# YannisLamp/crypto-recommendation

Measured on AMD Instinct MI355X. Metric: point hash+assign ops/sec at d=128, N=10M, K=256; 1/2/4/8 MI355X, higher is better.
Workload: dtype fp32 points; split-f16 MFMA scores (f32 accumulate); tuples, bucket IDs and cluster IDs bit-exact (x87-exact hashing, certified argmin); distances: certified f32, <= 2^-20 relative to the reference's fp64 (north star: 1e-5; the context's default LSHKM_DIST_CERTIFIED mode), LSHKM_DIST_EXACT for the r; 1 GPU; C3 Lloyd K=256 + C2 LSH L=5 k=4 hashing, N=10000000 per GPU, d=128; N_per_gpu=10000000, N_total=10000000, d=128, K=256, L=5, k=4, nb=100000, parallelism=dp1 (row shards)

## Files before the change

### crypto-recommendation_amd/csrc/api.cpp

```cpp
#include <hip/hip_runtime.h>

#include <algorithm>
#include <cmath>
#include <cstring>
#include <map>
#include <mutex>
#include <random>
#include <sstream>
#include <string>
#include <vector>

#include "../../include/lshkm.h"
#include "common.h"
#include "kernels.h"
#include "index.h"

namespace lshkm {
static thread_local std::string g_err;
void set_error(const std::string& msg) { g_err = msg; }

int device_cu_count(int* ncu) {
    static std::mutex mu;
    static std::map<int, int> cus;
    int dev = 0;
// ... 288 lines not shown
    return 0;
}

extern "C" {

int lshkm_kmeans_pp(lshkm_ctx ctx, const float* X, int64_t N, int d, int K, int metric, uint64_t seed,
                    int32_t* rows) {
    return kmeans_pp_impl(ctx, X, N, d, K, metric, seed, rows);
}

int lshkm_kmeans_pp_f64(lshkm_ctx ctx, const double* X, int64_t N, int d, int K, int metric, uint64_t seed,
                        int32_t* rows) {
    return kmeans_pp_impl(ctx, X, N, d, K, metric, seed, rows);
}

}

struct KppShardHost {
    uint64_t max_bits;
    double sum, s_out;
    int64_t pick;
};

static int kpp_shard_ws_check(lshkm_ctx ctx, int64_t n, const void* ws, int64_t ws_bytes) {
    LSHKM_CHECK(ctx && n >= 0 && n <= INT32_MAX, LSHKM_ERR_ARG, "bad arguments (need 0 <= n < 2^31)");
    LSHKM_CHECK(n == 0 || (ws && ws_bytes >= 0 && (size_t)ws_bytes >= kmeans_pp_ws_bytes(n)), LSHKM_ERR_ARG,
                "workspace smaller than lshkm_kpp_shard_ws_bytes");
    LSHKM_HIP(hipSetDevice(ctx->device));
    return 0;
}

static int kpp_shard_read(lshkm_ctx ctx, int64_t n, const void* ws, KppShardHost* out) {
    LSHKM_HIP(hipMemcpyAsync(out, (const char*)ws + kpp_shard_out_offset(n), sizeof(*out), hipMemcpyDeviceToHost,
                             ctx->stream));
    LSHKM_HIP(hipStreamSynchronize(ctx->stream));
    return 0;
}

static int kpp_shard_dist_impl(lshkm_ctx ctx, Pts X, int64_t n, int d, int metric, const void* c, int it, void* ws,
                               int64_t ws_bytes, uint64_t* max_bits, double* sum) {
    if (const int rc = kpp_shard_ws_check(ctx, n, ws, ws_bytes)) return rc;
    LSHKM_CHECK(max_bits && sum && d >= 1 && d <= 4096 && it >= 1, LSHKM_ERR_ARG,
                "bad arguments (need 1 <= d <= 4096, it >= 1)");
    LSHKM_CHECK(metric == LSHKM_METRIC_EUCLIDEAN || metric == LSHKM_METRIC_COSINE, LSHKM_ERR_ARG, "unknown metric");
    *max_bits = 0;
    *sum = 0.0;
    if (n == 0) return 0;
    LSHKM_CHECK(X.p && c, LSHKM_ERR_ARG, "rows or centroid row is NULL");
    KppShardHost o;
    int rc;
    if ((rc = launch_kpp_shard_dist(ctx->stream, X, n, d, metric, c, it, ws)) || (rc = kpp_shard_read(ctx, n, ws, &o))) {
        (void)hipStreamSynchronize(ctx->stream);
        return rc;
    }
    *max_bits = o.max_bits;
    *sum = o.sum;
    return 0;
}

extern "C" {

int lshkm_kpp_shard_ws_bytes(int64_t n, int64_t* bytes) {
    LSHKM_CHECK(bytes && n >= 0 && n <= INT32_MAX, LSHKM_ERR_ARG, "bad arguments (need 0 <= n < 2^31)");
    *bytes = (int64_t)kmeans_pp_ws_bytes(n);
    return 0;
}

int lshkm_kpp_shard_dist(lshkm_ctx ctx, const float* X, int64_t n, int d, int metric, const float* c, int it, void* ws,
                         int64_t ws_bytes, uint64_t* max_bits, double* sum) {
    return kpp_shard_dist_impl(ctx, X, n, d, metric, c, it, ws, ws_bytes, max_bits, sum);
}

int lshkm_kpp_shard_dist_f64(lshkm_ctx ctx, const double* X, int64_t n, int d, int metric, const double* c, int it,
                             void* ws, int64_t ws_bytes, uint64_t* max_bits, double* sum) {
    return kpp_shard_dist_impl(ctx, X, n, d, metric, c, it, ws, ws_bytes, max_bits, sum);
}

int lshkm_kpp_shard_units(lshkm_ctx ctx, int64_t n, uint64_t gmax_bits, double start, void* ws, int64_t ws_bytes) {
    if (const int rc = kpp_shard_ws_check(ctx, n, ws, ws_bytes)) return rc;
    if (n == 0) return 0;
    return launch_kpp_shard_units(ctx->stream, n, gmax_bits, start, ws);
}

int lshkm_kpp_shard_chain(lshkm_ctx ctx, int64_t n, double s_in, void* ws, int64_t ws_bytes, double* s_out) {
    if (const int rc = kpp_shard_ws_check(ctx, n, ws, ws_bytes)) return rc;
    LSHKM_CHECK(s_out, LSHKM_ERR_ARG, "s_out is NULL");
    *s_out = s_in;
    if (n == 0) return 0;
    KppShardHost o;
    int rc;
    if ((rc = launch_kpp_shard_chain(ctx->stream, n, s_in, ws, (unsigned long long*)ctx->stats.p)) ||
        (rc = kpp_shard_read(ctx, n, ws, &o))) {
        (void)hipStreamSynchronize(ctx->stream);
        return rc;
    }
    *s_out = o.s_out;
    return 0;
}

int lshkm_kpp_shard_pick(lshkm_ctx ctx, int64_t n, double rd, int owns_row0, void* ws, int64_t ws_bytes,
                         int64_t* row) {
    if (const int rc = kpp_shard_ws_check(ctx, n, ws, ws_bytes)) return rc;
    LSHKM_CHECK(row, LSHKM_ERR_ARG, "row is NULL");
    *row = -1;
    if (n == 0) return 0;
    KppShardHost o;
    int rc;
    if ((rc = launch_kpp_shard_pick(ctx->stream, n, rd, owns_row0, ws)) || (rc = kpp_shard_read(ctx, n, ws, &o))) {
        (void)hipStreamSynchronize(ctx->stream);
        return rc;
    }
    LSHKM_CHECK(o.pick >= -1 && o.pick < n, LSHKM_ERR_STATE, "pick outside the shard (rd above the running sum?)");
    *row = o.pick;
    return 0;
}

int lshkm_params_cube_cosine(uint64_t seed, int k, int d, double* R, uint32_t* state) {
    LSHKM_CHECK(k > 0 && d > 0 && R, LSHKM_ERR_ARG, "bad arguments");
    std::default_random_engine g;
    g.seed((unsigned long)seed);
    for (int i = 0; i < k; i++) draw_cosine_h(g, d, R + (size_t)i * d);
    if (state) *state = engine_state(g);
    return 0;
}

}

namespace lshkm {

int ProjTable::upload(hipStream_t s, int metric_, int d_, int L_, int k_, float w_, const float* V, const float* t,
                      const int32_t* r, const double* R) {
    metric = metric_; d = d_; L = L_; k = k_; w = w_;
    LK = L * k;
    LKpad = hash_lkpad(LK);
    const int drows = (d + 3) / 4 * 4;
    std::vector<double> PT((size_t)drows * LKpad, 0.0), pn(LK, 0.0);
    std::vector<float> tt(LK, 0.f);
    std::vector<int32_t> rr(LK, 0);
    for (int f = 0; f < LK; f++) {
        long double n2 = 0.0L;
        for (int j = 0; j < d; j++) {
            const double v = metric == LSHKM_METRIC_EUCLIDEAN ? (double)V[(size_t)f * d + j] : R[(size_t)f * d + j];
            PT[(size_t)j * LKpad + f] = v;
            n2 += (long double)v * (long double)v;
        }
        pn[f] = (double)sqrtl(n2) * (1.0 + 0x1p-40);
        if (metric == LSHKM_METRIC_EUCLIDEAN) { tt[f] = t ? t[f] : 0.f; rr[f] = r ? r[f] : 0; }
    }
    int rc;
    if ((rc = PT_d.reserve(PT.size() * 8)) || (rc = t_d.reserve(LK * 4)) || (rc = pn_d.reserve(LK * 8)) ||
        (rc = r_d.reserve(LK * 4)))
        return rc;
    LSHKM_HIP(hipMemcpyAsync(PT_d.p, PT.data(), PT.size() * 8, hipMemcpyHostToDevice, s));
    LSHKM_HIP(hipMemcpyAsync(t_d.p, tt.data(), LK * 4, hipMemcpyHostToDevice, s));
    LSHKM_HIP(hipMemcpyAsync(pn_d.p, pn.data(), LK * 8, hipMemcpyHostToDevice, s));
    LSHKM_HIP(hipMemcpyAsync(r_d.p, rr.data(), LK * 4, hipMemcpyHostToDevice, s));
    bool r_small = true;
    for (int f = 0; f < LK; f++) r_small = r_small && rr[f] >= 0 && rr[f] <= 100;
    fused_ok = metric == LSHKM_METRIC_EUCLIDEAN && d == 128 && LK <= 32 && r_small;
    mfma_ok = d == 128 && LK <= 32;
    std::vector<_Float16> vh, vl;
    std::vector<double> v1;
    if (mfma_ok) {
        vh.assign(64 * 128, (_Float16)0.f);
        vl.assign(64 * 128, (_Float16)0.f);
        v1.assign(LK, 0.0);
        for (int f = 0; f < LK; f++) {
            long double s1 = 0.0L;
            for (int j = 0; j < 128; j++) {
                const double v = metric == LSHKM_METRIC_EUCLIDEAN ? (double)V[(size_t)f * d + j] : R[(size_t)f * d + j];
                const _Float16 hv = (_Float16)v;
                vh[f * 128 + j] = hv;
                vl[f * 128 + j] = (_Float16)(float)(v - (double)hv);
                s1 += fabsl((long double)v);
            }
            v1[f] = (double)s1 * (1.0 + 0x1p-40);
        }
        if ((rc = vh_d.reserve(vh.size() * 2)) || (rc = vl_d.reserve(vl.size() * 2)) || (rc = v1_d.reserve(LK * 8)))
            return rc;
        LSHKM_HIP(hipMemcpyAsync(vh_d.p, vh.data(), vh.size() * 2, hipMemcpyHostToDevice, s));
        LSHKM_HIP(hipMemcpyAsync(vl_d.p, vl.data(), vl.size() * 2, hipMemcpyHostToDevice, s));
        LSHKM_HIP(hipMemcpyAsync(v1_d.p, v1.data(), LK * 8, hipMemcpyHostToDevice, s));
    }
    LSHKM_HIP(hipStreamSynchronize(s));
    hV.assign(V ? V : (const float*)nullptr, V ? V + (size_t)LK * d : nullptr);
    return 0;
}

HashParams ProjTable::params(int64_t nb) const {
    HashParams p;
    p.PT = (const double*)PT_d.p;
    p.t = (const float*)t_d.p;
    p.pnorm = (const double*)pn_d.p;
    p.r = (const int32_t*)r_d.p;
    p.w = w;
    p.d = d; p.L = L; p.k = k; p.LK = LK; p.LKpad = LKpad;
    p.nb = nb;
    return p;
}

HashMfmaParams ProjTable::mfma_params(int64_t nb) const {
    HashMfmaParams p;
    p.Vh = vh_d.as<_Float16>(); p.Vl = vl_d.as<_Float16>();
    p.t = (const float*)t_d.p; p.pnorm = (const double*)pn_d.p; p.v1 = (const double*)v1_d.p;
    p.r = (const int32_t*)r_d.p; p.PT = (const double*)PT_d.p;
    p.w = w;
    p.d = d; p.L = L; p.k = k; p.LK = LK; p.LKpad = LKpad;
    p.nb = nb;
    return p;
}

}

extern "C" {

int lshkm_lsh_create(lshkm_ctx ctx, int metric, int d, int k, int L, int64_t nb, float w, const float* V,
                     const float* t, const int32_t* r, const double* R, lshkm_lsh* out) {
    LSHKM_CHECK(ctx && out, LSHKM_ERR_ARG, "ctx/out is NULL");
    LSHKM_CHECK(d > 0 && d <= 1024 && k > 0 && L > 0 && L * k <= 256, LSHKM_ERR_ARG, "unsupported d/k/L");
    LSHKM_CHECK(k <= 30, LSHKM_ERR_ARG, "k > 30");
    if (metric == LSHKM_METRIC_EUCLIDEAN) {
        LSHKM_CHECK(V && t && r, LSHKM_ERR_ARG, "euclidean LSH needs V, t, r");
        LSHKM_CHECK(nb > 0 && nb < (1ll << 31), LSHKM_ERR_ARG, "nb must be in [1, 2^31)");
        LSHKM_CHECK(w > 0.f, LSHKM_ERR_ARG, "w must be > 0");
    } else if (metric == LSHKM_METRIC_COSINE) {
        LSHKM_CHECK(R, LSHKM_ERR_ARG, "cosine LSH needs R");
        nb = (int64_t)1 << k;
    } else {
        set_error("unknown metric");
        return LSHKM_ERR_ARG;
    }
    LSHKM_HIP(hipSetDevice(ctx->device));
    lshkm_lsh h = new lshkm_lsh_s();
    h->ctx = ctx; h->metric = metric; h->nb = nb;
    int rc = h->proj.upload(ctx->stream, metric, d, L, k, w, V, t, r, R);
    if (rc) { delete h; return rc; }
    *out = h;
    return 0;
}

int lshkm_lsh_destroy(lshkm_lsh lsh) {
    if (!lsh) return 0;
    (void)hipDeviceSynchronize();
    delete lsh;
    return 0;
}

}

static int lsh_hash_impl(lshkm_lsh lsh, Pts X, int64_t N, int32_t* tuples, int32_t* phi, int32_t* bucket) {
    LSHKM_CHECK(lsh && (X.p || N == 0) && N >= 0, LSHKM_ERR_ARG, "bad arguments");
    lshkm_ctx ctx = lsh->ctx;
    LSHKM_HIP(hipSetDevice(ctx->device));
    const int mode = lsh->metric == LSHKM_METRIC_EUCLIDEAN ? HM_LSH_EUCLID : HM_LSH_COSINE;
    const int rc = hash_rows(ctx, mode, X, N, lsh->proj, lsh->nb, mode == HM_LSH_EUCLID ? tuples : nullptr, phi, bucket,
                             nullptr);
    if (rc) { LSHKM_LAUNCH_CHECK(); return rc; }
    return 0;
}

extern "C" {

int lshkm_lsh_hash(lshkm_lsh lsh, const float* X, int64_t N, int32_t* tuples, int32_t* phi, int32_t* bucket) {
    return lsh_hash_impl(lsh, X, N, tuples, phi, bucket);
}

int lshkm_lsh_hash_f64(lshkm_lsh lsh, const double* X, int64_t N, int32_t* tuples, int32_t* phi, int32_t* bucket) {
    return lsh_hash_impl(lsh, X, N, tuples, phi, bucket);
}

}

static int assign_path(int metric, int d, int K, bool f64) {
    if (test_switch("LSHKM_ASSIGN_PATH", "exact")) return 2;
    if (!test_switch("LSHKM_ASSIGN_PATH", "f32")) {
        const FusedRoute r = fused_route(metric != LSHKM_METRIC_EUCLIDEAN, f64, d, K, false, 0, 0,
                                         test_switch("LSHKM_FUSED_FORM", "chunked"));
        if (r.form != FusedForm::none) return r.rows == 0 ? 0 : 3;
    }
    return assign_dp(d) > 0 ? 1 : 2;
}

static bool fuse_hash(const lshkm_lsh_s* lsh, int metric, int K, bool f64) {
    const lshkm::ProjTable& pj = lsh->proj;
    if (lsh->metric != metric || !(metric == LSHKM_METRIC_EUCLIDEAN ? pj.fused_ok : pj.mfma_ok)) return false;
    return fused_route(metric != LSHKM_METRIC_EUCLIDEAN, f64, pj.d, K, true, pj.k, pj.LK,
                       test_switch("LSHKM_FUSED_FORM", "chunked")).form != FusedForm::none;
}

bool lshkm::exact_pruned(Pts X, int d, int K, int metric) {
    return K <= 1024 && d <= 256 && !test_switch("LSHKM_EXACT_PASS", "full") &&
           (metric == LSHKM_METRIC_EUCLIDEAN || !X.f64);
}

static size_t exact_ct_bytes(const AssignJob& q) { return (size_t)q.d * ((q.K + 255) / 256 * 256) * 8; }

int lshkm::exact_listed_prep(lshkm_ctx ctx, const AssignJob& q) {
    int rc;
    if ((rc = ctx->ws_ct.reserve(exact_ct_bytes(q)))) return rc;
    return launch_assign_pruned_prep(ctx->stream, q.X.f64, q.d, q.C, q.K, (float*)ctx->ws_ct.p,
                                     q.metric == LSHKM_METRIC_EUCLIDEAN ? 0 : 1);
}

int lshkm::exact_listed(lshkm_ctx ctx, const AssignJob& q, const RowList& l, bool exact_dist, bool prepped,
                        const double* xn2, const double* nbv) {
    const bool prune = exact_pruned(q.X, q.d, q.K, q.metric);
    if (!prune && (q.metric != LSHKM_METRIC_EUCLIDEAN || (l.nseg == 0 && q.d > 256)))
        return launch_assign_exact(ctx->stream, q, l, xn2, nbv);
    int rc;
    if ((rc = ctx->ws_ct.reserve(exact_ct_bytes(q)))) return rc;
    if (prune) return launch_assign_pruned_list(ctx->stream, q, (float*)ctx->ws_ct.p, l, exact_dist ? 1 : 0, prepped);
    return launch_assign_exact_list(ctx->stream, q, (double*)ctx->ws_ct.p, l);
}

static int assign_f32_mfma(lshkm_ctx ctx, const AssignJob& q) {
    hipStream_t s = ctx->stream;
    const int DP = assign_dp(q.d), Kpad = (q.K + 63) / 64 * 64;
    const int64_t N = q.N;
    int rc;
    if ((rc = ctx->ws_c32.reserve((size_t)Kpad * DP * 4)) || (rc = ctx->ws_cconst.reserve((size_t)3 * Kpad * 4)) ||
        (rc = ctx->ws_ambig.reserve((size_t)std::max<int64_t>(N, 1) * 2 * 4)) ||
        (rc = ctx->ws_counter.reserve(64)))
        return rc;
    unsigned long long* cnt = (unsigned long long*)ctx->ws_counter.p;
    LSHKM_HIP(hipMemsetAsync(cnt, 0, 16, s));
    if ((rc = launch_centroid_prep(s, q.C, q.K, Kpad, q.d, DP, q.metric, q.X.f64, (float*)ctx->ws_c32.p, (float*)ctx->ws_cconst.p))) return rc;
    if ((rc = launch_assign_mfma(s, q.X, N, q.d, DP, q.C, q.K, Kpad, q.metric, (const float*)ctx->ws_c32.p, (const float*)ctx->ws_cconst.p,
                                 q.assign, q.dist, (int32_t*)ctx->ws_ambig.p, cnt))) return rc;
    RowList l;
    l.p = (int32_t*)ctx->ws_ambig.p; l.count = cnt; l.bound = N;
    if ((rc = exact_listed(ctx, q, l, true, false, nullptr, nullptr))) return rc;
    if (q.metric != LSHKM_METRIC_EUCLIDEAN &&
        ((rc = launch_cos_fix(s, q.X, N, q.d, q.C, (const int32_t*)ctx->ws_ambig.p + N, cnt + 1, q.assign, q.dist)) ||
         (rc = launch_add_counter(s, (unsigned long long*)ctx->stats.p + STAT_COS_FIX, cnt + 1)))) return rc;
    return launch_add_counter(s, (unsigned long long*)ctx->stats.p + STAT_ASSIGN_AMBIG, cnt);
}

static int assign_impl(lshkm_ctx ctx, Pts X, int64_t N, int d, const double* C, int K, int metric,
                       const int32_t* src_rows_host, int32_t* assign, double* dist, lshkm_lsh lsh, int32_t* tuples,
                       int32_t* phi, int32_t* bucket, bool force_exact = false) {
    hipStream_t s = ctx->stream;
    const int path = assign_path(metric, d, K, X.f64);
    AssignRequest q;
    q.X = X; q.N = N; q.d = d; q.C = C; q.K = K; q.metric = metric; q.assign = assign; q.dist = dist;
    q.tuples = tuples; q.phi = phi; q.bucket = bucket; q.force_exact = force_exact;
    if (lsh && path == 0 && fuse_hash(lsh, metric, K, X.f64)) q.lsh = lsh;
    int rc;
    if (lsh && !q.lsh && (rc = hash_rows(ctx, lsh->metric == LSHKM_METRIC_EUCLIDEAN ? HM_LSH_EUCLID : HM_LSH_COSINE,
                                         X, N, lsh->proj, lsh->nb,
                                         lsh->metric == LSHKM_METRIC_EUCLIDEAN ? tuples : nullptr, phi, bucket,
                                         nullptr))) { LSHKM_LAUNCH_CHECK(); return rc; }
    if (path == 0 || path == 3) rc = fused_assign(ctx, q);
    else if (path == 1) rc = assign_f32_mfma(ctx, q);
    else {
        RowList all;
        all.bound = N;
        rc = launch_assign_exact(s, q, all);
    }
    if (rc) { LSHKM_LAUNCH_CHECK(); return rc; }
    if (src_rows_host) {
        if ((rc = ctx->ws_src.reserve((size_t)K * 4))) return rc;
        const bool same = ctx->src_cache_dev == ctx->ws_src.p && ctx->src_cache_cap == ctx->ws_src.cap &&
                          ctx->src_cache.size() == (size_t)K &&
                          std::memcmp(ctx->src_cache.data(), src_rows_host, (size_t)K * 4) == 0;
        if (!same) {
            if ((rc = ctx->pin_stage((size_t)K * 4))) return rc;
            std::memcpy(ctx->pinned, src_rows_host, (size_t)K * 4);
            LSHKM_HIP(hipMemcpyAsync(ctx->ws_src.p, ctx->pinned, (size_t)K * 4, hipMemcpyHostToDevice, s));
            LSHKM_HIP(hipEventRecord(ctx->pinned_ev, s));
            ctx->src_cache.assign(src_rows_host, src_rows_host + K);
            ctx->src_cache_dev = ctx->ws_src.p;
            ctx->src_cache_cap = ctx->ws_src.cap;
        }
        if ((rc = launch_assign_override(s, (const int32_t*)ctx->ws_src.p, K, N, assign, dist))) { LSHKM_LAUNCH_CHECK(); return rc; }
    }
    return 0;
}

static int lloyd_impl(lshkm_ctx ctx, Pts X, int64_t N, int d, const double* C, int K, int metric,
                      const int32_t* src_rows_host, int32_t* assign, double* dist) {
    LSHKM_CHECK(ctx && (X.p || N == 0) && C && (assign || N == 0) && (dist || N == 0) && N >= 0 && d > 0 && K > 0,
                LSHKM_ERR_ARG, "bad arguments");
    LSHKM_CHECK(metric == LSHKM_METRIC_EUCLIDEAN || metric == LSHKM_METRIC_COSINE, LSHKM_ERR_ARG, "unknown metric");
    LSHKM_HIP(hipSetDevice(ctx->device));
    return assign_impl(ctx, X, N, d, C, K, metric, src_rows_host, assign, dist, nullptr, nullptr, nullptr, nullptr);
}

static int hash_assign_impl(lshkm_lsh lsh, Pts X, int64_t N, const double* C, int K, const int32_t* src_rows_host,
                            int32_t* tuples, int32_t* phi, int32_t* bucket, int32_t* assign, double* dist,
                            int metric = LSHKM_METRIC_EUCLIDEAN) {
    LSHKM_CHECK(lsh && (X.p || N == 0) && C && (assign || N == 0) && (dist || N == 0) && N >= 0 && K > 0, LSHKM_ERR_ARG,
                "bad arguments");
    lshkm_ctx ctx = lsh->ctx;
    LSHKM_HIP(hipSetDevice(ctx->device));
    LSHKM_CHECK(metric == LSHKM_METRIC_EUCLIDEAN || metric == LSHKM_METRIC_COSINE, LSHKM_ERR_ARG, "unknown metric");
    return assign_impl(ctx, X, N, lsh->proj.d, C, K, metric, src_rows_host, assign, dist, lsh, tuples, phi, bucket);
}

static int range_impl(lshkm_ctx ctx, Pts X, int64_t N, int d, const double* C, int K, int metric,
                      const int64_t* comb_ptr, const int32_t* comb_idx, const int32_t* key_host,
                      const int32_t* src_rows_host, int32_t* assign, double* dist, int* passes_host) {
    LSHKM_CHECK(ctx && (X.p || N == 0) && C && comb_ptr && (assign || N == 0) && (dist || N == 0) && N >= 0 &&
                    N < (1ll << 31) && d > 0 && K > 0,
                LSHKM_ERR_ARG, "bad arguments");
    LSHKM_CHECK(metric == LSHKM_METRIC_EUCLIDEAN || metric == LSHKM_METRIC_COSINE, LSHKM_ERR_ARG, "unknown metric");
    LSHKM_HIP(hipSetDevice(ctx->device));
    hipStream_t s = ctx->stream;
    lshkm::Buf* w = ctx->ws_range;
    int rc;
    int64_t M = 0;
    LSHKM_HIP(hipMemcpyAsync(&M, comb_ptr + K, 8, hipMemcpyDeviceToHost, s));
    LSHKM_HIP(hipStreamSynchronize(s));
    LSHKM_CHECK(M >= 0 && (M == 0 || comb_idx), LSHKM_ERR_ARG, "bad combined-bucket CSR");
    const size_t scratch = sort_scratch_bytes(std::max<int64_t>(M, 1), std::max<int64_t>(N, 1));
    if ((rc = w[0].reserve(64)) || (rc = w[1].reserve((size_t)std::max<int64_t>(M, 1) * 4 * 4)) ||
        (rc = w[2].reserve(scratch)) || (rc = w[3].reserve((size_t)(N + 1) * 8)) ||
        (rc = w[4].reserve((size_t)std::max<int64_t>(M, 1) * 9)) || (rc = w[5].reserve((size_t)K * 4)))
        return rc;
    double* r0 = (double*)w[0].p;
    unsigned long long* cnt = (unsigned long long*)w[0].p + 1;
    int32_t* rows = (int32_t*)w[1].p;
    int32_t* cents = rows + std::max<int64_t>(M, 1);
    int32_t* rows_s = cents + std::max<int64_t>(M, 1);
    int32_t* cents_s = rows_s + std::max<int64_t>(M, 1);
    int64_t* vptr = (int64_t*)w[3].p;
    double* cache = (double*)w[4].p;
    int8_t* cached = (int8_t*)(cache + std::max<int64_t>(M, 1));
    const int32_t* key = nullptr;
    if (key_host) {
        LSHKM_HIP(hipMemcpyAsync(w[5].p, key_host, (size_t)K * 4, hipMemcpyHostToDevice, s));
        key = (const int32_t*)w[5].p;
    }
    if ((rc = launch_range_radius(s, C, K, d, metric, r0, (unsigned long long*)w[0].p + 4))) return rc;
    if ((rc = launch_range_init(s, N, assign, dist))) return rc;
    int passes = 0;
    if (M > 0 && N > 0) {
        if ((rc = launch_range_pairs(s, comb_ptr, comb_idx, K, rows, cents))) return rc;
        if ((rc = stable_sort_by_key(s, rows, 1, cents, M, N, rows_s, cents_s, w[2].p))) return rc;
        if ((rc = launch_csr_bounds(s, rows_s, M, N, vptr))) return rc;
        LSHKM_HIP(hipMemsetAsync(cached, 0, (size_t)M, s));
        for (;;) {
            unsigned long long assigned = 0;
            LSHKM_HIP(hipMemsetAsync(cnt, 0, 8, s));
            if ((rc = launch_range_pass(s, X, d, C, K, metric, key, vptr, cents_s, cache, cached, N, r0, passes,
                                        assign, dist, cnt)))
                return rc;
            passes++;
            LSHKM_HIP(hipMemcpyAsync(&assigned, cnt, 8, hipMemcpyDeviceToHost, s));
            LSHKM_HIP(hipStreamSynchronize(s));
            if (!assigned) break;
        }
    } else {
        passes = 1;
    }
    if (N > 0) {
        if ((rc = w[6].reserve((size_t)N * 4))) return rc;
        int32_t* list = (int32_t*)w[6].p;
        unsigned long long* ucnt = cnt + 1;
        unsigned long long U = 0;
        LSHKM_HIP(hipMemsetAsync(ucnt, 0, 8, s));
        if ((rc = launch_range_unassigned(s, assign, N, list, ucnt))) return rc;
        LSHKM_HIP(hipMemcpyAsync(&U, ucnt, 8, hipMemcpyDeviceToHost, s));
        LSHKM_HIP(hipStreamSynchronize(s));
        if (U > 0) {
            if ((rc = w[7].reserve((size_t)U * d * X.esize())) || (rc = w[8].reserve((size_t)U * 12))) return rc;
            double* dr = (double*)w[8].p;
            int32_t* ar = (int32_t*)(dr + U);
            if ((rc = launch_range_gather(s, X, d, list, (int64_t)U, w[7].p))) return rc;
            const Pts Xr = X.f64 ? Pts(w[7].as<double>()) : Pts(w[7].as<float>());
            rc = assign_impl(ctx, Xr, (int64_t)U, d, C, K, metric, nullptr, ar, dr, nullptr, nullptr, nullptr, nullptr,
                             true);
            if (rc) return rc;
            if ((rc = launch_range_scatter(s, list, (int64_t)U, ar, dr, assign, dist))) return rc;
        }
    }
    if (src_rows_host) {
        if ((rc = ctx->ws_src.reserve((size_t)K * 4))) return rc;
        ctx->src_cache_dev = nullptr;
        LSHKM_HIP(hipMemcpyAsync(ctx->ws_src.p, src_rows_host, (size_t)K * 4, hipMemcpyHostToDevice, s));
        if ((rc = launch_assign_override(s, (const int32_t*)ctx->ws_src.p, K, N, assign, dist))) return rc;
        LSHKM_HIP(hipStreamSynchronize(s));
    }
    if (key_host) LSHKM_HIP(hipStreamSynchronize(s));
    if (passes_host) *passes_host = passes;
    return 0;
}

extern "C" {

int lshkm_lloyd_assign(lshkm_ctx ctx, const float* X, int64_t N, int d, const double* C, int K, int metric,
                       const int32_t* src_rows_host, int32_t* assign, double* dist) {
    return lloyd_impl(ctx, X, N, d, C, K, metric, src_rows_host, assign, dist);
}

int lshkm_lloyd_assign_f64(lshkm_ctx ctx, const double* X, int64_t N, int d, const double* C, int K, int metric,
                           const int32_t* src_rows_host, int32_t* assign, double* dist) {
    return lloyd_impl(ctx, X, N, d, C, K, metric, src_rows_host, assign, dist);
}

int lshkm_hash_assign(lshkm_lsh lsh, const float* X, int64_t N, const double* C, int K, const int32_t* src_rows_host,
                      int32_t* tuples, int32_t* phi, int32_t* bucket, int32_t* assign, double* dist) {
    return hash_assign_impl(lsh, X, N, C, K, src_rows_host, tuples, phi, bucket, assign, dist);
}

int lshkm_hash_assign_f64(lshkm_lsh lsh, const double* X, int64_t N, const double* C, int K,
                          const int32_t* src_rows_host, int32_t* tuples, int32_t* phi, int32_t* bucket,
                          int32_t* assign, double* dist) {
    return hash_assign_impl(lsh, X, N, C, K, src_rows_host, tuples, phi, bucket, assign, dist);
}

int lshkm_hash_assign_metric(lshkm_lsh lsh, const float* X, int64_t N, const double* C, int K, int metric,
                             const int32_t* src_rows_host, int32_t* tuples, int32_t* phi, int32_t* bucket,
                             int32_t* assign, double* dist) {
    return hash_assign_impl(lsh, X, N, C, K, src_rows_host, tuples, phi, bucket, assign, dist, metric);
}

int lshkm_hash_assign_metric_f64(lshkm_lsh lsh, const double* X, int64_t N, const double* C, int K, int metric,
                                 const int32_t* src_rows_host, int32_t* tuples, int32_t* phi, int32_t* bucket,
                                 int32_t* assign, double* dist) {
    return hash_assign_impl(lsh, X, N, C, K, src_rows_host, tuples, phi, bucket, assign, dist, metric);
}

int lshkm_range_assign(lshkm_ctx ctx, const float* X, int64_t N, int d, const double* C, int K, int metric,
                       const int64_t* comb_ptr, const int32_t* comb_idx, const int32_t* key_host,
                       const int32_t* src_rows_host, int32_t* assign, double* dist, int* passes_host) {
    return range_impl(ctx, X, N, d, C, K, metric, comb_ptr, comb_idx, key_host, src_rows_host, assign, dist,
                      passes_host);
}

int lshkm_range_assign_f64(lshkm_ctx ctx, const double* X, int64_t N, int d, const double* C, int K, int metric,
                           const int64_t* comb_ptr, const int32_t* comb_idx, const int32_t* key_host,
                           const int32_t* src_rows_host, int32_t* assign, double* dist, int* passes_host) {
    return range_impl(ctx, X, N, d, C, K, metric, comb_ptr, comb_idx, key_host, src_rows_host, assign, dist,
                      passes_host);
}

int lshkm_synth(lshkm_ctx ctx, uint64_t seed, int64_t row0, int64_t rows, int d, float* X) {
    LSHKM_CHECK(ctx && (X || rows == 0) && rows >= 0 && d > 0, LSHKM_ERR_ARG, "bad arguments");
    LSHKM_HIP(hipSetDevice(ctx->device));
    int rc = launch_synth(ctx->stream, seed, row0, rows, d, X);
    if (rc) { LSHKM_LAUNCH_CHECK(); }
    return rc;
}

int lshkm_synth_normal(lshkm_ctx ctx, uint64_t seed, int64_t row0, int64_t rows, int d, float* X) {
    LSHKM_CHECK(ctx && (X || rows == 0) && rows >= 0 && d > 0, LSHKM_ERR_ARG, "bad arguments");
    LSHKM_HIP(hipSetDevice(ctx->device));
    int rc = launch_synth(ctx->stream, seed, row0, rows, d, X, 1);
    if (rc) { LSHKM_LAUNCH_CHECK(); }
    return rc;
}

}
```

### crypto-recommendation_amd/csrc/assign.hip

```cpp
#include "common.h"
#include "kernels.h"
#include "exact.h"

namespace lshkm {

constexpr int AS_THREADS = 256;
constexpr int AS_PB = 128;
constexpr int AS_CC = 64;

typedef float floatx16 __attribute__((ext_vector_type(16)));

int assign_dp(int d) {
    const int dps[] = {16, 32, 64, 128, 256};
    for (int dp : dps)
        if (d <= dp) return dp;
    return 0;
}

__global__ void centroid_prep_kernel(const double* __restrict__ C, int K, int Kpad, int d, int DP, int metric,
                                     int xf64, float* __restrict__ C32, float* __restrict__ cconst) {
    const int c = blockIdx.x * 64 + threadIdx.x;
    const double xw = xf64 ? 2.0 : 0.0;
    float* cn2 = cconst;
    float* chunk = cconst + Kpad + 2 * blockIdx.x;
// ... 269 lines not shown

constexpr int XC_MAXV = 4;
constexpr int XE_SPLIT = 2;
template <typename TX>
__global__ __launch_bounds__(256) void assign_exact_kernel(
    const TX* __restrict__ X, int64_t N, int d, const double* __restrict__ C, int K, int metric,
    const int32_t* __restrict__ rows, const unsigned long long* __restrict__ row_count, int64_t max_rows,
    int32_t* __restrict__ assign, double* __restrict__ dist, const int32_t* __restrict__ seg_counts,
    int64_t seg_rows, const double* __restrict__ xn2, const double* __restrict__ nbv) {
    const int lane = threadIdx.x & 63;
    int64_t wglobal = (int64_t)blockIdx.x * 4 + (threadIdx.x >> 6);
    int64_t nw = (int64_t)gridDim.x * 4;
    int64_t total = rows ? (int64_t)*row_count : N;
    if (seg_counts) {
        const int seg = blockIdx.x % (gridDim.x / XE_SPLIT);
        rows += (int64_t)seg * seg_rows;
        total = seg_counts[SEG_SLOTS * seg + SEG_ROWS];
        wglobal = (int64_t)(blockIdx.x / (gridDim.x / XE_SPLIT)) * 4 + (threadIdx.x >> 6);
        nw = XE_SPLIT * 4;
    }
    if (total > max_rows) total = max_rows;
    for (int64_t it = wglobal; it < total; it += nw) {
        const int64_t row = rows ? rows[it] : it;
        const TX* x = X + row * d;
        double best = 0.0; int bi = -1;
        const double xa = metric == 1 && xn2 ? xn2[row] : -1.0;
        if (metric == 1 && K <= 64 * XC_MAXV) {
            double v[XC_MAXV], rad[XC_MAXV];
            int st[XC_MAXV];
            double U = __builtin_inf();
            bool unknown = false;
#pragma unroll
            for (int k = 0; k < XC_MAXV; k++) {
                const int c = lane + 64 * k;
                st[k] = 0; v[k] = 0.0; rad[k] = 0.0;
                if (c < K) {
                    st[k] = cosine_interval(x, C + (size_t)c * d, d, v[k], rad[k], xa, nbv ? nbv[c] : -1.0);
                    unknown |= st[k] == 2;
                    if (st[k] != 2) U = fmin(U, v[k] + rad[k]);
                }
            }
            if (!__ballot(unknown)) {
                for (int off = 32; off >= 1; off >>= 1) U = fmin(U, __shfl_xor(U, off));
#pragma unroll
                for (int k = 0; k < XC_MAXV; k++) {
                    const int c = lane + 64 * k;
                    if (c < K && v[k] - rad[k] <= U) {
                        const double dd = st[k] == 0 ? v[k] : exact_cosine_x87(x, C + (size_t)c * d, d, xa, nbv ? nbv[c] : -1.0);
                        if (bi < 0 || dd < best) { best = dd; bi = c; }
                    }
                }
                for (int off = 32; off >= 1; off >>= 1) {
                    const double ob = __shfl_xor(best, off);
                    const int oi = __shfl_xor(bi, off);
                    const bool take = oi >= 0 && (bi < 0 || ob < best || (ob == best && oi < bi));
                    if (take) { best = ob; bi = oi; }
                }
                if (lane == 0) {
                    assign[row] = bi;
                    dist[row] = best;
                }
                continue;
            }
        }
        for (int c = lane; c < K; c += 64) {
            const double dd = metric == 0 ? exact_euclid(x, C + (size_t)c * d, d)
                                          : exact_cosine_x87(x, C + (size_t)c * d, d, xa, nbv ? nbv[c] : -1.0);
            if (bi < 0 ? (dd == dd || c == 0) : dd < best) { best = dd; bi = c; }
        }
        for (int off = 32; off >= 1; off >>= 1) {
            const double ob = __shfl_xor(best, off);
            const int oi = __shfl_xor(bi, off);
            const bool take = oi >= 0 && (bi < 0 || ob < best || (ob == best && oi < bi));
            if (take) { best = ob; bi = oi; }
        }
        if (lane == 0) {
            assign[row] = bi < 0 ? 0 : bi;
            dist[row] = bi < 0 ? -1.0 : best;
        }
    }
}

int launch_assign_exact(hipStream_t s, const AssignJob& q, const RowList& l, const double* xn2, const double* nbv) {
    const Pts X = q.X;
    const int64_t N = q.N, max_rows = l.bound, seg_rows = l.seg_rows;
    const int d = q.d, K = q.K, metric = q.metric, nseg = l.nseg;
    const double* C = q.C;
    const int32_t *rows = l.p, *seg_counts = l.seg_counts();
    const unsigned long long* row_count = l.count;
    int32_t* assign = q.assign;
    double* dist = q.dist;
    if (max_rows <= 0) return 0;
    const int64_t blocks = seg_counts ? (int64_t)nseg * XE_SPLIT : std::min<int64_t>((max_rows + 3) / 4, rows ? 256 : 2048);
    if (blocks <= 0) return 0;
    if (X.f64)
        hipLaunchKernelGGL(assign_exact_kernel<double>, dim3((unsigned)blocks), dim3(256), 0, s, X.d(), N, d, C, K,
                           metric, rows, row_count, max_rows, assign, dist, seg_counts, seg_rows, xn2, nbv);
    else
        hipLaunchKernelGGL(assign_exact_kernel<float>, dim3((unsigned)blocks), dim3(256), 0, s, X.f(), N, d, C, K,
                           metric, rows, row_count, max_rows, assign, dist, seg_counts, seg_rows, xn2, nbv);
    return kstatus("assign.hip");
}

constexpr int XB_R = 8;
constexpr int XB_WAVES = 4;
constexpr int XB_SPLIT = 4;
constexpr int XB_DMAX = 256;

__global__ void transpose_centroids_kernel(const double* __restrict__ C, int K, int Kpad, int d,
                                           double* __restrict__ CT) {
    const int64_t e = (int64_t)blockIdx.x * blockDim.x + threadIdx.x;
    if (e >= (int64_t)d * Kpad) return;
    const int j = (int)(e / Kpad), c = (int)(e % Kpad);
    CT[e] = c < K ? C[(size_t)c * d + j] : 0.0;
}

template <typename TX>
__global__ __launch_bounds__(64 * XB_WAVES) void assign_exact_batch_kernel(
    const TX* __restrict__ X, int d, const double* __restrict__ CT, int K, int Kpad,
    const int32_t* __restrict__ rows, const unsigned long long* __restrict__ row_count, int64_t max_rows,
    int32_t* __restrict__ assign, double* __restrict__ dist, const int32_t* __restrict__ seg_counts,
    int64_t seg_rows) {
    __shared__ TX xs[XB_WAVES][XB_R][XB_DMAX];
    const int lane = threadIdx.x & 63, wave = threadIdx.x >> 6;
    int64_t total, g0, gstride;
    if (seg_counts) {
        const int nseg = gridDim.x / XB_SPLIT;
        const int seg = blockIdx.x % nseg, part = blockIdx.x / nseg;
        rows += (int64_t)seg * seg_rows;
        total = seg_counts[SEG_SLOTS * seg + SEG_ROWS];
        g0 = (int64_t)part * XB_WAVES + wave;
        gstride = (int64_t)XB_SPLIT * XB_WAVES;
    } else {
        total = (int64_t)*row_count;
        if (total > max_rows) total = max_rows;
        g0 = (int64_t)blockIdx.x * XB_WAVES + wave;
        gstride = (int64_t)gridDim.x * XB_WAVES;
    }
    const int64_t ngroups = (total + XB_R - 1) / XB_R;
    for (int64_t g = g0; g < ngroups; g += gstride) {
        const int nr = (int)min((int64_t)XB_R, total - g * XB_R);
        int64_t myrow[XB_R];
#pragma unroll
        for (int r = 0; r < XB_R; r++) myrow[r] = rows[g * XB_R + min(r, nr - 1)];
#pragma unroll
        for (int r = 0; r < XB_R; r++)
            for (int j = lane; j < d; j += 64) xs[wave][r][j] = X[myrow[r] * d + j];
        wave_sync();
        double best[XB_R];
        int bi[XB_R];
#pragma unroll
        for (int r = 0; r < XB_R; r++) { best[r] = 0.0; bi[r] = -1; }
        for (int c0 = 0; c0 < K; c0 += 256) {
            double acc[XB_R][4];
#pragma unroll
            for (int r = 0; r < XB_R; r++)
#pragma unroll
                for (int i = 0; i < 4; i++) acc[r][i] = 0.0;
            const double* ct = CT + c0 + lane;
#pragma unroll 4
            for (int j = 0; j < d; j++) {
                double cv[4];
#pragma unroll
                for (int i = 0; i < 4; i++) cv[i] = ct[(size_t)j * Kpad + 64 * i];
#pragma unroll
                for (int r = 0; r < XB_R; r++) {
                    const double xj = (double)xs[wave][r][j];
#pragma unroll
                    for (int i = 0; i < 4; i++) {
                        const double df = __dsub_rn(xj, cv[i]);
                        acc[r][i] = __dadd_rn(acc[r][i], gp_sq(df));
                    }
                }
            }
#pragma unroll
            for (int i = 0; i < 4; i++) {
                const int c = c0 + lane + 64 * i;
                if (c >= K) continue;
#pragma unroll
                for (int r = 0; r < XB_R; r++) {
                    const double dd = sqrt(acc[r][i]);
                    if (bi[r] < 0 || dd < best[r]) { best[r] = dd; bi[r] = c; }
                }
            }
        }
#pragma unroll
        for (int r = 0; r < XB_R; r++) {
            double b = best[r];
            int i1 = bi[r];
            for (int off = 32; off >= 1; off >>= 1) {
                const double ob = __shfl_xor(b, off);
                const int oi = __shfl_xor(i1, off);
                const bool take = oi >= 0 && (i1 < 0 || ob < b || (ob == b && oi < i1));
                if (take) { b = ob; i1 = oi; }
            }
            if (lane == 0 && r < nr) {
                assign[myrow[r]] = i1;
                dist[myrow[r]] = b;
            }
        }
        wave_sync();
    }
}

#ifndef XP_ROWS
#define XP_ROWS 8
#endif
#ifndef XP_SPLITS
#define XP_SPLITS 4
#endif
constexpr int XP_R = XP_ROWS;
#ifndef XP_WIDE_ROWS
#define XP_WIDE_ROWS 2
#endif
constexpr int XP_WR = XP_WIDE_ROWS;
constexpr int XP_WAVES = 4;
constexpr int XP_SPLIT = XP_SPLITS;

template <typename TX>
__device__ __attribute__((always_inline)) inline double exact_euclid_rolled(const TX* __restrict__ x,
                                                                            const double* __restrict__ c, int d) {
    double acc = 0.0;
#pragma unroll 1
    for (int j = 0; j < d; j++) acc = __dadd_rn(acc, gp_sq(__dsub_rn((double)x[j], c[j])));
    return sqrt(acc);
}

template <int MET, typename TX>
__device__ inline double pruned_dist(const TX* __restrict__ x, const double* __restrict__ c, int d) {
    if constexpr (MET == 0) {
        return exact_euclid_rolled(x, c, d);
    } else {
        if constexpr (sizeof(TX) == 4) {
            if ((d & 15) == 0) return exact_cosine_x87_b16(x, c, d);
        }
        return exact_cosine_x87(x, c, d);
    }
}

template <typename TX>
__device__ inline double euclid_sumsq_mul(const TX* __restrict__ x, const double* __restrict__ c, int d, PwAcc& pw) {
    double acc = 0.0;
    for (int j0 = 0; j0 < d; j0 += 16) {
        double cv[16];
#pragma unroll
        for (int t = 0; t < 16; t++) cv[t] = j0 + t < d ? c[j0 + t] : 0.0;
#pragma unroll
        for (int t = 0; t < 16; t++)
            if (j0 + t < d) {
                const double df = __dsub_rn((double)x[j0 + t], cv[t]);
                const double p = __dmul_rn(df, df);
                pw.add<true>(df);
                acc = __dadd_rn(acc, p);
            }
    }
    return acc;
}

template <int G>
__device__ inline void group_argmin(double& best, int& bi) {
#pragma unroll
    for (int off = G / 2; off >= 1; off >>= 1) {
        const double ob = __shfl_xor(best, off);
        const int oi = __shfl_xor(bi, off);
        const bool take = oi >= 0 && (bi < 0 || ob < best || (ob == best && oi < bi));
        if (take) { best = ob; bi = oi; }
    }
}
template <int G>
__device__ inline double group_min(double v) {
#pragma unroll
    for (int off = G / 2; off >= 1; off >>= 1) v = fmin(v, __shfl_xor(v, off));
    return v;
}

template <int G, typename TX>
__device__ inline void pruned_pick_euclid(const TX* __restrict__ xr, const double* __restrict__ C, int d, int c,
                                          bool exact_dist, double& best, int& bi) {
    PwAcc pw;
    const double S = c >= 0 ? euclid_sumsq_mul(xr, C + (size_t)c * d, d, pw) : 0.0;
    const bool hard = c >= 0 && pw.hard();
    best = c >= 0 ? sqrt(S) : 0.0;
    bi = c;
    group_argmin<G>(best, bi);
    int anyh = hard ? 1 : 0;
#pragma unroll
    for (int off = G / 2; off >= 1; off >>= 1) anyh |= __shfl_xor(anyh, off);
    if (!anyh) return;
    const double S1 = group_min<G>(c >= 0 && c == bi ? S : __builtin_inf());
    const double S2 = group_min<G>(c >= 0 && c != bi ? S : __builtin_inf());
    if (S2 != __builtin_inf() && !(S2 - S1 > 0x1p-41 * S2)) {
        best = c >= 0 ? exact_euclid_rolled(xr, C + (size_t)c * d, d) : 0.0;
        bi = c;
        group_argmin<G>(best, bi);
        return;
    }
    if (!exact_dist) return;
    const int w = bi;
    double v = __builtin_inf();
    if (c == w) v = hard ? exact_euclid_rolled(xr, C + (size_t)c * d, d) : best;
    best = group_min<G>(v);
}

__global__ void exact_prep_kernel(const double* __restrict__ C, int K, int Kpad, int d, int xf64,
                                  float* __restrict__ CT32, float* __restrict__ cconst, int metric) {
    const int c = blockIdx.x, lane = threadIdx.x;
    double scale = 1.0;
    if (metric == 1) {
        double q = 0.0;
        for (int j = lane; j < d; j += 64) {
            const double v = c < K ? C[(size_t)c * d + j] : 0.0;
            q = fma(v, v, q);
        }
        for (int off = 32; off >= 1; off >>= 1) q += __shfl_xor(q, off);
        scale = (q >= 1e-200 && q <= 1e200) ? 1.0 / sqrt(q) : 0.0;
        if (c < K && scale == 0.0) {
            for (int j = lane; j < d; j += 64) CT32[(size_t)j * Kpad + c] = 0.f;
            if (lane == 0) cconst[c] = __builtin_inff();
            return;
        }
    }
    double sq = 0.0;
    for (int j = lane; j < d; j += 64) {
        const double v = c < K ? C[(size_t)c * d + j] * scale : 0.0;
        sq = fma(v, v, sq);
        CT32[(size_t)j * Kpad + c] = (float)v;
    }
    for (int off = 32; off >= 1; off >>= 1) sq += __shfl_xor(sq, off);
    if (lane != 0) return;
    if (c >= K) { cconst[c] = __builtin_inff(); return; }
    if (metric == 1) {
        cconst[c] = 0.f;
        const double ec = ((d + 2.0) * 0x1p-24 * (1.0 + 0x1p-10) + 0x1p-40 + (xf64 ? 0x1p-23 : 0.0)) * (1.0 + 0x1p-18);
        unsigned int* chunk = reinterpret_cast<unsigned int*>(cconst + Kpad + 2 * (c / 64));
        atomicMax(chunk, __float_as_uint((float)(ec * (1.0 + 0x1p-20))));
        atomicMax(chunk + 1, __float_as_uint(1e-30f));
        return;
    }
    const double up = 1.0 + 0x1p-18;
    const double nc = sqrt(sq) * (1.0 + 0x1p-30);
    cconst[c] = (float)sq;
    const double ec = 0x1p-24 * (2.0 * d + 12.0 + (xf64 ? 2.0 : 0.0)) * nc * up;
    const double eb = (0x1p-24 * 5.0 * sq + 0x1p-40 * sq + (xf64 ? 0x1p-140 * nc : 0.0)) * up + 1e-30;
    unsigned int* chunk = reinterpret_cast<unsigned int*>(cconst + Kpad + 2 * (c / 64));
    atomicMax(chunk, __float_as_uint((float)(ec * (1.0 + 0x1p-20))));
    atomicMax(chunk + 1, __float_as_uint((float)(eb * (1.0 + 0x1p-20))));
}

template <typename TX, int NCH = 4, int R = XP_R, int MET = 0>
__global__ __launch_bounds__(64 * XP_WAVES) void assign_pruned_kernel(
    const TX* __restrict__ X, int d, const double* __restrict__ C, const float* __restrict__ CT32,
    const float* __restrict__ cconst, int K, int Kpad, const int32_t* __restrict__ rows,
    const unsigned long long* __restrict__ row_count, int64_t max_rows, int32_t* __restrict__ assign,
    double* __restrict__ dist, const int32_t* __restrict__ seg_counts, int64_t seg_rows, int exact_dist) {
    constexpr int RL = 64 / R;
    __shared__ TX xs[XP_WAVES][R][XB_DMAX];
    const int lane = threadIdx.x & 63, wave = threadIdx.x >> 6;
    int64_t total, g0, gstride;
    if (seg_counts) {
        const int nseg = gridDim.x / XP_SPLIT;
        const int seg = blockIdx.x % nseg, part = blockIdx.x / nseg;
        rows += (int64_t)seg * seg_rows;
        total = seg_counts[SEG_SLOTS * seg + SEG_ROWS];
        g0 = (int64_t)part * XP_WAVES + wave;
        gstride = (int64_t)XP_SPLIT * XP_WAVES;
    } else {
        total = (int64_t)*row_count;
        if (total > max_rows) total = max_rows;
        g0 = (int64_t)blockIdx.x * XP_WAVES + wave;
        gstride = (int64_t)gridDim.x * XP_WAVES;
    }
    const float* chunkc = cconst + Kpad;
    const int64_t ngroups = (total + R - 1) / R;
    for (int64_t g = g0; g < ngroups; g += gstride) {
        const int nr = (int)min((int64_t)R, total - g * R);
        int32_t myrow[R];
#pragma unroll
        for (int r = 0; r < R; r++) myrow[r] = rows[g * R + min(r, nr - 1)];
        float xn2p[R];
        TX xv[R][XB_DMAX / 64];
#pragma unroll
        for (int r = 0; r < R; r++)
#pragma unroll
            for (int u = 0; u < XB_DMAX / 64; u++) {
                const int j = lane + 64 * u;
                xv[r][u] = j < d ? X[(int64_t)myrow[r] * d + j] : TX(0);
            }
#pragma unroll
        for (int r = 0; r < R; r++) {
            float q = 0.f;
#pragma unroll
            for (int u = 0; u < XB_DMAX / 64; u++) {
                const int j = lane + 64 * u;
                if (j < d) {
                    xs[wave][r][j] = xv[r][u];
                    q = fmaf((float)xv[r][u], (float)xv[r][u], q);
                }
            }
            xn2p[r] = q;
        }
        wave_sync();
        float acc[R][NCH];
#pragma unroll
        for (int r = 0; r < R; r++)
#pragma unroll
            for (int i = 0; i < NCH; i++) acc[r][i] = 0.f;
        int coff[NCH];
#pragma unroll
        for (int i = 0; i < NCH; i++) coff[i] = (64 * i < Kpad ? 64 * i : 0) + lane;
#pragma unroll 8
        for (int j = 0; j < d; j++) {
            float cv[NCH];
#pragma unroll
            for (int i = 0; i < NCH; i++) cv[i] = CT32[(size_t)j * Kpad + coff[i]];
#pragma unroll
            for (int r = 0; r < R; r++) {
                const float xj = (float)xs[wave][r][j];
#pragma unroll
                for (int i = 0; i < NCH; i++) acc[r][i] = fmaf(xj, cv[i], acc[r][i]);
            }
        }
        unsigned long long cm[R][NCH];
        int ncand[R];
        bool pr[R];
#pragma unroll
        for (int r = 0; r < R; r++) {
            double xn2 = (double)xn2p[r];
            for (int off = 32; off >= 1; off >>= 1) xn2 += __shfl_xor(xn2, off);
            xn2 = xn2 * (sizeof(TX) == 4 ? 1.0 + 0x1p-20 : 1.0 + 0x1p-19) + (sizeof(TX) == 4 ? 0.0 : 0x1p-280);
            const float nx = (float)(sqrt(xn2) * (1.0 + 0x1p-30));
            const float ex = (float)(0x1p-40 * xn2 * (1.0 + 0x1p-18) + 1e-30);
            float lo[NCH];
            float U = __builtin_inff();
            bool finite = nx <= 3.0e38f;
#pragma unroll
            for (int i = 0; i < NCH; i++) {
                const int c = lane + 64 * i;
                lo[i] = __builtin_inff();
                if (c < K) {
                    const float E = fmaf(nx, chunkc[2 * i], chunkc[2 * i + 1] + ex);
                    const float sc = MET == 1 ? cconst[c] - acc[r][i] : fmaf(-2.f, acc[r][i], cconst[c]);
                    lo[i] = sc - E;
                    const float hi = sc + E;
                    finite = finite && (hi - lo[i]) <= 3.0e38f;
                    U = fminf(U, hi);
                }
            }
            for (int off = 32; off >= 1; off >>= 1) U = fminf(U, __shfl_xor(U, off));
            ncand[r] = 0;
#pragma unroll
            for (int i = 0; i < NCH; i++) {
                cm[r][i] = __ballot(lo[i] <= U);
                ncand[r] += __popcll(cm[r][i]);
            }
            pr[r] = r < nr && __all(finite) && ncand[r] >= 1;
        }
        {
            const int r = lane / RL, k = lane % RL;
            int c = -1;
            int seen = 0;
#pragma unroll
            for (int rr = 0; rr < R; rr++) {
                if (rr != r || !pr[rr] || ncand[rr] > RL) continue;
#pragma unroll
                for (int i = 0; i < NCH; i++) {
                    const int n = __popcll(cm[rr][i]);
                    if (c < 0 && k >= seen && k < seen + n) {
                        unsigned long long m = cm[rr][i];
                        for (int t = k - seen; t > 0; t--) m &= m - 1;
                        c = 64 * i + __builtin_ctzll(m);
                    }
                    seen += n;
                }
            }
            double best = 0.0;
            int bi = -1;
            if constexpr (MET == 0) {
                pruned_pick_euclid<RL>(xs[wave][r], C, d, c, exact_dist != 0, best, bi);
            } else {
                if (c >= 0) {
                    best = pruned_dist<MET>(xs[wave][r], C + (size_t)c * d, d);
                    bi = c;
                }
                group_argmin<RL>(best, bi);
            }
            if (k == 0 && bi >= 0) {
                assign[myrow[r]] = bi;
                dist[myrow[r]] = best;
            }
        }
        for (int r = 0; r < nr; r++) {
            if (pr[r] && ncand[r] <= RL) continue;
            const bool prune = pr[r] && ncand[r] <= 64;
            const TX* xr = xs[wave][r];
            double best = 0.0;
            int bi = -1;
            if (prune) {
                int c = -1, seen = 0;
#pragma unroll
                for (int i = 0; i < NCH; i++) {
                    const int n = __popcll(cm[r][i]);
                    if (c < 0 && lane >= seen && lane < seen + n) {
                        unsigned long long m = cm[r][i];
                        for (int t = lane - seen; t > 0; t--) m &= m - 1;
                        c = 64 * i + __builtin_ctzll(m);
                    }
                    seen += n;
                }
                if constexpr (MET == 0) {
                    pruned_pick_euclid<64>(xr, C, d, c, exact_dist != 0, best, bi);
                } else if (c >= 0) {
                    best = pruned_dist<MET>(xr, C + (size_t)c * d, d);
                    bi = c;
                }
            } else {
                for (int c = lane; c < K; c += 64) {
                    const double dd = pruned_dist<MET>(xr, C + (size_t)c * d, d);
                    if (bi < 0 ? (dd == dd || c == 0) : dd < best) { best = dd; bi = c; }
                }
            }
            for (int off = 32; off >= 1; off >>= 1) {
                const double ob = __shfl_xor(best, off);
                const int oi = __shfl_xor(bi, off);
                const bool take = oi >= 0 && (bi < 0 || ob < best || (ob == best && oi < bi));
                if (take) { best = ob; bi = oi; }
            }
            if (lane == 0) {
                assign[myrow[r]] = bi < 0 ? 0 : bi;
                dist[myrow[r]] = bi < 0 ? -1.0 : best;
            }
        }
        wave_sync();
    }
}

#ifndef XPW_ROWS
#define XPW_ROWS 4
#endif
constexpr int XPW_MAXSEG = 4096;
template <typename TX, int MET = 0, int NCH = 16, int R = XPW_ROWS>
__global__ __launch_bounds__(64 * XP_WAVES) void assign_pruned_wide_kernel(
    const TX* __restrict__ X, int d, const double* __restrict__ C, const float* __restrict__ CT32,
    const float* __restrict__ cconst, int K, int Kpad, const int32_t* __restrict__ rows,
    const unsigned long long* __restrict__ row_count, int64_t max_rows, int32_t* __restrict__ assign,
    double* __restrict__ dist, const int32_t* __restrict__ seg_counts, int64_t seg_rows, int nseg, int exact_dist) {
    __shared__ TX xs[XP_WAVES][R][XB_DMAX];
    __shared__ int gpre[XPW_MAXSEG + 1];
    const int lane = threadIdx.x & 63, wave = threadIdx.x >> 6;
    int64_t ngroups;
    if (seg_counts) {
        for (int sg = threadIdx.x; sg < nseg; sg += 64 * XP_WAVES) gpre[sg + 1] = (seg_counts[SEG_SLOTS * sg + SEG_ROWS] + R - 1) / R;
        __syncthreads();
        if (threadIdx.x == 0) {
            gpre[0] = 0;
            for (int sg = 0; sg < nseg; sg++) gpre[sg + 1] += gpre[sg];
        }
        __syncthreads();
        ngroups = gpre[nseg];
    } else {
        int64_t total = (int64_t)*row_count;
        if (total > max_rows) total = max_rows;
        ngroups = (total + R - 1) / R;
    }
    const float* chunkc = cconst + Kpad;
    const int64_t g0 = (int64_t)blockIdx.x * XP_WAVES + wave, gstride = (int64_t)gridDim.x * XP_WAVES;
    for (int64_t g = g0; g < ngroups; g += gstride) {
        const int32_t* grows;
        int64_t gbase, cnt;
        if (seg_counts) {
            int lo = 0, hi = nseg;
            while (hi - lo > 1) {
                const int mid = (lo + hi) >> 1;
                if (gpre[mid] <= g) lo = mid; else hi = mid;
            }
            grows = rows + (int64_t)lo * seg_rows;
            gbase = (g - gpre[lo]) * R;
            cnt = seg_counts[SEG_SLOTS * lo + SEG_ROWS];
        } else {
            grows = rows;
            gbase = g * R;
            cnt = min((int64_t)*row_count, max_rows);
        }
        const int nr = (int)min((int64_t)R, cnt - gbase);
        int32_t myrow[R];
#pragma unroll
        for (int r = 0; r < R; r++) myrow[r] = grows[gbase + min(r, nr - 1)];
        float xn2p[R];
#pragma unroll
        for (int r = 0; r < R; r++) {
            TX xv[XB_DMAX / 64];
#pragma unroll
            for (int u = 0; u < XB_DMAX / 64; u++) {
                const int j = lane + 64 * u;
                xv[u] = j < d ? X[(int64_t)myrow[r] * d + j] : TX(0);
            }
            float q = 0.f;
#pragma unroll
            for (int u = 0; u < XB_DMAX / 64; u++) {
                const int j = lane + 64 * u;
                if (j < d) {
                    xs[wave][r][j] = xv[u];
                    q = fmaf((float)xv[u], (float)xv[u], q);
                }
            }
            xn2p[r] = q;
        }
        wave_sync();
        float acc[R][NCH];
#pragma unroll
        for (int r = 0; r < R; r++)
#pragma unroll
            for (int i = 0; i < NCH; i++) acc[r][i] = 0.f;
        int coff[NCH];
#pragma unroll
        for (int i = 0; i < NCH; i++) coff[i] = (64 * i < Kpad ? 64 * i : 0) + lane;
#pragma unroll 2
        for (int j = 0; j < d; j++) {
            float cv[NCH];
#pragma unroll
            for (int i = 0; i < NCH; i++) cv[i] = CT32[(size_t)j * Kpad + coff[i]];
#pragma unroll
            for (int r = 0; r < R; r++) {
                const float xj = (float)xs[wave][r][j];
#pragma unroll
                for (int i = 0; i < NCH; i++) acc[r][i] = fmaf(xj, cv[i], acc[r][i]);
            }
        }
#pragma unroll
        for (int r = 0; r < R; r++) {
            if (r >= nr) break;
            double xn2 = (double)xn2p[r];
            for (int off = 32; off >= 1; off >>= 1) xn2 += __shfl_xor(xn2, off);
            xn2 = xn2 * (sizeof(TX) == 4 ? 1.0 + 0x1p-20 : 1.0 + 0x1p-19) + (sizeof(TX) == 4 ? 0.0 : 0x1p-280);
            const float nx = (float)(sqrt(xn2) * (1.0 + 0x1p-30));
            const float ex = (float)(0x1p-40 * xn2 * (1.0 + 0x1p-18) + 1e-30);
            float lo[NCH];
            float U = __builtin_inff();
            bool finite = nx <= 3.0e38f;
#pragma unroll
            for (int i = 0; i < NCH; i++) {
                const int c = lane + 64 * i;
                lo[i] = __builtin_inff();
                if (c < K) {
                    const float E = fmaf(nx, chunkc[2 * i], chunkc[2 * i + 1] + ex);
                    const float sc = MET == 1 ? cconst[c] - acc[r][i] : fmaf(-2.f, acc[r][i], cconst[c]);
                    lo[i] = sc - E;
                    const float hi = sc + E;
                    finite = finite && (hi - lo[i]) <= 3.0e38f;
                    U = fminf(U, hi);
                }
            }
            for (int off = 32; off >= 1; off >>= 1) U = fminf(U, __shfl_xor(U, off));
            unsigned long long cm[NCH];
            int ncand = 0;
#pragma unroll
            for (int i = 0; i < NCH; i++) {
                cm[i] = __ballot(lo[i] <= U);
                ncand += __popcll(cm[i]);
            }
            const bool prune = __all(finite) && ncand >= 1 && ncand <= 64;
            const TX* xr = xs[wave][r];
            double best = 0.0;
            int bi = -1;
            if (prune) {
                int c = -1, seen = 0;
#pragma unroll
                for (int i = 0; i < NCH; i++) {
                    const int n = __popcll(cm[i]);
                    if (c < 0 && lane >= seen && lane < seen + n) {
                        unsigned long long m = cm[i];
                        for (int t = lane - seen; t > 0; t--) m &= m - 1;
                        c = 64 * i + __builtin_ctzll(m);
                    }
                    seen += n;
                }
                if constexpr (MET == 0) {
                    pruned_pick_euclid<64>(xr, C, d, c, exact_dist != 0, best, bi);
                } else if (c >= 0) {
                    best = pruned_dist<MET>(xr, C + (size_t)c * d, d);
                    bi = c;
                }
            } else {
                for (int c = lane; c < K; c += 64) {
                    const double dd = pruned_dist<MET>(xr, C + (size_t)c * d, d);
                    if (bi < 0 ? (dd == dd || c == 0) : dd < best) { best = dd; bi = c; }
                }
            }
            for (int off = 32; off >= 1; off >>= 1) {
                const double ob = __shfl_xor(best, off);
                const int oi = __shfl_xor(bi, off);
                const bool take = oi >= 0 && (bi < 0 || ob < best || (ob == best && oi < bi));
                if (take) { best = ob; bi = oi; }
            }
            if (lane == 0) {
                assign[myrow[r]] = bi < 0 ? 0 : bi;
                dist[myrow[r]] = bi < 0 ? -1.0 : best;
            }
        }
        wave_sync();
    }
}

int launch_assign_pruned_prep(hipStream_t s, bool xf64, int d, const double* C, int K, float* ws, int metric) {
    if (d > XB_DMAX || K > 1024) {
        set_error("launch_assign_pruned_prep: unsupported shape");
        return -1;
    }
    const int Kpad = (K + 63) / 64 * 64;
    float* cconst = ws + (size_t)d * Kpad;
    if (hipMemsetAsync(cconst + Kpad, 0, (size_t)(Kpad / 64) * 2 * 4, s) != hipSuccess) return kstatus("pruned prep");
    hipLaunchKernelGGL(exact_prep_kernel, dim3((unsigned)Kpad), dim3(64), 0, s, C, K, Kpad, d, xf64 ? 1 : 0, ws, cconst,
                       metric);
    return kstatus("exact_prep_kernel");
}

int launch_assign_pruned_list(hipStream_t s, const AssignJob& q, float* ws, const RowList& l, int exact_dist,
                              bool prepped) {
    const Pts X = q.X;
    const int64_t max_rows = l.bound, seg_rows = l.seg_rows;
    const int d = q.d, K = q.K, nseg = l.nseg, metric = q.metric == 0 ? 0 : 1;
    const double* C = q.C;
    const int32_t *rows = l.p, *seg_counts = l.seg_counts();
    const unsigned long long* row_count = l.count;
    int32_t* assign = q.assign;
    double* dist = q.dist;
    if (max_rows <= 0) return 0;
    if (d > XB_DMAX || K > 1024 || (seg_counts && nseg <= 0)) {
        set_error("launch_assign_pruned_list: unsupported shape");
        return -1;
    }
    const int Kpad = (K + 63) / 64 * 64;
    float* CT32 = ws;
    float* cconst = ws + (size_t)d * Kpad;
    if (!prepped) {
        int rc = launch_assign_pruned_prep(s, X.f64, d, C, K, ws, metric);
        if (rc) return rc;
    }
    const bool wide = Kpad > 256;
    const bool flat = wide && (!seg_counts || nseg <= XPW_MAXSEG);
    const int R = wide ? (flat ? XPW_ROWS : XP_WR) : XP_R;
    const int64_t groups = (max_rows + R - 1) / R;
    const int64_t blocks = seg_counts ? (int64_t)nseg * XP_SPLIT : std::min<int64_t>((groups + XP_WAVES - 1) / XP_WAVES, 2048);
#define XP_LAUNCH(TX, NCH, RR, MT, XP)                                                                              \
    hipLaunchKernelGGL((assign_pruned_kernel<TX, NCH, RR, MT>), dim3((unsigned)blocks), dim3(64 * XP_WAVES), 0, s, XP, \
                       d, C, CT32, cconst, K, Kpad, rows, row_count, max_rows, assign, dist, seg_counts, seg_rows, exact_dist)
#define XPW_LAUNCH(TX, MT, NC, RW, XP)                                                                           \
    hipLaunchKernelGGL((assign_pruned_wide_kernel<TX, MT, NC, RW>), dim3((unsigned)wblocks), dim3(64 * XP_WAVES), 0, s, \
                       XP, d, C, CT32, cconst, K, Kpad, rows, row_count, max_rows, assign, dist, seg_counts, seg_rows, nseg, \
                       exact_dist)
    const int64_t wblocks = std::min<int64_t>((groups + XP_WAVES - 1) / XP_WAVES, 1024);
    if (flat) {
        if (metric == 1) {
            if (X.f64) XPW_LAUNCH(double, 1, 16, XPW_ROWS, X.d()); else XPW_LAUNCH(float, 1, 16, XPW_ROWS, X.f());
        } else {
            if (X.f64) XPW_LAUNCH(double, 0, 16, XPW_ROWS, X.d()); else XPW_LAUNCH(float, 0, 16, XPW_ROWS, X.f());
        }
    } else if (metric == 1) {
        if (X.f64) {
            if (wide) XP_LAUNCH(double, 16, XP_WR, 1, X.d()); else XP_LAUNCH(double, 4, XP_R, 1, X.d());
        } else {
            if (wide) XP_LAUNCH(float, 16, XP_WR, 1, X.f()); else XP_LAUNCH(float, 4, XP_R, 1, X.f());
        }
    } else if (X.f64) {
        if (wide) XP_LAUNCH(double, 16, XP_WR, 0, X.d()); else XP_LAUNCH(double, 4, XP_R, 0, X.d());
    } else {
        if (wide) XP_LAUNCH(float, 16, XP_WR, 0, X.f()); else XP_LAUNCH(float, 4, XP_R, 0, X.f());
    }
#undef XP_LAUNCH
#undef XPW_LAUNCH
    return kstatus("assign_pruned_kernel");
}

int launch_assign_exact_list(hipStream_t s, const AssignJob& q, double* CT, const RowList& l) {
    const Pts X = q.X;
    const int64_t max_rows = l.bound, seg_rows = l.seg_rows;
    const int d = q.d, K = q.K, nseg = l.nseg;
    const double* C = q.C;
    const int32_t *rows = l.p, *seg_counts = l.seg_counts();
    const unsigned long long* row_count = l.count;
    int32_t* assign = q.assign;
    double* dist = q.dist;
    if (max_rows <= 0) return 0;
    if (d > XB_DMAX || (seg_counts && nseg <= 0)) {
        set_error("launch_assign_exact_list: unsupported shape");
        return -1;
    }
    const int Kpad = (K + 255) / 256 * 256;
    const int64_t ne = (int64_t)d * Kpad;
    hipLaunchKernelGGL(transpose_centroids_kernel, dim3((unsigned)((ne + 255) / 256)), dim3(256), 0, s, C, K, Kpad, d, CT);
    const int64_t groups = (max_rows + XB_R - 1) / XB_R;
    const int64_t blocks = seg_counts ? (int64_t)nseg * XB_SPLIT : std::min<int64_t>((groups + XB_WAVES - 1) / XB_WAVES, 2048);
    if (X.f64)
        hipLaunchKernelGGL(assign_exact_batch_kernel<double>, dim3((unsigned)blocks), dim3(64 * XB_WAVES), 0, s, X.d(),
                           d, CT, K, Kpad, rows, row_count, max_rows, assign, dist, seg_counts, seg_rows);
    else
        hipLaunchKernelGGL(assign_exact_batch_kernel<float>, dim3((unsigned)blocks), dim3(64 * XB_WAVES), 0, s, X.f(),
                           d, CT, K, Kpad, rows, row_count, max_rows, assign, dist, seg_counts, seg_rows);
    return kstatus("assign_exact_batch_kernel");
}

__global__ void assign_override_kernel(const int32_t* __restrict__ src, int K, int64_t N,
                                       int32_t* __restrict__ assign, double* __restrict__ dist) {
    const int c = blockIdx.x * blockDim.x + threadIdx.x;
    if (c >= K) return;
    const int32_t r = src[c];
    if (r < 0 || r >= N) return;
    for (int c2 = c + 1; c2 < K; c2++)
        if (src[c2] == r) return;
    assign[r] = c;
    dist[r] = 0.0;
}

constexpr int OV_LDS_MAX = 8192;
__global__ __launch_bounds__(1024) void assign_override_lds_kernel(const int32_t* __restrict__ src, int K, int64_t N,
                                                                  int32_t* __restrict__ assign,
                                                                  double* __restrict__ dist) {
    __shared__ __attribute__((aligned(16))) int32_t ls[OV_LDS_MAX + 16];
    const int Kp = (K + 15) & ~15;
    for (int c = threadIdx.x; c < Kp + 16; c += blockDim.x) ls[c] = c < K ? src[c] : -1;
    __syncthreads();
    for (int c = threadIdx.x; c < K; c += blockDim.x) {
        const int32_t r = ls[c];
        if (r < 0 || r >= N) continue;
        bool later = false;
        for (int b = (c + 1) & ~15; b < Kp && !later; b += 16) {
            const int4 v0 = *reinterpret_cast<const int4*>(ls + b);
            const int4 v1 = *reinterpret_cast<const int4*>(ls + b + 4);
            const int4 v2 = *reinterpret_cast<const int4*>(ls + b + 8);
            const int4 v3 = *reinterpret_cast<const int4*>(ls + b + 12);
            const int w[16] = {v0.x, v0.y, v0.z, v0.w, v1.x, v1.y, v1.z, v1.w,
                               v2.x, v2.y, v2.z, v2.w, v3.x, v3.y, v3.z, v3.w};
#pragma unroll
            for (int t = 0; t < 16; t++) later |= b + t > c && w[t] == r;
        }
        if (!later) {
            assign[r] = c;
            dist[r] = 0.0;
        }
    }
}

int launch_assign_override(hipStream_t s, const int32_t* src_rows, int K, int64_t N, int32_t* assign,
                           double* dist) {
    if (K <= OV_LDS_MAX)
        hipLaunchKernelGGL(assign_override_lds_kernel, dim3(1), dim3(1024), 0, s, src_rows, K, N, assign, dist);
    else
        hipLaunchKernelGGL(assign_override_kernel, dim3((K + 255) / 256), dim3(256), 0, s, src_rows, K, N, assign,
                           dist);
    return kstatus("assign.hip");
}

__global__ void add_counter_kernel(unsigned long long* dst, const unsigned long long* src) {
    if (threadIdx.x == 0) *dst += *src;
}

int launch_add_counter(hipStream_t s, unsigned long long* dst, const unsigned long long* src) {
    hipLaunchKernelGGL(add_counter_kernel, dim3(1), dim3(1), 0, s, dst, src);
    return kstatus("assign.hip");
}

struct CounterAdds {
    int n;
    int dst[8];
    const unsigned long long* src[8];
};
__global__ void add_counters_kernel(unsigned long long* stats, CounterAdds c) {
    if ((int)threadIdx.x < c.n) atomicAdd(stats + c.dst[threadIdx.x], *c.src[threadIdx.x]);
}

int launch_add_counters(hipStream_t s, unsigned long long* stats, int n, const int* dst_idx,
                        const unsigned long long* const* src) {
    if (n <= 0) return 0;
    if (n > 8) {
        set_error("launch_add_counters: at most 8 counters");
        return -1;
    }
    CounterAdds c;
    c.n = n;
    for (int i = 0; i < n; i++) { c.dst[i] = dst_idx[i]; c.src[i] = src[i]; }
    hipLaunchKernelGGL(add_counters_kernel, dim3(1), dim3(64), 0, s, stats, c);
    return kstatus("assign.hip");
}

}
```

### crypto-recommendation_amd/csrc/common.h

```cpp
#pragma once
#include <hip/hip_runtime.h>
#include <stdint.h>
#include <string>
#ifdef LSHKM_TEST_SWITCHES
#include <cstdlib>
#include <cstring>
#endif

namespace lshkm {

inline bool test_switch(const char* name, const char* value) {
#ifdef LSHKM_TEST_SWITCHES
    const char* e = std::getenv(name);
    return e && !std::strcmp(e, value);
#else
    (void)name;
    (void)value;
    return false;
#endif
}

void set_error(const std::string& msg);

#define LSHKM_HIP(expr)                                                              \
    do {                                                                             \
        hipError_t _e = (expr);                                                      \
        if (_e != hipSuccess) {                                                      \
            ::lshkm::set_error(std::string(#expr) + ": " + hipGetErrorString(_e));   \
            return LSHKM_ERR_HIP;                                                    \
        }                                                                            \
    } while (0)

#define LSHKM_CHECK(cond, code, msg)                                                 \
    do {                                                                             \
        if (!(cond)) { ::lshkm::set_error(msg); return code; }                       \
    } while (0)

#define LSHKM_LAUNCH_CHECK() LSHKM_HIP(hipGetLastError())

inline int kstatus(const char* what) {
    const hipError_t e = hipGetLastError();
    if (e == hipSuccess) return 0;
    set_error(std::string(what) + ": " + hipGetErrorString(e));
    return -2;
}

__device__ inline void wave_sync() {
    __builtin_amdgcn_fence(__ATOMIC_RELEASE, "wavefront");
    __builtin_amdgcn_wave_barrier();
    __builtin_amdgcn_fence(__ATOMIC_ACQUIRE, "wavefront");
}

template <typename E, typename C>
__device__ __forceinline__ void seg_append(bool want, E entry, C* count, E* seg, int lane) {
    const unsigned long long m = __ballot(want);
    if (!m) return;
    const int leader = __builtin_ctzll(m);
    C base = 0;
    if (lane == leader) base = atomicAdd(count, (C)__popcll(m));
    base = __shfl(base, leader);
    if (want) seg[base + __popcll(m & ((1ull << lane) - 1ull))] = entry;
}

inline unsigned gsz(int64_t work, int64_t per_block, int64_t cap) {
    int64_t b = (work + per_block - 1) / per_block;
    if (b < 1) b = 1;
    if (b > cap) b = cap;
    return (unsigned)b;
}

enum Stat {
    STAT_HASH_EXACT = 0,
    STAT_ASSIGN_AMBIG = 1,
    STAT_KPP_CHUNKS = 2,
    STAT_KPP_SEQ = 3,
    STAT_COS_FIX = 4,
    STAT_REFINED = 5,
    STAT_HASH_FIX = 6,
    STAT_REC_SOFT = 7,
    STAT_POW_FIX = 8,
    STAT_KM_SEQ = 9,
    STAT_PAM_SCREENED = 10,
    STAT_PAM_EXACT = 11,
    STAT_COUNT = 12
};

constexpr int WAVE = 64;

int device_cu_count(int* ncu);

}
```

### crypto-recommendation_amd/csrc/fused.hip

```cpp
#include "../../include/lshkm.h"
#include "fused_impl.h"
#include "index.h"

namespace lshkm {

namespace {

struct FusedPlan {
    bool hash = false, cos = false;
    int rows = 0;
    int nblk = 0;
    int64_t seg_rows = 0;
    int np_hi = 0;
    int np_refine = 0;
};

int fused_workspace(lshkm_ctx ctx, const FusedShape& sh, FusedWorkspace& w) {
    const FusedLayout l = fused_layout(sh);
    int rc;
    struct { Buf& b; size_t bytes; } const bufs[] = {
        {ctx->ws_c32, l.c16},      {ctx->ws_cconst, l.cconst}, {ctx->ws_ambig, l.list1}, {ctx->ws_counter, l.counter},
        {ctx->ws_seg, l.seg1},     {ctx->ws_hfix, l.fix},      {ctx->ws_seg3, l.seg3},   {ctx->ws_part, l.part},
        {ctx->ws_ambig2, l.list2}, {ctx->ws_seg2, l.seg2},     {ctx->ws_tuples, l.tuples}, {ctx->ws_cf32, l.cf32},
        {ctx->ws_c64p, l.c64p},    {ctx->ws_xn2, l.xn2}};
    for (const auto& e : bufs)
        if (e.bytes && (rc = e.b.reserve(e.bytes))) return rc;
    const auto at = [](const Buf& b, size_t off) { return off == FusedLayout::NONE ? nullptr : (char*)b.p + off; };
    w.list_cap = l.list_cap;
    w.Ch = (_Float16*)at(ctx->ws_c32, 0); w.Cl = (_Float16*)at(ctx->ws_c32, l.cl_off);
    w.cbound = (float*)at(ctx->ws_cconst, 0); w.cnh = (float*)at(ctx->ws_cconst, l.cnh_off);
    w.nbv = (double*)at(ctx->ws_cconst, l.nbv_off);
    if (l.cf32) { w.C32 = (float*)at(ctx->ws_cf32, 0); w.rn32 = (float*)at(ctx->ws_cf32, l.rn32_off); }
    if (l.c64p) w.C64p = ctx->ws_c64p.as<double>();
    w.list1 = ctx->ws_ambig.as<int32_t>(); w.seg1 = ctx->ws_seg.as<int32_t>();
    w.list2 = ctx->ws_ambig2.as<int32_t>(); w.seg2 = ctx->ws_seg2.as<int32_t>();
    if (l.seg3) w.seg3 = ctx->ws_seg3.as<int32_t>();
    w.hfix = (unsigned long long*)at(ctx->ws_hfix, l.hfix_off);
    w.cfix = (unsigned long long*)at(ctx->ws_hfix, l.cfix_off);
    w.hfix2 = (unsigned long long*)at(ctx->ws_hfix, l.hfix2_off);
    if (l.part) w.part = ctx->ws_part.as<float4>();
    w.cnt = ctx->ws_counter.as<unsigned long long>();
    if (l.xn2) w.xn2 = ctx->ws_xn2.as<double>();
    if (l.tuples) w.tuples = ctx->ws_tuples.as<int32_t>();
    return 0;
}

FusedArgs fused_common_args(lshkm_ctx ctx, const AssignRequest& q, const FusedShape& sh, const FusedWorkspace& w) {
    FusedArgs a{};
    a.X = q.X.f64 ? nullptr : q.X.f(); a.X64 = q.X.f64 ? q.X.d() : nullptr;
    a.N = q.N; a.d = q.d;
    a.xvec = sh.rows == 1 ? (a.d % 4 == 0 && ((uintptr_t)a.X & 15) == 0) : (a.d % 2 == 0 && ((uintptr_t)a.X64 & 15) == 0);
    a.Ch = w.Ch; a.Cl = w.Cl; a.cnh = w.cnh; a.cbound = w.cbound; a.Kpad = sh.Kpad();
    a.C64 = w.C64p ? w.C64p : q.C; a.Cd = q.C;
    a.C32 = w.C32; a.rn32 = w.rn32; a.fast_dist = sh.fast ? 1 : 0;
    a.assign = q.assign; a.dist = q.dist;
    a.stats = ctx->stats.as<unsigned long long>();
    a.nb = 1;
    if (q.lsh) {
        const ProjTable& pj = q.lsh->proj;
        a.Vh = pj.vh_d.as<_Float16>(); a.Vl = pj.vl_d.as<_Float16>(); a.PT = pj.PT_d.as<double>();
        a.tv = pj.t_d.as<float>(); a.pnorm = pj.pn_d.as<double>(); a.v1 = pj.v1_d.as<double>();
        a.rv = pj.r_d.as<int32_t>(); a.w = pj.w; a.L = pj.L; a.k = pj.k; a.LK = pj.LK; a.LKpad = pj.LKpad;
        a.nb = q.lsh->nb;
    }
    a.bdiv = make_bucket_div(a.nb);
    if (sh.cosine) { a.nbv = w.nbv; a.xn2 = w.xn2; }
    a.cfix = w.cfix; a.cfix_counts = w.seg3; a.cfix_count = w.cfix ? w.cnt + CNT_CFIX : nullptr;
    a.pass_first = 1; a.pass_last = 1;
    return a;
}

void hash_outputs(FusedArgs& a, const AssignRequest& q, const FusedShape& sh, const FusedWorkspace& w) {
    a.hfix = w.hfix; a.hfix_count = w.hfix ? w.cnt + CNT_HFIX : nullptr;
    if (!q.lsh) return;
    a.phi = q.phi; a.bucket = q.bucket;
    a.tuples = sh.cosine ? nullptr : q.tuples ? q.tuples : w.tuples;
}

template <typename T>
DevList<T> segmented(T* p, unsigned long long* count, int32_t* counts, const AssignRequest& q, const FusedPlan& plan) {
    DevList<T> l;
    l.p = p; l.count = count; l.bound = q.N; l.counts = counts;
    l.seg_rows = plan.seg_rows; l.nseg = plan.nblk;
    return l;
}

int fused_hi_passes(hipStream_t s, const FusedArgs& hi, const FusedPlan& p) {
    const bool gather_on = !test_switch("LSHKM_GATHER", "0");
    int rc;
    if (p.rows != 0) {
        HiForm h;
        h.metric = p.cos; h.rows = p.rows;
        h.fast = !p.cos && hi.fast_dist;
        h.gath = !p.cos && !h.fast && p.rows == 1 && hi.Kpad <= FH_GATH_KMAX && gather_on;
        return launch_fused_hi_pass(s, p.nblk, h, hi);
    }
    if (!p.cos && p.np_hi == 2 && test_switch("LSHKM_HI_TWO_IMAGE", "1")) {
        HiForm h;
        h.hash = p.hash; h.two_image = true;
        return launch_fused_hi_pass(s, p.nblk, h, hi);
    }
    for (int i = 0; i < p.np_hi; i++) {
        const int c0 = i * FH_KMAX;
        FusedArgs a = hi;
        a.Ch = hi.Ch + (size_t)c0 * FU_D; a.cnh = hi.cnh + c0;
        a.Kpad = std::min(FH_KMAX, hi.Kpad - c0);
        a.t0 = c0 / 32; a.pass_first = i == 0; a.pass_last = i == p.np_hi - 1;
        HiForm h;
        h.hash = p.hash && i == 0; h.mp = p.np_hi > 1; h.metric = p.cos;
        if (!p.cos && !h.mp) {
            const bool small = a.Kpad <= FH_GATH_KMAX && gather_on;
            h.fast = small && a.fast_dist;
            h.gath = small && !a.fast_dist;
        } else if (!p.cos) {
            h.fast = !h.hash && a.fast_dist && a.pass_last;
        }
        if ((rc = launch_fused_hi_pass(s, p.nblk, h, a))) return rc;
    }
    return 0;
}

int fused_refine_passes(hipStream_t s, const FusedArgs& rf, const FusedPlan& p) {
    for (int i = 0; i < p.np_refine; i++) {
        const int c0 = i * FP_KMAX;
        FusedArgs r = rf;
        r.Ch = rf.Ch + (size_t)c0 * FU_D; r.Cl = rf.Cl + (size_t)c0 * FU_D; r.cnh = rf.cnh + c0;
        r.Kpad = std::min(FP_KMAX, rf.Kpad - c0);
        r.t0 = c0 / 32; r.pass_first = i == 0; r.pass_last = i == p.np_refine - 1;
        const int rc = launch_fused_refine_pass(s, (unsigned)p.nblk, p.cos, p.np_refine > 1, p.rows, r);
        if (rc) return rc;
    }
    return 0;
}

struct SideFork {
    lshkm_ctx c;
    bool open = false;
    int fork() {
        if (hipEventRecord(c->fork_ev, c->stream) != hipSuccess ||
            hipStreamWaitEvent(c->side_stream, c->fork_ev, 0) != hipSuccess)
            return kstatus("fused_assign (fork)");
        open = true;
        return 0;
    }
    int end_side() {
        if (c->timing) {
            if (hipEventRecord(c->tev[2], c->side_stream) != hipSuccess) return kstatus("fused_assign (timing)");
            c->tev_side = true;
        }
        if (hipEventRecord(c->join_ev, c->side_stream) != hipSuccess) return kstatus("fused_assign (join)");
        return 0;
    }
    int join() {
        if (!open) return 0;
        if (hipStreamWaitEvent(c->stream, c->join_ev, 0) != hipSuccess) return kstatus("fused_assign (join)");
        open = false;
        return 0;
    }
    ~SideFork() { if (open) (void)hipStreamSynchronize(c->side_stream); }
};

#ifdef LSHKM_PHASE_TIMING
struct PhaseReport {
    hipStream_t s;
    unsigned long long* d = nullptr;
    explicit PhaseReport(hipStream_t s_) : s(s_) {
        static unsigned long long* prof_d = nullptr;
        if (!prof_d) (void)hipMalloc(&prof_d, 64);
        (void)hipMemsetAsync(prof_d, 0, 64, s);
        d = prof_d;
    }
    ~PhaseReport() {
        unsigned long long v[6];
        (void)hipMemcpyAsync(v, d, 48, hipMemcpyDeviceToHost, s);
        (void)hipStreamSynchronize(s);
        fprintf(stderr, "PHASES %llu %llu %llu %llu %llu\n", v[0], v[1], v[2], v[3], v[4]);
    }
};
#endif

}

int fused_assign(lshkm_ctx ctx, const AssignRequest& q) {
    hipStream_t s = ctx->stream;
    const bool cosine = q.metric != LSHKM_METRIC_EUCLIDEAN;
    const ProjTable* pj = q.lsh ? &q.lsh->proj : nullptr;
    const FusedRoute route = fused_route(cosine, q.X.f64, q.d, q.K, pj != nullptr, pj ? pj->k : 0, pj ? pj->LK : 0,
                                         test_switch("LSHKM_FUSED_FORM", "chunked"));
    if (route.form == FusedForm::none || (pj && (q.lsh->metric != q.metric || !pj->mfma_ok))) {
        set_error("fused_assign: no fused form runs this shape (fused_route, fused_layout.h)");
        return LSHKM_ERR_ARG;
    }
    FusedShape sh;
    sh.N = q.N; sh.d = q.d; sh.K = q.K; sh.cosine = cosine; sh.rows = route.rows;
    sh.hash = pj != nullptr; sh.LK = pj ? pj->LK : 0;
    sh.fast = !cosine && sh.rows != 2 && !q.force_exact && ctx->dist_mode == LSHKM_DIST_CERTIFIED;
    sh.image32 = sh.fast || (!cosine && sh.rows != 2 && sh.Kpad() <= 256 && !test_switch("LSHKM_GATHER32", "0"));
    sh.own_tuples = sh.hash && !cosine && !q.tuples;
    const bool pwfix = sh.pwfix();
    int rc;
    FusedWorkspace w;
    if ((rc = fused_workspace(ctx, sh, w))) return rc;
    LSHKM_HIP(hipMemsetAsync(w.cnt, 0, FUSED_COUNTER_CLEAR, s));
    if (ctx->timing) LSHKM_HIP(hipEventRecord(ctx->tev[0], s));
    ctx->tev_side = false;
    if ((rc = launch_fused_prep(s, q.C, q.K, q.d, cosine ? 1 : 0, w))) return rc;
    const bool xprep = exact_pruned(q.X, q.d, q.K, q.metric);
    if (xprep && (rc = exact_listed_prep(ctx, q))) return rc;
    if (w.xn2 && (rc = launch_row_sumsq(s, q.X.d(), q.N, q.d, w.xn2))) return rc;

    const FusedArgs common = fused_common_args(ctx, q, sh, w);
    RowList exact_rows;
    exact_rows.p = w.list1; exact_rows.count = w.cnt + CNT_AMBIG; exact_rows.bound = q.N;
    RecList dist_fix[2];
    int ndist_fix = 0;
    SideFork side{ctx};
    if (q.N > 0 && route.form == FusedForm::chunked) {
        FusedArgs a = common;
        hash_outputs(a, q, sh, w);
        a.ambig = w.list1; a.ambig_count = w.cnt + CNT_AMBIG;
        if ((rc = launch_fused_chunked(s, sh.hash, a))) return rc;
    } else if (q.N > 0) {
        FusedPlan p;
        p.hash = sh.hash; p.cos = cosine; p.rows = sh.rows;
        int ncu = 0;
        if (device_cu_count(&ncu)) return LSHKM_ERR_HIP;
        p.nblk = fused_grid(q.N, ncu);
        p.seg_rows = fused_seg_rows(q.N, p.nblk);
        if (p.nblk > FUSED_MAX_SEGS) {
            set_error("fused_assign: more blocks than list segments");
            return LSHKM_ERR_ARG;
        }
        p.np_hi = (sh.Kpad() + FH_KMAX - 1) / FH_KMAX;
        p.np_refine = (sh.Kpad() + FP_KMAX - 1) / FP_KMAX;
        const RowList l1 = segmented(w.list1, w.cnt + CNT_REFINED, w.seg1, q, p);
        const RecList lh = segmented(w.hfix, w.cnt + CNT_HFIX, w.seg1, q, p);
        const RowList l2 = segmented(w.list2, w.cnt + CNT_AMBIG, w.seg2, q, p);
        FusedArgs seg = common;
        seg.seg_rows = p.seg_rows; seg.part = w.part;
#ifdef LSHKM_PHASE_TIMING
        PhaseReport report(s);
        seg.prof = report.d;
#endif
        FusedArgs hi = seg;
        hash_outputs(hi, q, sh, w);
        hi.ambig = l1.p; hi.ambig_count = l1.count; hi.seg_counts = l1.counts;
        if ((rc = fused_hi_passes(s, hi, p))) return rc;
        if (sh.hash) {
            const bool forked = ctx->side_init() == 0;
            if (forked && (rc = side.fork())) return rc;
            launch_hash_fixup(forked ? ctx->side_stream : s, lh, cosine, hi);
            if (forked && (rc = side.end_side())) return rc;
        }
        FusedArgs rf = seg;
        rf.list_in = l1.p; rf.list_counts = l1.counts; rf.list_seg_rows = l1.seg_rows;
        rf.ambig = l2.p; rf.ambig_count = l2.count; rf.seg_counts = l2.counts;
        rf.hfix = cosine ? w.hfix2 : hi.hfix; rf.hfix_count = cosine ? w.cnt + CNT_CFIX : hi.hfix_count;
        if ((rc = fused_refine_passes(s, rf, p))) return rc;
        if (cosine && (rc = side.join())) return rc;
        if ((rc = kstatus("fused_hi_kernel"))) return rc;
        exact_rows = l2;
        if (cosine || pwfix) dist_fix[ndist_fix++] = segmented(w.cfix, w.cnt + CNT_CFIX, w.seg3, q, p);
        if (cosine) dist_fix[ndist_fix++] = segmented(w.hfix2, w.cnt + CNT_CFIX, w.seg2, q, p);
    }
    if (ctx->timing) LSHKM_HIP(hipEventRecord(ctx->tev[1], s));
    if ((rc = exact_listed(ctx, q, exact_rows, !sh.fast, xprep, cosine ? w.xn2 : nullptr, cosine ? w.nbv : nullptr)))
        return rc;
    if ((rc = side.join())) return rc;
    {
        int di[3], n = 0;
        const unsigned long long* sp[3];
        di[n] = STAT_REFINED; sp[n++] = w.cnt + CNT_REFINED;
        if (sh.hash) { di[n] = STAT_HASH_FIX; sp[n++] = w.cnt + CNT_HFIX; }
        di[n] = STAT_ASSIGN_AMBIG; sp[n++] = w.cnt + CNT_AMBIG;
        if ((rc = launch_add_counters(s, ctx->stats.as<unsigned long long>(), n, di, sp))) return rc;
    }
    if (cosine || pwfix) {
        if ((rc = launch_cos_fix_seg(s, q, ndist_fix, dist_fix, cosine ? w.xn2 : nullptr, cosine ? w.nbv : nullptr)))
            return rc;
        if ((rc = launch_add_counter(s, ctx->stats.as<unsigned long long>() + (cosine ? STAT_COS_FIX : STAT_POW_FIX),
                                     w.cnt + CNT_CFIX)))
            return rc;
    }
    return 0;
}

}
```

### crypto-recommendation_amd/csrc/fused_args.h

```cpp
#pragma once
#include <hip/hip_runtime.h>
#include <stdint.h>

#include "fused_layout.h"
#include "tile.h"

namespace lshkm {

struct FusedArgs {
    const float* X;
    int64_t N;
    const _Float16* Ch;
    const _Float16* Cl;
    const float* cnh;
    const float* cbound;
    const double* C64;
    int Kpad;
    const _Float16* Vh;
    const _Float16* Vl;
    const double* PT;
    const float* tv;
    const double* pnorm;
    const double* v1;
    const int32_t* rv;
    float w;
    int L, k, LK, LKpad;
    int64_t nb;
    int32_t* tuples;
    int32_t* phi;
    int32_t* bucket;
    int32_t* assign;
    double* dist;
    int32_t* ambig;
    unsigned long long* ambig_count;
    unsigned long long* hfix;
    unsigned long long* hfix_count;
    unsigned long long* cfix;
    int32_t* cfix_counts;
    unsigned long long* cfix_count;
    unsigned long long* stats;
    int64_t seg_rows;
    int32_t* seg_counts;
    BucketDiv bdiv;
    const double* nbv;
    const double* xn2;
    float4* part;
    int t0, pass_first, pass_last;
    const int32_t* list_in;
    const int32_t* list_counts;
    int64_t list_seg_rows;
    unsigned long long* prof;
    const float* C32;
    const float* rn32;
    int fast_dist;
    const double* X64;
    int d, xvec;
    const double* Cd;
    int pw_lds;
};

}
```

### crypto-recommendation_amd/csrc/fused_impl.h

```cpp
#pragma once
#include <algorithm>
#include <cstdlib>
#include <cstring>
#include <cstdio>
#include <type_traits>

#include "common.h"
#include "kernels.h"
#include "hash_exact.h"
#include "exact.h"
#include "hash_tile.h"
#include "fused_args.h"

namespace lshkm {

static_assert(FU_D == FUSED_DIMS, "fused_layout.h states the kernels' dimension");
constexpr int FP_THREADS = 64 * FP_WAVES;
constexpr int FH_GATH_KMAX = 256;
constexpr int FP_HC_BYTES = 32 * (4 + 4 + 4 + 4);
constexpr int MFMA_PRIO = 1;
constexpr int CHAIN_PRIO = 2;

struct FusedWorkspace {
    int64_t list_cap = 0;
    _Float16 *Ch = nullptr, *Cl = nullptr;
    float *cbound = nullptr, *cnh = nullptr;
    double* nbv = nullptr;
    float *C32 = nullptr, *rn32 = nullptr;
    double* C64p = nullptr;
    int32_t *list1 = nullptr, *seg1 = nullptr;
    int32_t *list2 = nullptr, *seg2 = nullptr;
    int32_t* seg3 = nullptr;
    unsigned long long *hfix = nullptr, *cfix = nullptr, *hfix2 = nullptr;
    float4* part = nullptr;
    unsigned long long* cnt = nullptr;
    double* xn2 = nullptr;
    int32_t* tuples = nullptr;
};

int launch_fused_prep(hipStream_t s, const double* C, int K, int d, int metric, const FusedWorkspace& w);
int launch_row_sumsq(hipStream_t s, const double* X, int64_t N, int d, double* out);
int launch_fused_chunked(hipStream_t s, bool hash, const FusedArgs& a);
struct HiForm {
    bool hash = false;
    bool mp = false;
    int metric = 0;
    bool two_image = false;
    bool gath = false;
    int rows = 0;
    bool fast = false;
};
int launch_fused_hi_pass(hipStream_t s, unsigned nblk, const HiForm& f, FusedArgs a);
int launch_fused_refine_pass(hipStream_t s, unsigned nblk, int metric, bool mp, int rows, const FusedArgs& a);
void launch_hash_fixup(hipStream_t s, const RecList& l, bool cosine, FusedArgs a);
int launch_cos_fix_seg(hipStream_t s, const AssignJob& q, int nlists, const RecList* lists, const double* xn2,
                       const double* nbv);

#ifdef LSHKM_PHASE_TIMING
#define PT_DECL unsigned long long pt_acc[6] = {0, 0, 0, 0, 0, 0}; unsigned long long pt_t = __builtin_amdgcn_s_memtime();
#define PT_MARK(i) { const unsigned long long t_ = __builtin_amdgcn_s_memtime(); pt_acc[i] += t_ - pt_t; pt_t = t_; }
#define PT_FLUSH if (lane == 0) for (int i_ = 0; i_ < 6; i_++) atomicAdd(a.prof + i_, pt_acc[i_]);
#elif defined(LSHKM_ISA_MARK)
#define PT_DECL
#define PT_MARK(i) asm volatile(";PTMARK " #i);
#define PT_FLUSH
#else
#define PT_DECL
#define PT_MARK(i)
#define PT_FLUSH
#endif

__device__ inline double swap_halves(double v, int h) {
    const uint64_t b = (uint64_t)__double_as_longlong(v);
    const auto lo = __builtin_amdgcn_permlane32_swap((uint32_t)b, (uint32_t)b, false, false);
    const auto hi = __builtin_amdgcn_permlane32_swap((uint32_t)(b >> 32), (uint32_t)(b >> 32), false, false);
    const uint32_t l = h ? lo[0] : lo[1], u = h ? hi[0] : hi[1];
    return __longlong_as_double((long long)(((uint64_t)u << 32) | l));
}

__device__ inline float swap_halves_f(float v, int h) {
    const auto r = __builtin_amdgcn_permlane32_swap(__float_as_uint(v), __float_as_uint(v), false, false);
    return __uint_as_float(h ? r[0] : r[1]);
}

__device__ inline double take_from_lower(double v) {
    const uint64_t b = (uint64_t)__double_as_longlong(v);
    const uint32_t l = __builtin_amdgcn_permlane32_swap((uint32_t)b, (uint32_t)b, false, false)[0];
    const uint32_t u = __builtin_amdgcn_permlane32_swap((uint32_t)(b >> 32), (uint32_t)(b >> 32), false, false)[0];
    return __longlong_as_double((long long)(((uint64_t)u << 32) | l));
}
__device__ inline double take_from_upper(double v) {
    const uint64_t b = (uint64_t)__double_as_longlong(v);
    const uint32_t l = __builtin_amdgcn_permlane32_swap((uint32_t)b, (uint32_t)b, false, false)[1];
    const uint32_t u = __builtin_amdgcn_permlane32_swap((uint32_t)(b >> 32), (uint32_t)(b >> 32), false, false)[1];
    return __longlong_as_double((long long)(((uint64_t)u << 32) | l));
}

__device__ inline void tile_mfma(const _Float16* ah_row, const _Float16* al_row, const half8 (&bh)[8],
                                 const half8 (&bl)[8], floatx16& acc_hi, floatx16& acc_lo) {
#pragma unroll
    for (int r = 0; r < 16; r++) { acc_hi[r] = 0.f; acc_lo[r] = 0.f; }
#pragma unroll
    for (int s = 0; s < 8; s++) {
        const half8 ah = *reinterpret_cast<const half8*>(ah_row + 16 * s);
        const half8 al = *reinterpret_cast<const half8*>(al_row + 16 * s);
        acc_hi = __builtin_amdgcn_mfma_f32_32x32x16_f16(ah, bh[s], acc_hi, 0, 0, 0);
        acc_lo = __builtin_amdgcn_mfma_f32_32x32x16_f16(ah, bl[s], acc_lo, 0, 0, 0);
        acc_lo = __builtin_amdgcn_mfma_f32_32x32x16_f16(al, bh[s], acc_lo, 0, 0, 0);
    }
}

template <int ROWS>
__device__ inline void load_row_gen(const FusedArgs& a, int64_t rowc, int h, float (&dst)[64]) {
    const int64_t ro = rowc * (int64_t)a.d;
#pragma unroll
    for (int s = 0; s < 8; s++) {
        const int j0 = 16 * s + 8 * h;
        if (a.xvec && j0 + 8 <= a.d) {
            if constexpr (ROWS == 1) {
                const float4 p0 = *reinterpret_cast<const float4*>(a.X + ro + j0);
                const float4 p1 = *reinterpret_cast<const float4*>(a.X + ro + j0 + 4);
                dst[8 * s + 0] = p0.x; dst[8 * s + 1] = p0.y; dst[8 * s + 2] = p0.z; dst[8 * s + 3] = p0.w;
                dst[8 * s + 4] = p1.x; dst[8 * s + 5] = p1.y; dst[8 * s + 6] = p1.z; dst[8 * s + 7] = p1.w;
            } else {
#pragma unroll
                for (int j = 0; j < 4; j++) {
                    const double2 q = *reinterpret_cast<const double2*>(a.X64 + ro + j0 + 2 * j);
                    dst[8 * s + 2 * j] = (float)q.x;
                    dst[8 * s + 2 * j + 1] = (float)q.y;
                }
            }
        } else {
#pragma unroll
            for (int e = 0; e < 8; e++) {
                float v = 0.f;
                if (j0 + e < a.d) v = ROWS == 1 ? a.X[ro + j0 + e] : (float)a.X64[ro + j0 + e];
                dst[8 * s + e] = v;
            }
        }
    }
}
__device__ inline void load_x64_step(const FusedArgs& a, int64_t rowc, int st, int h, double2 (&o)[4]) {
    const int64_t ro = rowc * (int64_t)a.d;
    const int j0 = 16 * st + 8 * h;
    if (a.xvec && j0 + 8 <= a.d) {
#pragma unroll
        for (int j = 0; j < 4; j++) o[j] = *reinterpret_cast<const double2*>(a.X64 + ro + j0 + 2 * j);
    } else {
#pragma unroll
        for (int j = 0; j < 4; j++) {
            o[j] = make_double2(0.0, 0.0);
            if (j0 + 2 * j < a.d) o[j].x = a.X64[ro + j0 + 2 * j];
            if (j0 + 2 * j + 1 < a.d) o[j].y = a.X64[ro + j0 + 2 * j + 1];
        }
    }
}

__device__ inline float vmax3(float a, float b, float c) {
    float r;
    asm("v_max3_f32 %0, %1, %2, %3" : "=v"(r) : "v"(a), "v"(b), "v"(c));
    return r;
}
__device__ inline void tile_epilogue(const float (&sv)[16], float& m1, float& m2) {
#pragma unroll
    for (int r = 0; r < 16; r += 2) {
        const float ta = __uint_as_float((__float_as_uint(sv[r]) & ~0xFu) | (uint32_t)r);
        const float tb = __uint_as_float((__float_as_uint(sv[r + 1]) & ~0xFu) | (uint32_t)(r + 1));
        m2 = __builtin_amdgcn_fmed3f(m2, __builtin_amdgcn_fmed3f(m1, ta, tb), 0x1.fffffep127f);
        m1 = vmax3(m1, ta, tb);
    }
}

}
```

### crypto-recommendation_amd/csrc/fused_layout.h

```cpp
#pragma once
#include <algorithm>
#include <cstddef>
#include <cstdint>

namespace lshkm {

constexpr int FP_WAVES = 8;
constexpr int FH_WAVES_MIN = 8, FH_WAVES_MAX = 12;
constexpr int HMF_W = 4;
constexpr int HMF_BPC = 2;
constexpr int FP_KMAX = 256;
constexpr int FH_KMAX = 512;
constexpr int FUSED_DIMS = 128;

enum class FusedForm { none, hi, chunked };
struct FusedRoute {
    FusedForm form;
    int rows;
};
inline FusedRoute fused_route(bool cosine, bool f64, int d, int K, bool hash, int k, int LK, bool chunked_switch) {
    const bool hash_ok = !hash || (LK >= 1 && LK <= 32 && (!cosine || k == 4));
    if (!f64 && d == FUSED_DIMS && hash_ok) {
        if (!cosine) return {chunked_switch || (hash && k != 4) ? FusedForm::chunked : FusedForm::hi, 0};
        if (!chunked_switch) return {FusedForm::hi, 0};
    }
    if (!hash && d >= 1 && d <= FUSED_DIMS && K <= FH_KMAX) return {FusedForm::hi, f64 ? 2 : 1};
    return {FusedForm::none, 0};
}

constexpr int FUSED_MAX_SEGS = 1024;
constexpr int SEG_ROWS = 0, SEG_FIX = 1, SEG_SLOTS = 2;
constexpr size_t SEG_COUNTER_BYTES = (size_t)FUSED_MAX_SEGS * SEG_SLOTS * 4;
constexpr int64_t FUSED_LIST_SLACK = 32 + (int64_t)FUSED_MAX_SEGS * FH_WAVES_MAX * 32;
inline int64_t fused_list_cap(int64_t N) { return N + FUSED_LIST_SLACK; }
inline int64_t seg_rows_for(int64_t N, int nblk, int W) {
    const int64_t ntiles = (N + 31) / 32;
    return (int64_t)W * 32 * ((ntiles + (int64_t)nblk * W - 1) / ((int64_t)nblk * W));
}
inline int fused_grid(int64_t N, int ncu) {
    const int64_t want = ((N + 31) / 32 + FP_WAVES - 1) / FP_WAVES;
    return (int)std::max<int64_t>(1, std::min<int64_t>(ncu, want));
}
inline int64_t fused_seg_rows(int64_t N, int nblk) {
    int64_t r = 0;
    for (const int W : {FP_WAVES, FH_WAVES_MIN, FH_WAVES_MAX}) r = std::max(r, seg_rows_for(N, nblk, W));
    return r;
}
inline int hash_mfma_grid(int64_t N, int ncu) {
    const int64_t want = ((N + 31) / 32 + HMF_W - 1) / HMF_W;
    return (int)std::max<int64_t>(1, std::min<int64_t>((int64_t)ncu * HMF_BPC, want));
}
inline int64_t hash_mfma_seg_rows(int64_t N, int nblk) { return seg_rows_for(N, nblk, HMF_W); }

constexpr int64_t FUSED_PART_BYTES_PER_ROW = 32;
inline int64_t fused_part_bytes(int64_t N) {
    const int64_t tiles = std::max<int64_t>((N + 31) / 32, (fused_list_cap(N) + 31) / 32 + FUSED_MAX_SEGS);
    return tiles * 32 * FUSED_PART_BYTES_PER_ROW;
}

constexpr int CNT_AMBIG = 0;
constexpr int CNT_HFIX = 1;
constexpr int CNT_REFINED = 2;
constexpr int CNT_CFIX = 3;
constexpr size_t FUSED_COUNTER_BYTES = 64, FUSED_COUNTER_CLEAR = 32;

struct FusedShape {
    int64_t N = 0;
    int d = FUSED_DIMS, K = 0;
    bool cosine = false;
    int rows = 0;
    bool hash = false;
    int LK = 0;
    bool fast = false;
    bool image32 = false;
    bool own_tuples = false;
    int Kpad() const { return (K + 63) / 64 * 64; }
    bool pwfix() const { return !cosine && !fast; }
};
struct FusedLayout {
    static constexpr size_t NONE = ~(size_t)0;
    int64_t list_cap = 0;
    int64_t part_bytes = 0;
    size_t c16 = 0;
    size_t cconst = 0;
    size_t list1 = 0, list2 = 0;
    size_t seg1 = 0, seg2 = 0, seg3 = 0;
    size_t counter = 0;
    size_t fix = 0;
    size_t part = 0;
    size_t tuples = 0;
    size_t cf32 = 0;
    size_t c64p = 0;
    size_t xn2 = 0;
    size_t cl_off = 0, cnh_off = 0, nbv_off = 0, rn32_off = 0;
    size_t hfix_off = NONE, cfix_off = NONE, hfix2_off = NONE;
};
inline FusedLayout fused_layout(const FusedShape& q) {
    FusedLayout l;
    const size_t Kpad = (size_t)q.Kpad(), D = FUSED_DIMS;
    const bool pwfix = q.pwfix();
    l.list_cap = fused_list_cap(q.N);
    const size_t cap = (size_t)l.list_cap, rows1 = (size_t)std::max<int64_t>(q.N, 1);
    l.c16 = Kpad * D * 2 * 2;
    l.cl_off = Kpad * D * 2;
    l.cconst = (Kpad + 8) * 4 + Kpad * 8;
    l.cnh_off = 8 * 4;
    l.nbv_off = (Kpad + 8) * 4;
    l.list1 = l.list2 = cap * 4;
    l.seg1 = l.seg2 = SEG_COUNTER_BYTES;
    l.counter = FUSED_COUNTER_BYTES;
    size_t regions = 0;
    if (q.hash || q.cosine || pwfix) regions++;
    if (q.hash || q.cosine) l.hfix_off = 0;
    if (q.cosine || pwfix) l.cfix_off = regions++ * cap * 8;
    if (q.cosine) l.hfix2_off = regions++ * cap * 8;
    l.fix = regions * cap * 8;
    if (q.cosine || pwfix) l.seg3 = SEG_COUNTER_BYTES;
    if (Kpad > (size_t)FP_KMAX) l.part = (size_t)(l.part_bytes = fused_part_bytes(q.N));
    if (q.hash && !q.cosine && q.own_tuples) l.tuples = rows1 * (size_t)q.LK * 4;
    if (q.image32) {
        l.cf32 = Kpad * D * 4 + Kpad * 4;
        l.rn32_off = Kpad * D * 4;
    }
    if (q.rows != 0 && q.d != FUSED_DIMS) l.c64p = Kpad * D * 8;
    if (q.cosine && q.rows == 2) l.xn2 = rows1 * 8;
    return l;
}

struct HashLayout {
    int64_t list_cap = 0;
    size_t fix = 0, seg1 = 0, tuples = 0;
};
inline HashLayout hash_layout(int64_t N, int LK, bool own_tuples) {
    HashLayout l;
    l.list_cap = fused_list_cap(N);
    l.fix = (size_t)l.list_cap * 8;
    l.seg1 = SEG_COUNTER_BYTES;
    if (own_tuples) l.tuples = (size_t)N * (size_t)LK * 4;
    return l;
}

}
```

### crypto-recommendation_amd/csrc/fused_refine.hip

```cpp
#include "fused_impl.h"

namespace lshkm {

__device__ inline void split8p(const float* x, half8& hi, half8& lo) {
#pragma unroll
    for (int j = 0; j < 8; j += 2) {
        const half2v hp = {(_Float16)x[j], (_Float16)x[j + 1]};
        hi[j] = hp.x;
        hi[j + 1] = hp.y;
        const half2v lp = {(_Float16)resid_lo(x[j], hp), (_Float16)resid_hi(x[j + 1], hp)};
        lo[j] = lp.x;
        lo[j + 1] = lp.y;
    }
}

__device__ inline void tile_scores(const floatx16& acc_hi, const floatx16& acc_lo, const float* cn_tile_h,
                                   float (&sv)[16]) {
#pragma unroll
    for (int g = 0; g < 4; g++) {
        const float4 cn = *reinterpret_cast<const float4*>(cn_tile_h + 8 * g);
        const float2v h01 = {acc_hi[4 * g], acc_hi[4 * g + 1]}, l01 = {acc_lo[4 * g], acc_lo[4 * g + 1]};
        const float2v h23 = {acc_hi[4 * g + 2], acc_hi[4 * g + 3]}, l23 = {acc_lo[4 * g + 2], acc_lo[4 * g + 3]};
        const float2v c01 = {cn.x, cn.y}, c23 = {cn.z, cn.w};
        const float2v s01 = (h01 + l01) + c01, s23 = (h23 + l23) + c23;
        sv[4 * g] = s01.x; sv[4 * g + 1] = s01.y; sv[4 * g + 2] = s23.x; sv[4 * g + 3] = s23.y;
    }
}

__host__ __device__ constexpr int fp_lds_bytes(int Kpad) { return 16 + 2 * Kpad * FU_RS * 2 + Kpad * 4; }
static_assert(fp_lds_bytes(FP_KMAX) <= 160 * 1024, "refinement LDS image exceeds 160 KiB");

template <int MET, bool MP, int ROWS>
__global__ __launch_bounds__(FP_THREADS, 1) void fused_persistent_kernel(FusedArgs a) {
    extern __shared__ __attribute__((aligned(16))) char smem[];
    const int Kpad = a.Kpad;
    int* lcount = reinterpret_cast<int*>(smem);
    _Float16* lch = reinterpret_cast<_Float16*>(smem + 16);
    _Float16* lcl = lch + Kpad * FU_RS;
    float* lcn = reinterpret_cast<float*>(lcl + Kpad * FU_RS);

    constexpr int FP_CU = 4;
    for (int e0 = 0; e0 < Kpad * 16; e0 += FP_THREADS * FP_CU) {
        float4 vh[FP_CU], vl[FP_CU];
#pragma unroll
        for (int u = 0; u < FP_CU; u++) {
            const int e = e0 + u * FP_THREADS + (int)threadIdx.x < Kpad * 16 ? e0 + u * FP_THREADS + (int)threadIdx.x : 0;
            const int r = e >> 4, g = e & 15;
            vh[u] = *reinterpret_cast<const float4*>(a.Ch + (size_t)r * FU_D + g * 8);
            vl[u] = *reinterpret_cast<const float4*>(a.Cl + (size_t)r * FU_D + g * 8);
        }
#pragma unroll
        for (int u = 0; u < FP_CU; u++) {
            const int e = e0 + u * FP_THREADS + (int)threadIdx.x < Kpad * 16 ? e0 + u * FP_THREADS + (int)threadIdx.x : 0;
            const int r = e >> 4, g = e & 15;
            *reinterpret_cast<float4*>(lch + r * FU_RS + g * 8) = vh[u];
            *reinterpret_cast<float4*>(lcl + r * FU_RS + g * 8) = vl[u];
        }
    }
    for (int e = threadIdx.x; e < Kpad; e += FP_THREADS) lcn[e] = a.cnh[e];
    if (threadIdx.x < 2) lcount[threadIdx.x] = 0;
    int32_t* ambig_seg = a.ambig + (int64_t)blockIdx.x * a.seg_rows;
    unsigned long long* hfix_seg = a.hfix + (int64_t)blockIdx.x * a.seg_rows;
    __syncthreads();

    const int lane = threadIdx.x & 63, wave = threadIdx.x >> 6;
    const int col = lane & 31, h = lane >> 5;
    const float ecf = a.cbound[0], ebf = a.cbound[1], cmaxf = a.cbound[3];
    const bool c_ok = __float_as_uint(a.cbound[2]) == 0u;
    const _Float16* my_h = lch + col * FU_RS + 8 * h;
    const _Float16* my_l = lcl + col * FU_RS + 8 * h;
    const int ntile32 = Kpad >> 5;
    const int32_t* lrows = a.list_in + (int64_t)blockIdx.x * a.list_seg_rows;
    const int64_t lcnt = (int64_t)a.list_counts[SEG_SLOTS * blockIdx.x + SEG_ROWS];
    const int64_t ptile0 = (int64_t)blockIdx.x * ((a.list_seg_rows + 31) >> 5);

    PT_DECL
    for (int64_t tile = wave; tile < (lcnt + 31) >> 5; tile += FP_WAVES) {
        const bool valid = tile * 32 + col < lcnt;
        const int64_t row = lrows[valid ? tile * 32 + col : lcnt - 1];
        const int64_t ptile = ptile0 + tile;

        float xf[64];
        if constexpr (ROWS != 0) {
            load_row_gen<ROWS>(a, valid ? row : a.N - 1, h, xf);
        } else {
            load_row_b(a.X + (valid ? row : a.N - 1) * FU_D + 8 * h, xf);
        }
        half8 bh[8], bl[8];
        float2v n2a = {0.f, 0.f}, n2b = {0.f, 0.f};
#pragma unroll
        for (int s = 0; s < 8; s++) {
            split8p(xf + 8 * s, bh[s], bl[s]);
#pragma unroll
            for (int j = 0; j < 8; j += 4) {
                const float2v u = {xf[8 * s + j], xf[8 * s + j + 1]}, v = {xf[8 * s + j + 2], xf[8 * s + j + 3]};
                n2a = __builtin_elementwise_fma(u, u, n2a);
                n2b = __builtin_elementwise_fma(v, v, n2b);
            }
        }
        float xn2f = (n2a.x + n2a.y) + (n2b.x + n2b.y);
        xn2f += __shfl_xor(xn2f, 32);
        const double xn2 = (double)xn2f * (1.0 + 0x1p-16);
        const double nx = sqrt(xn2);
        const double x1 = FU_SQRT_D * nx;
        const bool x_ok = xn2f <= FU_RANGE * FU_RANGE;

        PT_MARK(0)
        PT_MARK(1)
        const float E = MET == 0
            ? (float)(nx * (double)ecf + (double)ebf + FU_A2 * x1 + 0x1p-41 * xn2 +
                      0x1p-18 * (nx * (double)cmaxf + 0.5 * (double)cmaxf * (double)cmaxf) +
                      (ROWS == 2 ? 0x1p-24 * nx * (double)cmaxf : 0.0)) * (1.f + 0x1p-20f) + 1e-30f
            : (float)(nx * (double)ecf + (double)ebf + FU_A2 * x1 + 0x1p-41 * xn2 +
                      0x1p-18 * nx * (double)cmaxf + 0x1p-43 * nx) * (1.f + 0x1p-20f) + 1e-30f;
        float m1 = -__builtin_inff(), m2 = -__builtin_inff();
        int t1 = 0;
        if (MP && !a.pass_first) {
            const float4 st = a.part[ptile * 64 + lane];
            m1 = st.x; m2 = st.y; t1 = __float_as_int(st.z);
        }
        const int tg0 = MP ? a.t0 : 0;
        __builtin_amdgcn_s_setprio(MFMA_PRIO);
#pragma unroll 1
        for (int t = 0; t < ntile32; t++) {
            const float m1_prev = m1;
            float sv[16];
            floatx16 acc_hi, acc_lo;
            tile_mfma(my_h + t * 32 * FU_RS, my_l + t * 32 * FU_RS, bh, bl, acc_hi, acc_lo);
            tile_scores(acc_hi, acc_lo, lcn + t * 32 + 4 * h, sv);
            tile_epilogue(sv, m1, m2);
            t1 = m1 != m1_prev ? t + tg0 : t1;
        }
        __builtin_amdgcn_s_setprio(0);
        if (MP && !a.pass_last) {
            a.part[ptile * 64 + lane] = make_float4(m1, m2, __int_as_float(t1), 0.f);
            continue;
        }
        const uint32_t l1 = __float_as_uint(m1) & 0xFu;
        const int i1 = t1 * 32 + 8 * (int)(l1 >> 2) + 4 * h + (int)(l1 & 3u);
        const float om1 = __shfl_xor(m1, 32), om2 = __shfl_xor(m2, 32);
        const int oi1 = __shfl_xor(i1, 32);
        const float M2 = fmaxf(fmaxf(m2, om2), fminf(m1, om1));
        const int I1 = (om1 > m1 || (om1 == m1 && oi1 < i1)) ? oi1 : i1;
        const float M1 = fmaxf(m1, om1);
        const bool cert = x_ok && c_ok && ((double)M2 < (double)M1 - 2.0 * (double)E);

        PT_MARK(2)
        if constexpr (MET == 1) {
            bool fix = false;
            if (h == 1 && valid && cert) {
                a.assign[row] = I1;
                double v;
                bool okc;
                if constexpr (ROWS == 1) okc = cosine_fast_nb(a.X + row * a.d, a.Cd + (size_t)I1 * a.d, a.d, a.nbv[I1], v);
                else if constexpr (ROWS == 2) okc = cosine_fast_nb(a.X64 + row * a.d, a.Cd + (size_t)I1 * a.d, a.d, a.nbv[I1], v);
                else okc = cosine_fast_nb(a.X + row * FU_D, a.C64 + (size_t)I1 * FU_D, FU_D, a.nbv[I1], v);
                if (okc) a.dist[row] = v;
                else fix = true;
            }
            const unsigned long long fb = __ballot(fix);
            if (fb) {
                const int leader = __builtin_ctzll(fb);
                int base = 0;
                if (lane == leader) base = atomicAdd(lcount + 1, __popcll(fb));
                base = __shfl(base, leader);
                if (fix) hfix_seg[base + __popcll(fb & ((1ull << lane) - 1ull))] = (unsigned long long)row;
            }
        } else {
            const double* crow = a.C64 + (size_t)I1 * FU_D + 8 * h;
            double acc = 0.0;
            double2 cbuf[4];
            double2 xnext[4];
            const int64_t rowc = valid ? row : a.N - 1;
            if constexpr (ROWS == 2) load_x64_step(a, rowc, 0, h, xnext);
#pragma unroll
            for (int j = 0; j < 4; j++) cbuf[j] = *reinterpret_cast<const double2*>(crow + 2 * j);
#pragma unroll
            for (int s = 0; s < 8; s++) {
                double sq[8];
                double2 cur[4];
#pragma unroll
                for (int j = 0; j < 4; j++) cur[j] = cbuf[j];
                if (s + 1 < 8) {
#pragma unroll
                    for (int j = 0; j < 4; j++) cbuf[j] = *reinterpret_cast<const double2*>(crow + 16 * (s + 1) + 2 * j);
                }
                double2 xcur[4];
                if constexpr (ROWS == 2) {
#pragma unroll
                    for (int j = 0; j < 4; j++) xcur[j] = xnext[j];
                    if (s + 1 < 8) load_x64_step(a, rowc, s + 1, h, xnext);
                } else {
#pragma unroll
                    for (int j = 0; j < 4; j++) xcur[j] = make_double2((double)xf[8 * s + 2 * j], (double)xf[8 * s + 2 * j + 1]);
                }
#pragma unroll
                for (int j = 0; j < 4; j++) {
                    const double2 cc = cur[j];
                    const double d0 = __dsub_rn(xcur[j].x, cc.x);
                    const double d1 = __dsub_rn(xcur[j].y, cc.y);
                    sq[2 * j] = a.fast_dist ? __dmul_rn(d0, d0) : gp_sq(d0);
                    sq[2 * j + 1] = a.fast_dist ? __dmul_rn(d1, d1) : gp_sq(d1);
                }
                if (h == 0) {
#pragma unroll
                    for (int j = 0; j < 8; j++) acc = __dadd_rn(acc, sq[j]);
                }
                acc = take_from_lower(acc);
                if (h == 1) {
#pragma unroll
                    for (int j = 0; j < 8; j++) acc = __dadd_rn(acc, sq[j]);
                }
                acc = take_from_upper(acc);
            }
            if (h == 1 && valid && cert) {
                a.assign[row] = I1;
                a.dist[row] = sqrt(acc);
            }
        }
        PT_MARK(3)
        const bool amb = valid && !cert;
        const unsigned long long amask = __ballot(amb && h == 1);
        if (h == 1 && valid) {
            if (!cert) {
                int base = 0;
                const int leader = __builtin_ctzll(amask);
                if (lane == leader) base = atomicAdd(lcount, __popcll(amask));
                base = __shfl(base, leader);
                const int rank = __popcll(amask & ((1ull << lane) - 1ull));
                ambig_seg[base + rank] = (int32_t)row;
            }
        }
        PT_MARK(4)
    }
    PT_FLUSH
    __syncthreads();
    if (threadIdx.x < 2 && (!MP || (threadIdx.x == 0 ? a.pass_last != 0 : (MET == 1 && a.pass_last)))) {
        const int c = lcount[threadIdx.x];
        a.seg_counts[SEG_SLOTS * blockIdx.x + threadIdx.x] = c;
        if (c) atomicAdd(threadIdx.x == 0 ? a.ambig_count : a.hfix_count, (unsigned long long)c);
    }
}

template <int MET, bool MP, int ROWS>
static void refine_launch(hipStream_t s, unsigned nblk, const FusedArgs& a) {
    hipLaunchKernelGGL((fused_persistent_kernel<MET, MP, ROWS>), dim3(nblk), dim3(FP_THREADS),
                       (size_t)fp_lds_bytes(a.Kpad), s, a);
}
template <int MET, bool MP>
static void refine_rows(hipStream_t s, unsigned nblk, int rows, const FusedArgs& a) {
    if (rows == 0) refine_launch<MET, MP, 0>(s, nblk, a);
    else if (rows == 1) refine_launch<MET, MP, 1>(s, nblk, a);
    else refine_launch<MET, MP, 2>(s, nblk, a);
}

int launch_fused_refine_pass(hipStream_t s, unsigned nblk, int metric, bool mp, int rows, const FusedArgs& a) {
    if (metric < 0 || metric > 1 || rows < 0 || rows > 2 || a.Kpad > FP_KMAX) {
        set_error("launch_fused_refine_pass: no kernel for this metric / row kind / slice");
        return -1;
    }
    if (metric == 1) mp ? refine_rows<1, true>(s, nblk, rows, a) : refine_rows<1, false>(s, nblk, rows, a);
    else mp ? refine_rows<0, true>(s, nblk, rows, a) : refine_rows<0, false>(s, nblk, rows, a);
    return 0;
}

}
```

### crypto-recommendation_amd/csrc/index.h

```cpp
#pragma once
#include <algorithm>
#include <hip/hip_runtime.h>
#include <stdint.h>

#include <vector>

#include "kernels.h"

namespace lshkm {

struct Buf {
    void* p = nullptr;
    size_t cap = 0;
    Buf() = default;
    Buf(const Buf&) = delete;
    Buf& operator=(const Buf&) = delete;
    ~Buf();
    int reserve(size_t bytes);
    template <typename T> T* as() const { return reinterpret_cast<T*>(p); }
};

struct ProjTable {
    int metric = 0, d = 0, L = 0, k = 0, LK = 0, LKpad = 0;
    float w = 0.f;
    Buf PT_d, t_d, pn_d, r_d;
    bool fused_ok = false;
    bool mfma_ok = false;
    Buf vh_d, vl_d, v1_d;
    std::vector<float> hV;
    int upload(hipStream_t s, int metric, int d, int L, int k, float w, const float* V, const float* t,
               const int32_t* r, const double* R);
    HashParams params(int64_t nb) const;
    HashMfmaParams mfma_params(int64_t nb) const;
};

}

struct lshkm_ctx_s;
struct lshkm_lsh_s;
namespace lshkm {
int hash_rows(lshkm_ctx_s* ctx, int mode, Pts X, int64_t N, const ProjTable& pj, int64_t nb, int32_t* out_h,
              int32_t* out_phi, int32_t* out_bucket, int32_t* mm, bool* h16 = nullptr);
bool exact_pruned(Pts X, int d, int K, int metric);
int exact_listed_prep(lshkm_ctx_s* ctx, const AssignJob& q);
int exact_listed(lshkm_ctx_s* ctx, const AssignJob& q, const RowList& l, bool exact_dist, bool prepped,
                 const double* xn2, const double* nbv);
struct AssignRequest : AssignJob {
    const ::lshkm_lsh_s* lsh = nullptr;
    int32_t *tuples = nullptr, *phi = nullptr, *bucket = nullptr;
    bool force_exact = false;
};
int fused_assign(lshkm_ctx_s* ctx, const AssignRequest& q);

}

struct lshkm_ctx_s {
    int device = 0;
    int dist_mode = 0;
    hipStream_t stream = nullptr;
    hipStream_t own_stream = nullptr;
    lshkm::Buf stats;
    lshkm::Buf ws_c32, ws_cconst, ws_ambig, ws_counter, ws_src, ws_hfix, ws_ct, ws_seg, ws_tuples, ws_part;
    lshkm::Buf ws_cf32, ws_c64p;
    lshkm::Buf ws_ambig2, ws_seg2;
    lshkm::Buf ws_seg3;
    lshkm::Buf ws_xn2;
    lshkm::Buf ws[16];
    lshkm::Buf ws_range[12];
    lshkm::Buf ws_long;
    lshkm::Buf ws_km_seg;
    lshkm::Buf ws_scan;
    lshkm::Buf ws_pam[5];
    lshkm::Buf ws_call[10];
    uint64_t ws_epoch = 0;
    bool timing = false;
    hipEvent_t tev[3] = {nullptr, nullptr, nullptr};
    bool tev_side = false;
    hipStream_t side_stream = nullptr;
    hipEvent_t fork_ev = nullptr, join_ev = nullptr;
    int side_init() {
        if (side_stream) return 0;
        if (hipStreamCreateWithFlags(&side_stream, hipStreamNonBlocking) != hipSuccess) return -2;
        if (hipEventCreateWithFlags(&fork_ev, hipEventDisableTiming) != hipSuccess ||
            hipEventCreateWithFlags(&join_ev, hipEventDisableTiming) != hipSuccess)
            return -2;
        return 0;
    }
    static constexpr int PIN_SLOTS = 4;
    void* pin_buf[PIN_SLOTS] = {};
    size_t pin_cap[PIN_SLOTS] = {};
    hipEvent_t pin_ev[PIN_SLOTS] = {};
    bool pin_used[PIN_SLOTS] = {};
    int pin_cur = -1;
    void* pinned = nullptr;
    hipEvent_t pinned_ev = nullptr;
    std::vector<int32_t> src_cache;
    void* src_cache_dev = nullptr;
    size_t src_cache_cap = 0;
    int pin_stage(size_t bytes) {
        const int i = (pin_cur + 1) % PIN_SLOTS;
        if (!pin_ev[i] && hipEventCreateWithFlags(&pin_ev[i], hipEventDisableTiming) != hipSuccess) return -2;
        if (pin_used[i]) (void)hipEventSynchronize(pin_ev[i]);
        if (bytes > pin_cap[i]) {
            if (pin_buf[i]) (void)hipHostFree(pin_buf[i]);
            pin_buf[i] = nullptr; pin_cap[i] = 0;
            if (hipHostMalloc(&pin_buf[i], bytes, hipHostMallocDefault) != hipSuccess) return -3;
            pin_cap[i] = bytes;
        }
        pin_cur = i;
        pin_used[i] = true;
        pinned = pin_buf[i];
        pinned_ev = pin_ev[i];
        return 0;
    }
    void* rb_buf = nullptr;
    size_t rb_cap = 0;
    void* ub_buf = nullptr;
    size_t ub_cap = 0;
    hipEvent_t ub_ev = nullptr;
    bool ub_pending = false;
    static int pin_grow(void*& b, size_t& cap, size_t bytes) {
        if (bytes <= cap) return 0;
        if (b) (void)hipHostFree(b);
        b = nullptr;
        cap = 0;
        const size_t nb = std::max<size_t>(bytes, 64 << 10);
        if (hipHostMalloc(&b, nb, hipHostMallocDefault) != hipSuccess) return -3;
        cap = nb;
        return 0;
    }
    ~lshkm_ctx_s() {
        if (rb_buf) (void)hipHostFree(rb_buf);
        if (ub_ev) {
            if (ub_pending) (void)hipEventSynchronize(ub_ev);
            (void)hipEventDestroy(ub_ev);
        }
        if (ub_buf) (void)hipHostFree(ub_buf);
        for (hipEvent_t& e : tev)
            if (e) (void)hipEventDestroy(e);
        if (side_stream) (void)hipStreamSynchronize(side_stream), (void)hipStreamDestroy(side_stream);
        if (fork_ev) (void)hipEventDestroy(fork_ev);
        if (join_ev) (void)hipEventDestroy(join_ev);
        for (int i = 0; i < PIN_SLOTS; i++) {
            if (pin_ev[i]) (void)hipEventSynchronize(pin_ev[i]), (void)hipEventDestroy(pin_ev[i]);
            if (pin_buf[i]) (void)hipHostFree(pin_buf[i]);
        }
    }
};

namespace lshkm {
struct D2H { void* dst; const void* src; size_t bytes; };
struct H2D { void* dst; const void* src; size_t bytes; };
int d2h_batch(lshkm_ctx_s* ctx, const D2H* r, int n);
int h2d_batch(lshkm_ctx_s* ctx, const H2D* r, int n);
}

struct lshkm_lsh_s {
    lshkm_ctx_s* ctx = nullptr;
    int metric = 0;
    int64_t nb = 0;
    lshkm::ProjTable proj;
    int built = 0;
    int64_t N = 0;
    lshkm::Buf tuples, bucket, row_ptr, idx;
    lshkm::Buf mt0;
    bool mt0_valid = false;
    bool q_valid = false;
    uint64_t q_epoch = 0;
    const void* q_Q = nullptr;
    bool q_f64 = false;
    const void* q_alias = nullptr;
    const int64_t* q_out_ptr = nullptr;
    int64_t q_nq = 0, q_total = 0;
    int q_filtered = 0;
};

struct lshkm_cube_s {
    lshkm_ctx_s* ctx = nullptr;
    int metric = 0;
    int k = 0;
    lshkm::ProjTable proj;
    int32_t hmin = 0, hspan = 0;
    lshkm::Buf memo, memo2, first_row;
    lshkm::Buf rng_d;
    lshkm::Buf mm, cnt;
    int built = 0;
    int64_t N = 0;
    lshkm::Buf vertex, row_ptr, idx;
};
```

### crypto-recommendation_amd/csrc/kernels.h

```cpp
#pragma once
#include <climits>
#include <hip/hip_runtime.h>
#include <stdint.h>

#include "fused_layout.h"
#include "recom_layout.h"

namespace lshkm {

struct Pts {
    const void* p = nullptr;
    bool f64 = false;
    Pts() = default;
    Pts(const float* x) : p(x), f64(false) {}
    Pts(const double* x) : p(x), f64(true) {}
    const float* f() const { return static_cast<const float*>(p); }
    const double* d() const { return static_cast<const double*>(p); }
    size_t esize() const { return f64 ? 8 : 4; }
    Pts row(int64_t r, int d) const {
        Pts q = *this;
        q.p = static_cast<const char*>(p) + (size_t)r * d * esize();
        return q;
    }
};

struct AssignJob {
    Pts X;
    int64_t N = 0;
    int d = 0;
    const double* C = nullptr;
    int K = 0;
    int metric = 0;
    int32_t* assign = nullptr;
    double* dist = nullptr;
};

template <typename T>
struct DevList {
    static constexpr int slot = sizeof(T) == 4 ? SEG_ROWS : SEG_FIX;
    T* p = nullptr;
    unsigned long long* count = nullptr;
    int64_t bound = 0;
    int32_t* counts = nullptr;
    int64_t seg_rows = 0;
    int nseg = 0;
    const int32_t* seg_counts() const { return nseg > 0 ? counts : nullptr; }
};
using RowList = DevList<int32_t>;
using RecList = DevList<unsigned long long>;

enum HashMode {
    HM_LSH_EUCLID = 0,
    HM_LSH_COSINE = 1,
    HM_CUBE_EUCLID_H = 2,
    HM_CUBE_COSINE = 3,
};

struct HashParams {
    const double* PT;
    const float* t;
    const double* pnorm;
    const int32_t* r;
    float w;
    int d, L, k, LK, LKpad;
    int64_t nb;
};
int hash_fb(int LK);
int hash_lkpad(int LK);

int launch_proj_hash(hipStream_t s, int mode, Pts X, int64_t N, const HashParams& p,
                     int32_t* out_h, int32_t* out_phi, int32_t* out_bucket,
                     unsigned long long* stats);

struct HashMfmaParams {
    const _Float16* Vh;
    const _Float16* Vl;
    const float* t;
    const double* pnorm;
    const double* v1;
    const int32_t* r;
    const double* PT;
    float w;
    int d, L, k, LK, LKpad;
    int64_t nb;
};
int launch_hash_mfma(hipStream_t s, int mode, const float* X, int64_t N, const HashMfmaParams& p, int32_t* out_h,
                     int32_t* out_phi, int32_t* out_bucket, int32_t* mm, const RecList& list,
                     unsigned long long* stats, int h16 = 0);

int assign_dp(int d);
int launch_centroid_prep(hipStream_t s, const double* C, int K, int Kpad, int d, int DP, int metric, bool xf64,
                         float* C32, float* cconst);
int launch_assign_mfma(hipStream_t s, Pts X, int64_t N, int d, int DP, const double* C, int K,
                       int Kpad, int metric, const float* C32, const float* cconst, int32_t* assign, double* dist,
                       int32_t* ambig, unsigned long long* ambig_count);
int launch_cos_fix(hipStream_t s, Pts X, int64_t N, int d, const double* C, const int32_t* rows,
                   const unsigned long long* count, const int32_t* assign, double* dist);
int launch_assign_exact(hipStream_t s, const AssignJob& q, const RowList& l, const double* xn2 = nullptr,
                        const double* nbv = nullptr);
int launch_assign_exact_list(hipStream_t s, const AssignJob& q, double* CT, const RowList& l);
int launch_assign_pruned_list(hipStream_t s, const AssignJob& q, float* ws, const RowList& l, int exact_dist,
                              bool prepped);
int launch_assign_pruned_prep(hipStream_t s, bool xf64, int d, const double* C, int K, float* ws, int metric);
int launch_assign_override(hipStream_t s, const int32_t* src_rows, int K, int64_t N, int32_t* assign,
                           double* dist);

int launch_add_counter(hipStream_t s, unsigned long long* dst, const unsigned long long* src);
int launch_add_counters(hipStream_t s, unsigned long long* stats, int n, const int* dst_idx,
                        const unsigned long long* const* src);

size_t sort_scratch_bytes(int64_t N, int64_t range, int T = 1);
int pow_contract_check();

int sort_pairs_small(hipStream_t s, const int32_t* keys, const int32_t* vals, int64_t n, int32_t* keys_out,
                     int32_t* vals_out, const unsigned int* n_dev = nullptr);
int stable_sort_by_key(hipStream_t s, const int32_t* keys, int64_t kstride, const int32_t* vals, int64_t N,
                       int64_t range, int32_t* keys_out, int32_t* vals_out, void* scratch);
int launch_csr_bounds(hipStream_t s, const int32_t* sorted_keys, int64_t N, int64_t nb, int64_t* row_ptr, int T = 1);
int stable_sort_by_key_batched(hipStream_t s, const int32_t* keys, int64_t kstride, int64_t key_ts, const int32_t* vals,
                               int64_t val_ts, int T, int64_t N, int64_t range, int32_t* keys_out, int32_t* vals_out,
                               void* scratch);

size_t scan_ws_bytes(int64_t M);
int launch_scan_i64(hipStream_t s, const int64_t* a, int64_t M, int64_t* out, int64_t* scratch = nullptr);
int launch_lsh_query(hipStream_t s, const int32_t* qbucket, const int32_t* qtuple, const int32_t* alias, int64_t nq,
                     int L, int k, int64_t nb, int filtered, int64_t N, const int32_t* tuples, const int32_t* bucket,
                     const int64_t* row_ptr, const int32_t* idx, int64_t* sizes, int64_t* cand_off,
                     int32_t* klist, int64_t* kcount, int64_t* qsz, int64_t* out_ptr, int32_t* out, int phase,
                     int64_t* scan_ws = nullptr, const int32_t* mt0 = nullptr);
int launch_lsh_gather_t0(hipStream_t s, const int32_t* tuples, const int32_t* idx, int64_t N, int L, int k, int32_t* mt0);
int launch_cube_query(hipStream_t s, const int32_t* qvert, int64_t nq, const int32_t* masks, int S,
                      const int64_t* row_ptr, const int32_t* idx, int64_t* sizes, int64_t* slot_off,
                      int64_t* out_ptr, int32_t* out, int64_t* scan_ws = nullptr);

int launch_h_minmax(hipStream_t s, const int32_t* h, int64_t n, int32_t* mm_dev);
int launch_coin_first(hipStream_t s, const void* h, bool h16, int64_t N, int k, int32_t hmin, int32_t hspan,
                      const int32_t* memo, int32_t* first_row);
int launch_coin_collect(hipStream_t s, int32_t* first_row, int64_t total, int k, int32_t hspan, int32_t* keys,
                        int32_t* vals, unsigned int* count);
int launch_coin_draw(hipStream_t s, const int32_t* sorted_vals, const unsigned int* count, int32_t hmin, int32_t hspan,
                     int32_t* memo, uint32_t* state);
int launch_coin_vertex(hipStream_t s, const void* h, bool h16, int64_t N, int k, int32_t hmin, int32_t hspan,
                       const int32_t* memo, int32_t* vertex);
int launch_memo_rehome(hipStream_t s, const int32_t* old_memo, int32_t old_min, int32_t old_span, int32_t* new_memo,
                       int32_t new_min, int32_t new_span, int k);
int launch_memo_scatter(hipStream_t s, const int32_t* off, const int32_t* bit, int64_t n, int32_t* memo);

int launch_km_chain(hipStream_t s, Pts X, int d, const int32_t* rows, const int64_t* crow, int K,
                    double* sums, int64_t* counts, const double* carry = nullptr,
                    const int64_t* carry_counts = nullptr);
size_t km_seg_ws_bytes(int64_t M, int K, int d);
constexpr size_t KM_SEG_WS_CAP = (size_t)8 << 30;
int launch_km_sums_seg(hipStream_t s, Pts X, int d, const int32_t* rows, const int64_t* crow, int K, int64_t M,
                       double* sums, int64_t* counts, const double* carry, const int64_t* carry_counts, void* ws,
                       const int* flag = nullptr);
size_t km_fx_ws_bytes(int K, int d);
int launch_km_sums_fx(hipStream_t s, Pts X, int d, const int32_t* rows, const int64_t* crow, int K, int64_t M,
                      double* sums, int64_t* counts, const double* carry, const int64_t* carry_counts, void* ws,
                      unsigned long long* stat = nullptr, void* seg_ws = nullptr);
size_t km_shard_ws_bytes(int64_t M, int K, int d);
int launch_km_shard_begin(hipStream_t s, Pts X, int d, const int32_t* rows, const int64_t* crow, int K, int64_t M,
                          double* sums, double* asum, int32_t* qt, int64_t* counts, void* ws);
int launch_km_shard_certify(hipStream_t s, const double* gathered, int world, int rank, const double* asum,
                            const int32_t* qt, const int64_t* counts, int K, int d, double* sums_out, double* start,
                            int* flag, uint8_t* mask, unsigned long long* nflag);
int launch_km_shard_prepare(hipStream_t s, Pts X, int d, const int32_t* rows, const int64_t* crow, int K, int64_t M,
                            const double* start, const int* flag, const uint8_t* mask, void* ws);
int launch_km_shard_chain(hipStream_t s, Pts X, int d, const int32_t* rows, const int64_t* crow, int K, int64_t M,
                          const int* flag, const uint8_t* mask, const double* carry, void* ws, double* sums);
size_t seg_columns_ws_bytes(int64_t n, int K, int m);
int launch_seg_iota(hipStream_t s, int32_t* iota, int64_t n);
int launch_seg_columns(hipStream_t s, const double* V, int64_t n, int K, int m, const int32_t* iota,
                       const int64_t* crow, const double* carry, double* out, void* ws);
int launch_grid_bits(hipStream_t s, Pts X, int64_t n, int* qt);
bool grid_exact_squares(const int* qt_host);
int launch_km_finalize(hipStream_t s, const double* sums, const int64_t* counts, int K, int d, const double* C_old,
                       int metric, double min_dist, double* C_new, int* moved);

size_t kmeans_pp_ws_bytes(int64_t N);
int launch_kmeans_pp(hipStream_t s, Pts X, int64_t N, int d, int K, int metric, const double* canon,
                     int32_t* chosen, void* ws, unsigned long long* stats);
size_t kpp_shard_out_offset(int64_t n);
int launch_kpp_shard_dist(hipStream_t s, Pts X, int64_t n, int d, int metric, const void* crow, int it, void* ws);
int launch_kpp_shard_units(hipStream_t s, int64_t n, unsigned long long gmax_bits, double start, void* ws);
int launch_kpp_shard_chain(hipStream_t s, int64_t n, double s_in, void* ws, unsigned long long* stats);
int launch_kpp_shard_pick(hipStream_t s, int64_t n, double rd, int owns_row0, void* ws);

int launch_rc_norms(hipStream_t s, const double* X, int64_t N, int d, double* xa);
struct RecomJob {
    Pts X;
    const double* x_mean;
    int64_t N;
    int d;
    const int64_t* crow;
    const int32_t* crows;
    int K;
    Pts U;
    const double* u_mean;
    int64_t nq;
    const int32_t* ucl;
    const int64_t* unk_ptr;
    const int32_t* unk_idx;
};
struct RecomCarry {
    double *main, *abs;
    int64_t* cnt;
};
struct RecomOut {
    double* pred;
    int32_t* pidx;
    int n_top;
    int32_t* out;
};
int launch_rc_cluster_top_n(hipStream_t s, const RecomJob& j, double* scratch, const RcWaveScratch& ws,
                            const RecomOut& o, unsigned long long* soft_count);
struct RcGroups {
    const int32_t* ioff;
    int ngroups;
    int64_t nitems;
    const int32_t* gcl;
    const int32_t* gptr;
    const int32_t* gusr;
    void* items;
    int64_t nusers;
    void* users;
};
struct RcTermsOut {
    const int64_t *soff, *toff;
    int64_t total;
    double *sims, *terms;
};
int launch_rc_terms(hipStream_t s, const RecomJob& j, const RcTermsOut& t, char* map, const RcGroups& groups,
                    unsigned long long* soft_count);
struct RcLong {
    const RcLongUser* tab;
    int64_t nlong, rows;
    int D;
    const int64_t* crow;
    double *V, *carry, *sums;
    int32_t* iota;
    void* ws;
};
int launch_rc_chain_terms(hipStream_t s, const RecomJob& j, const RcTermsOut& t, const RecomCarry& in,
                          const RecomCarry& out, double* pred, int64_t long_min);
int launch_rc_long(hipStream_t s, const RcTermsOut& t, const RecomCarry& in, const double* u_mean,
                   const RecomCarry& out, double* pred, const RcLong& lng);
int launch_rc_top(hipStream_t s, const RecomJob& j, const int64_t* soff, const int64_t* carry_cnt, const RecomOut& o);
int launch_rc_shard_sims(hipStream_t s, const RecomJob& j, const int64_t* soff, double* sims,
                         unsigned long long* soft_count);
int launch_rc_shard_chain(hipStream_t s, const RecomJob& j, const int64_t* soff, const double* sims,
                          const RecomCarry& in, const RecomCarry& out, const RecomOut& o);
int launch_rc_p_closest(hipStream_t s, const double* X, const double* xa, int d, const double* U, int64_t nq,
                        const int64_t* cand_ptr, const int32_t* cand_idx, int P, double* sim, double* key,
                        int32_t* pos, int32_t* out_idx, double* out_sim, int32_t* out_cnt, int32_t* replay,
                        unsigned int* replay_count);
int launch_rc_top_n(hipStream_t s, const double* X, const double* x_mean, int d, const double* u_mean, int64_t nq,
                    const int64_t* unk_ptr, const int32_t* unk_idx, const int32_t* nb_idx, const double* nb_sim,
                    const int32_t* nb_cnt, int P, int n_top, double* pred, int32_t* pidx, int32_t* out);

int launch_cv_gather(hipStream_t s, const double* X, const double* x_mean, const int32_t* rows, int64_t M, int d,
                     double* W, double* w_mean);
int launch_cv_hide(hipStream_t s, const double* X, const double* x_mean, const int32_t* rows, int64_t M, int d,
                   const int64_t* unk_ptr, const int32_t* unk_idx, const int32_t* draw, double* H, double* h_mean,
                   int32_t* hide_idx, double* old);
int launch_cv_exclude(hipStream_t s, const int64_t* in_ptr, const int32_t* in_idx, int64_t nq, int32_t lo, int32_t hi,
                      int64_t* cnt, int32_t* run_a, int32_t* run_b, int64_t* out_ptr, int32_t* out_idx);
int launch_cv_predict(hipStream_t s, const double* X, const double* x_mean, int d, const double* u_mean, int64_t nq,
                      int64_t entries, const int64_t* unk_ptr, const int32_t* unk_idx, const int32_t* nb_idx,
                      const double* nb_sim, const int32_t* nb_cnt, int P, double* pred);
int launch_cv_fold_sum(hipStream_t s, int64_t F, const int32_t* hide_idx, const double* old, const double* pred,
                       const int64_t* nb_ptr, double* err, double* k_sum_out, int64_t* cnt_out, bool carry);

int launch_range_radius(hipStream_t s, const double* C, int K, int d, int metric, double* r0,
                        unsigned long long* tmp);
int launch_range_pairs(hipStream_t s, const int64_t* comb_ptr, const int32_t* comb_idx, int K, int32_t* rows,
                       int32_t* cents);
int launch_range_init(hipStream_t s, int64_t N, int32_t* assign, double* dist);
int launch_range_pass(hipStream_t s, Pts X, int d, const double* C, int K, int metric, const int32_t* key,
                      const int64_t* vptr, const int32_t* cents, double* cache, int8_t* cached, int64_t N,
                      const double* r0, int64_t pass, int32_t* assign, double* dist, unsigned long long* count);
int launch_range_unassigned(hipStream_t s, const int32_t* assign, int64_t N, int32_t* list,
                            unsigned long long* count);
int launch_range_gather(hipStream_t s, Pts X, int d, const int32_t* list, int64_t M, void* Xr);
int launch_range_scatter(hipStream_t s, const int32_t* list, int64_t M, const int32_t* ar, const double* dr,
                         int32_t* assign, double* dist);

int launch_sil_near(hipStream_t s, const double* C, int K, int d, int metric, int32_t* near);
int launch_sil_points(hipStream_t s, Pts X, int d, int metric, const int32_t* rows, const int64_t* crow,
                      const int32_t* assign, const int32_t* near, int64_t N, double* s_out, bool exsq = false);
int launch_sil_sum(hipStream_t s, const double* sv, const int32_t* rows, const int64_t* crow, int K, int64_t N,
                   double* raw, double* out);

int launch_pam_check_assign(hipStream_t s, const int32_t* assign, int64_t N, int K, int* bad);
constexpr int PAM_SCREEN_DMAX = 128;
constexpr int PAM_SCREEN_COLS = 128;
int launch_pam_prep(hipStream_t s, Pts X, int d, const int32_t* rows, const int32_t* assign, int64_t N, double* n2,
                    float* rho, int* cbad, unsigned long long* cmax);
int launch_pam_screen(hipStream_t s, Pts X, int d, const int32_t* rows, const int64_t* crow, const int2* items,
                      int64_t nitems, const double* n2, const float* rho, double* St, double* Et,
                      const unsigned long long* cmax, unsigned long long* Sfix, unsigned long long* Efix);
int launch_pam_mark(hipStream_t s, const int64_t* crow, int K, const int32_t* screen, const int* cbad,
                    const double* St, const double* Et, const unsigned long long* cmax,
                    const unsigned long long* Sfix, const unsigned long long* Efix, uint8_t* flag, int64_t* cnt,
                    unsigned long long* stats);
int launch_pam_compact(hipStream_t s, const int64_t* crow, int K, const uint8_t* flag, const int64_t* coff,
                       int32_t* cand);
int launch_pam_exact(hipStream_t s, Pts X, int d, int metric, const int32_t* rows, const int64_t* crow,
                     const int32_t* assign, const int32_t* cand, const int64_t* m_dev, int64_t N, double* sums,
                     bool exsq);
int launch_pam_select(hipStream_t s, const int32_t* rows, const int32_t* cand, const int64_t* coff, int K,
                      const double* sums, int32_t* med, double* csum);
int launch_pam_gather(hipStream_t s, Pts X, int d, const int32_t* med, int K, const double* C_old, double* C_new);

int launch_synth(hipStream_t s, uint64_t seed, int64_t row0, int64_t rows, int d, float* X, int kind = 0);

}
```

### crypto-recommendation_amd/lshkm.py

```python
import ctypes as C
import os
import re

import numpy as np

_HERE = os.path.dirname(os.path.abspath(__file__))
LIB_PATH = os.environ.get("LSHKM_LIB") or os.path.join(_HERE, "liblshkm.so")
HEADER = os.path.join(os.path.dirname(_HERE), "include", "lshkm.h")

EUCLIDEAN, COSINE = 0, 1
STAT_HASH_EXACT, STAT_ASSIGN_AMBIG, STAT_COS_FIX, STAT_REFINED, STAT_HASH_FIX, STAT_REC_SOFT = 0, 1, 4, 5, 6, 7
STAT_POW_FIX = 8
STAT_KM_SEQ = 9
STAT_PAM_SCREENED, STAT_PAM_EXACT = 10, 11
_METRIC = {"euclidean": EUCLIDEAN, "cosine": COSINE, EUCLIDEAN: EUCLIDEAN, COSINE: COSINE}
DIST_CERTIFIED, DIST_EXACT = 0, 1
_DIST = {"certified": DIST_CERTIFIED, "default": DIST_CERTIFIED, "exact": DIST_EXACT,
         DIST_CERTIFIED: DIST_CERTIFIED, DIST_EXACT: DIST_EXACT}

_lib = None


class LshkmError(RuntimeError):
    pass


def pow_selfcheck():
    m, t = C.c_int64(), C.c_int64()
    _ck(lib().lshkm_pow_selfcheck(C.byref(m), C.byref(t)))
    return m.value, t.value


def declared_symbols():
    with open(HEADER) as f:
        txt = f.read()
    return sorted(set(re.findall(r"^(?:int|const char\*)\s+(lshkm_\w+)\(", txt, re.M)))


def lib():
    global _lib
    if _lib is None:
        if not os.path.exists(LIB_PATH):
            raise LshkmError(f"{LIB_PATH} not built: run __graft_entry__.build() (no CPU fallback exists)")
        L = C.CDLL(LIB_PATH)
        vp, i64, i32, u64, f32, f64 = C.c_void_p, C.c_int64, C.c_int, C.c_uint64, C.c_float, C.c_double
        sigs = {
            "lshkm_last_error": (C.c_char_p, []),
            "lshkm_version": (C.c_char_p, []),
            "lshkm_pow2": (i32, [vp, vp, i64, vp]),
            "lshkm_pow_selfcheck": (i32, [C.POINTER(i64), C.POINTER(i64)]),
            "lshkm_ctx_create": (i32, [i32, C.POINTER(vp)]),
            "lshkm_ctx_set_stream": (i32, [vp, vp]),
            "lshkm_ctx_set_dist_mode": (i32, [vp, i32]),
            "lshkm_ctx_get_dist_mode": (i32, [vp, C.POINTER(i32)]),
            "lshkm_ctx_sync": (i32, [vp]),
            "lshkm_ctx_destroy": (i32, [vp]),
            "lshkm_dev_alloc": (i32, [vp, i64, C.POINTER(vp)]),
            "lshkm_dev_free": (i32, [vp, vp]),
            "lshkm_memcpy_h2d": (i32, [vp, vp, vp, i64]),
            "lshkm_memcpy_d2h": (i32, [vp, vp, vp, i64]),
            "lshkm_get_stat": (i32, [vp, i32, C.POINTER(i64)]),
            "lshkm_reset_stats": (i32, [vp]),
            "lshkm_ctx_enable_timing": (i32, [vp, i32]),
            "lshkm_last_kernel_ms": (i32, [vp, C.POINTER(C.c_float)]),
            "lshkm_params_lsh_euclidean": (i32, [u64, i32, i32, i32, f32, vp, vp, vp, C.POINTER(C.c_uint32)]),
            "lshkm_params_lsh_cosine": (i32, [u64, i32, i32, i32, vp, C.POINTER(C.c_uint32)]),
            "lshkm_params_cube_euclidean": (i32, [u64, i32, i32, f32, vp, vp, C.POINTER(C.c_uint32)]),
            "lshkm_params_cube_cosine": (i32, [u64, i32, i32, vp, C.POINTER(C.c_uint32)]),
            "lshkm_lsh_create": (i32, [vp, i32, i32, i32, i32, i64, f32, vp, vp, vp, vp, C.POINTER(vp)]),
            "lshkm_lsh_destroy": (i32, [vp]),
            "lshkm_lsh_hash": (i32, [vp, vp, i64, vp, vp, vp]),
            "lshkm_lsh_build": (i32, [vp, vp, i64]),
            "lshkm_lsh_get_buckets": (i32, [vp, i32, vp, vp]),
            "lshkm_lsh_device_views": (i32, [vp, C.POINTER(vp), C.POINTER(vp), C.POINTER(vp), C.POINTER(vp)]),
            "lshkm_lsh_query": (i32, [vp, vp, i64, vp, i32, vp, vp, i64, C.POINTER(i64)]),
            "lshkm_cube_create": (i32, [vp, i32, i32, i32, f32, vp, vp, vp, C.c_uint32, C.POINTER(vp)]),
            "lshkm_cube_destroy": (i32, [vp]),
            "lshkm_cube_build": (i32, [vp, vp, i64]),
            "lshkm_cube_vertices": (i32, [vp, vp, i64, vp]),
            "lshkm_cube_get_buckets": (i32, [vp, vp, vp]),
            "lshkm_cube_query": (i32, [vp, vp, i64, i32, vp, vp, i64, C.POINTER(i64)]),
            "lshkm_cube_get_memo": (i32, [vp, vp, vp, vp, i64, C.POINTER(i64), C.POINTER(C.c_uint32)]),
            "lshkm_cube_unseen": (i32, [vp, vp, i64, vp, vp, vp, i64, C.POINTER(i64)]),
            "lshkm_cube_import_coins": (i32, [vp, vp, vp, vp, i64, C.c_uint32]),
            "lshkm_coins_draw": (i32, [C.POINTER(C.c_uint32), vp, i64, vp]),
            "lshkm_lloyd_assign": (i32, [vp, vp, i64, i32, vp, i32, i32, vp, vp, vp]),
            "lshkm_range_assign": (i32, [vp, vp, i64, i32, vp, i32, i32, vp, vp, vp, vp, vp, vp, C.POINTER(i32)]),
            "lshkm_silhouette": (i32, [vp, vp, i64, i32, vp, vp, i32, i32, vp, vp]),
            "lshkm_vectors_read": (i32, [C.c_char_p, C.c_char, i32, i32, C.POINTER(vp)]),
            "lshkm_vectors_info": (i32, [vp, C.POINTER(i64), C.POINTER(i32), C.POINTER(i64), C.POINTER(i32),
                                         C.POINTER(i32), C.POINTER(i32)]),
            "lshkm_vectors_values": (i32, [vp, vp, vp]),
            "lshkm_vectors_ids": (i32, [vp, vp, vp]),
            "lshkm_vectors_meta": (i32, [vp, i32, C.c_char_p, i64, C.POINTER(i64)]),
            "lshkm_vectors_free": (i32, [vp]),
            "lshkm_config_value": (i32, [C.c_char_p, C.c_char_p, C.c_char_p, i64, C.POINTER(i32)]),
            "lshkm_config_load": (i32, [C.c_char_p, vp]),
            "lshkm_hash_assign": (i32, [vp, vp, i64, vp, i32, vp, vp, vp, vp, vp, vp]),
            "lshkm_hash_assign_metric": (i32, [vp, vp, i64, vp, i32, i32, vp, vp, vp, vp, vp, vp]),
            "lshkm_kmeans_update": (i32, [vp, vp, i64, i32, vp, vp, i32, i32, f64, vp, vp, C.POINTER(i32)]),
            "lshkm_kmeans_partial": (i32, [vp, vp, i64, i32, vp, i32, vp, vp]),
            "lshkm_kmeans_partial_carry": (i32, [vp, vp, i64, i32, vp, i32, vp, vp, vp, vp]),
            "lshkm_kmeans_partial_csr": (i32, [vp, vp, i64, i32, vp, vp, i32, vp, vp]),
            "lshkm_kmeans_finalize": (i32, [vp, vp, vp, i32, i32, vp, i32, f64, vp, C.POINTER(i32)]),
            "lshkm_kmeans_shard_begin": (i32, [vp, vp, i64, i32, vp, vp, i32, vp, vp, vp, vp]),
            "lshkm_kmeans_shard_certify": (i32, [vp, i32, i32, i32, i32, vp, vp, vp, vp, vp, vp, vp, vp,
                                                 C.POINTER(i64)]),
            "lshkm_kmeans_shard_ws_bytes": (i32, [i64, i32, i32, C.POINTER(i64)]),
            "lshkm_kmeans_shard_prepare": (i32, [vp, vp, i64, i32, vp, vp, i32, vp, vp, vp, vp, i64]),
            "lshkm_kmeans_shard_chain": (i32, [vp, vp, i64, i32, vp, vp, i32, vp, vp, vp, vp, i64, vp]),
            "lshkm_kmeans_pp": (i32, [vp, vp, i64, i32, i32, i32, u64, vp]),
            "lshkm_kpp_draws": (i32, [u64, i64, i32, C.POINTER(i64), vp]),
            "lshkm_kpp_shard_ws_bytes": (i32, [i64, C.POINTER(i64)]),
            "lshkm_kpp_shard_dist": (i32, [vp, vp, i64, i32, i32, vp, i32, vp, i64, C.POINTER(u64), C.POINTER(f64)]),
            "lshkm_kpp_shard_units": (i32, [vp, i64, u64, f64, vp, i64]),
            "lshkm_kpp_shard_chain": (i32, [vp, i64, f64, vp, i64, C.POINTER(f64)]),
            "lshkm_kpp_shard_pick": (i32, [vp, i64, f64, i32, vp, i64, C.POINTER(i64)]),
            "lshkm_rand_selection": (i32, [u64, i64, i32, vp]),
            "lshkm_p_closest": (i32, [vp, vp, i64, i32, vp, i64, vp, vp, i32, vp, vp, vp]),
            "lshkm_top_n_recom": (i32, [vp, vp, vp, i64, i32, vp, i64, vp, vp, vp, vp, vp, i32, i32, vp]),
            "lshkm_cluster_top_n": (i32, [vp, vp, vp, i64, i32, vp, vp, i32, vp, vp, i64, vp, vp, vp, i32, vp]),
            "lshkm_cluster_sims": (i32, [vp, vp, i64, i32, vp, vp, i32, vp, i64, vp, vp, vp, vp, i64,
                                         C.POINTER(i64)]),
            "lshkm_cluster_chain": (i32, [vp, vp, vp, i64, i32, vp, vp, i32, i64, vp, vp, vp, vp, vp, vp, vp, vp,
                                          vp, vp, vp, vp, i32, vp]),
            "lshkm_cluster_terms": (i32, [vp, vp, vp, i64, i32, vp, vp, i32, vp, i64, vp, vp, vp, vp, vp, vp, vp,
                                          i64, i64, C.POINTER(i64), C.POINTER(i64)]),
            "lshkm_cluster_chain_terms": (i32, [vp, i64, vp, vp, vp, vp, vp, vp, vp, vp, vp, vp, vp, vp, vp, i32,
                                                vp]),
            "lshkm_cluster_terms_supported": (i32, [i32, i32]),
            "lshkm_cv_split10": (i32, [u64, i64, vp]),
            "lshkm_cv_draws": (i32, [vp, i64, i64, vp]),
            "lshkm_cv_hide": (i32, [vp, vp, vp, i64, i32, vp, vp, vp, vp, vp, vp, vp]),
            "lshkm_cv_exclude": (i32, [vp, vp, vp, i64, i32, i32, vp, vp]),
            "lshkm_cv_fold_sum": (i32, [vp, i64, vp, vp, vp, vp, vp, vp, vp]),
            "lshkm_predicted_scores": (i32, [vp, vp, vp, i64, i32, vp, i64, vp, vp, vp, vp, vp, i32, vp]),
            "lshkm_lsh_validate10": (i32, [vp, vp, vp, i64, i32, vp, vp, i32, i32, i32, i32, f32, i32, u64, u64, vp, vp,
                                           C.POINTER(f64), vp, vp, vp]),
            "lshkm_synth": (i32, [vp, u64, i64, i64, i32, vp]),
            "lshkm_synth_normal": (i32, [vp, u64, i64, i64, i32, vp]),
            "lshkm_clusters": (i32, [vp, vp, i64, i32, vp, vp]),
            "lshkm_pam_update": (i32, [vp, vp, i64, i32, vp, i32, i32, vp, vp, vp, vp, vp, C.POINTER(i32)]),
        }
        for name, (res, args) in sigs.items():
            for nm in (name, name + "_f64"):
                if not hasattr(L, nm):
                    continue
                fn = getattr(L, nm)
                fn.restype = res
                fn.argtypes = args
        _lib = L
    return _lib


def _ck(rc):
    if rc != 0:
        raise LshkmError(f"lshkm error {rc}: {lib().lshkm_last_error().decode()}")


def _np_ptr(a):
    return None if a is None else a.ctypes.data_as(C.c_void_p)


def _t_ptr(t):
    return None if t is None else C.c_void_p(t.data_ptr())


def _fn(name, X):
    dt = str(X.dtype)
    if dt.endswith("float32"):
        return getattr(lib(), name)
    if dt.endswith("float64"):
        return getattr(lib(), name + "_f64")
    raise LshkmError(f"{name}: rows must be float32 or float64, got {dt}")


def params_lsh_euclidean(seed, L, k, d, w):
    V = np.empty((L, k, d), np.float32); t = np.empty((L, k), np.float32); r = np.empty((L, k), np.int32)
    st = C.c_uint32()
    _ck(lib().lshkm_params_lsh_euclidean(seed, L, k, d, float(np.float32(w)), _np_ptr(V), _np_ptr(t), _np_ptr(r), C.byref(st)))
    return V, t, r, st.value


def params_lsh_cosine(seed, L, k, d):
    R = np.empty((L, k, d), np.float64); st = C.c_uint32()
    _ck(lib().lshkm_params_lsh_cosine(seed, L, k, d, _np_ptr(R), C.byref(st)))
    return R, st.value


def params_cube_euclidean(seed, k, d, w):
    V = np.empty((k, d), np.float32); t = np.empty((k,), np.float32); st = C.c_uint32()
    _ck(lib().lshkm_params_cube_euclidean(seed, k, d, float(np.float32(w)), _np_ptr(V), _np_ptr(t), C.byref(st)))
    return V, t, st.value


def params_cube_cosine(seed, k, d):
    R = np.empty((k, d), np.float64); st = C.c_uint32()
    _ck(lib().lshkm_params_cube_cosine(seed, k, d, _np_ptr(R), C.byref(st)))
    return R, st.value


class Context:
    def __init__(self, device=0, use_torch_stream=True):
        import torch
        self.torch = torch
        self.device = device
        self.dev = torch.device("cuda", device)
        h = C.c_void_p()
        _ck(lib().lshkm_ctx_create(device, C.byref(h)))
        self.h = h
        if use_torch_stream:
            _ck(lib().lshkm_ctx_set_stream(self.h, C.c_void_p(torch.cuda.current_stream(self.dev).cuda_stream)))

    def set_dist_mode(self, mode):
        _ck(lib().lshkm_ctx_set_dist_mode(self.h, _DIST[mode]))

    def pow2(self, x):
        x = x.contiguous()
        assert x.dtype == self.torch.float64 and x.device.type == "cuda"
        out = self.torch.empty_like(x)
        _ck(lib().lshkm_pow2(self.h, C.c_void_p(x.data_ptr()), x.numel(), C.c_void_p(out.data_ptr())))
        return out

    def dist_mode(self):
        m = C.c_int()
        _ck(lib().lshkm_ctx_get_dist_mode(self.h, C.byref(m)))
        return "exact" if m.value == DIST_EXACT else "certified"

    def sync(self):
        _ck(lib().lshkm_ctx_sync(self.h))

    def stat(self, which):
        v = C.c_int64()
        _ck(lib().lshkm_get_stat(self.h, which, C.byref(v)))
        return v.value

    def reset_stats(self):
        _ck(lib().lshkm_reset_stats(self.h))

    def close(self):
        if self.h:
            lib().lshkm_ctx_destroy(self.h)
            self.h = None

    def __del__(self):
        try:
            self.close()
        except Exception:
            pass

    def empty(self, shape, dtype):
        return self.torch.empty(shape, dtype=dtype, device=self.dev)

    def synth(self, seed, rows, d, row0=0, kind="grid"):
        X = self.empty((rows, d), self.torch.float32)
        fn = {"grid": lib().lshkm_synth, "normal": lib().lshkm_synth_normal}[kind]
        _ck(fn(self.h, seed, row0, rows, d, _t_ptr(X)))
        return X


class LSH:

    def __init__(self, ctx, metric, d, k, L, nb=0, w=0.0, V=None, t=None, r=None, R=None):
        self.ctx, self.metric, self.d, self.k, self.L = ctx, _METRIC[metric], d, k, L
        self.nb = nb if self.metric == EUCLIDEAN else (1 << k)
        self.w = float(np.float32(w))
        keep = [np.ascontiguousarray(a, dt) if a is not None else None
                for a, dt in ((V, np.float32), (t, np.float32), (r, np.int32), (R, np.float64))]
        h = C.c_void_p()
        _ck(lib().lshkm_lsh_create(ctx.h, self.metric, d, k, L, self.nb, self.w, *[_np_ptr(a) for a in keep], C.byref(h)))
        self.h = h
        self.N = 0

    def close(self):
        if self.h:
            lib().lshkm_lsh_destroy(self.h)
            self.h = None
        self.ctx = None

    def __del__(self):
        try:
            self.close()
        except Exception:
            pass

    def hash(self, X, tuples=True, phi=True, bucket=True):
        torch = self.ctx.torch
        N = X.shape[0]
        tu = self.ctx.empty((N, self.L, self.k), torch.int32) if (tuples and self.metric == EUCLIDEAN) else None
        ph = self.ctx.empty((N, self.L), torch.int32) if phi else None
        bu = self.ctx.empty((N, self.L), torch.int32) if bucket else None
        _ck(_fn("lshkm_lsh_hash", X)(self.h, _t_ptr(X), N, _t_ptr(tu), _t_ptr(ph), _t_ptr(bu)))
        return tu, ph, bu

    def build(self, X):
        _ck(_fn("lshkm_lsh_build", X)(self.h, _t_ptr(X), X.shape[0]))
        self.N = X.shape[0]

    def buckets(self, table):
        rp = np.empty(self.nb + 1, np.int64); idx = np.empty(max(self.N, 1), np.int32)
        _ck(lib().lshkm_lsh_get_buckets(self.h, table, _np_ptr(rp), _np_ptr(idx)))
        return rp, idx[:self.N]

    def query(self, Q, filtered=True, alias_rows=None, device=False):
        torch = self.ctx.torch
        nq = Q.shape[0]
        ptr = self.ctx.empty((nq + 1,), torch.int64)
        total = C.c_int64()
        _ck(_fn("lshkm_lsh_query", Q)(self.h, _t_ptr(Q), nq, _t_ptr(alias_rows), int(filtered), _t_ptr(ptr), None, 0,
                                  C.byref(total)))
        out = self.ctx.empty((max(total.value, 1),), torch.int32)
        _ck(_fn("lshkm_lsh_query", Q)(self.h, _t_ptr(Q), nq, _t_ptr(alias_rows), int(filtered), _t_ptr(ptr), _t_ptr(out),
                                  total.value, C.byref(total)))
        self.ctx.sync()
        if device:
            return ptr, out[:total.value]
        return ptr.cpu().numpy(), out[:total.value].cpu().numpy()
# ... 641 lines not shown
```

Measured before the change: 4.997 billion point hash+assign ops/s.

## Track top-3 scores in fused refine and resolve two-candidate ambiguous rows cheaply

The fused refine kernel now tracks the top three scores per row. When the third-best score is separated by more than the error bound, the row is sent to a new pair list holding only its two candidate centroids instead of the full ambiguous-row list. The pruned exact pass handles pair groups by computing exact distances to just those two candidates, skipping the full pruned scan over all K centroids. The trade-off is extra register and ALU work in the refine epilogue, plus a new workspace region and counter.

New measurement: 4.999 billion point hash+assign ops/s, median of 6. No clear change (+0.0%).

```diff
diff --git a/crypto-recommendation_amd/csrc/api.cpp b/crypto-recommendation_amd/csrc/api.cpp
--- a/crypto-recommendation_amd/csrc/api.cpp
+++ b/crypto-recommendation_amd/csrc/api.cpp
@@ -614,14 +614,20 @@
                                      q.metric == LSHKM_METRIC_EUCLIDEAN ? 0 : 1);
 }
 
-int lshkm::exact_listed(lshkm_ctx ctx, const AssignJob& q, const RowList& l, bool exact_dist, bool prepped,
-                        const double* xn2, const double* nbv) {
+int lshkm::exact_listed(lshkm_ctx ctx, const AssignJob& q, const RowList& l, const RecList& pairs, bool exact_dist,
+                        bool prepped, const double* xn2, const double* nbv) {
     const bool prune = exact_pruned(q.X, q.d, q.K, q.metric);
+    if (pairs.p && (!prune || q.metric != LSHKM_METRIC_EUCLIDEAN || l.nseg <= 0 || pairs.nseg != l.nseg ||
+                    pairs.seg_rows != l.seg_rows || pairs.counts != l.counts)) {
+        set_error("exact_listed: a pair list needs the pruned euclidean pass and list segments like the rows'");
+        return LSHKM_ERR_ARG;
+    }
     if (!prune && (q.metric != LSHKM_METRIC_EUCLIDEAN || (l.nseg == 0 && q.d > 256)))
         return launch_assign_exact(ctx->stream, q, l, xn2, nbv);
     int rc;
     if ((rc = ctx->ws_ct.reserve(exact_ct_bytes(q)))) return rc;
-    if (prune) return launch_assign_pruned_list(ctx->stream, q, (float*)ctx->ws_ct.p, l, exact_dist ? 1 : 0, prepped);
+    if (prune)
+        return launch_assign_pruned_list(ctx->stream, q, (float*)ctx->ws_ct.p, l, pairs.p, exact_dist ? 1 : 0, prepped);
     return launch_assign_exact_list(ctx->stream, q, (double*)ctx->ws_ct.p, l);
 }
 
@@ -641,7 +647,7 @@
                                  q.assign, q.dist, (int32_t*)ctx->ws_ambig.p, cnt))) return rc;
     RowList l;
     l.p = (int32_t*)ctx->ws_ambig.p; l.count = cnt; l.bound = N;
-    if ((rc = exact_listed(ctx, q, l, true, false, nullptr, nullptr))) return rc;
+    if ((rc = exact_listed(ctx, q, l, RecList{}, true, false, nullptr, nullptr))) return rc;
     if (q.metric != LSHKM_METRIC_EUCLIDEAN &&
         ((rc = launch_cos_fix(s, q.X, N, q.d, q.C, (const int32_t*)ctx->ws_ambig.p + N, cnt + 1, q.assign, q.dist)) ||
          (rc = launch_add_counter(s, (unsigned long long*)ctx->stats.p + STAT_COS_FIX, cnt + 1)))) return rc;
diff --git a/crypto-recommendation_amd/csrc/assign.hip b/crypto-recommendation_amd/csrc/assign.hip
--- a/crypto-recommendation_amd/csrc/assign.hip
+++ b/crypto-recommendation_amd/csrc/assign.hip
@@ -595,6 +595,41 @@
     best = group_min<G>(v);
 }
 
+template <int R, typename TX>
+__device__ inline void pruned_pair_group(const TX* __restrict__ X, int d, const double* __restrict__ C, int K,
+                                         const unsigned long long* __restrict__ recs, int nr, TX (*xs)[XB_DMAX],
+                                         int lane, bool exact_dist, int32_t* __restrict__ assign,
+                                         double* __restrict__ dist) {
+    constexpr int RL = 64 / R, XU = 16;
+    const int r = lane / RL, k = lane % RL;
+    const unsigned long long rec = recs[min(r, nr - 1)];
+    const int64_t row = (int64_t)(rec & 0xFFFFFFFFull);
+    const int cand = k == 0 ? (int)((rec >> 32) & 0xFFFFu) : (int)(rec >> 48);
+    const int c = r < nr && k < 2 && cand < K ? cand : -1;
+    for (int j0 = 0; j0 < d; j0 += XU * RL) {
+        TX xv[XU];
+#pragma unroll
+        for (int u = 0; u < XU; u++) {
+            const int j = j0 + k + RL * u;
+            xv[u] = j < d ? X[row * d + j] : TX(0);
+        }
+#pragma unroll
+        for (int u = 0; u < XU; u++) {
+            const int j = j0 + k + RL * u;
+            if (j < d) xs[r][j] = xv[u];
+        }
+    }
+    wave_sync();
+    double best = 0.0;
+    int bi = -1;
+    pruned_pick_euclid<RL>(xs[r], C, d, c, exact_dist, best, bi);
+    if (k == 0 && bi >= 0) {
+        assign[row] = bi;
+        dist[row] = best;
+    }
+    wave_sync();
+}
+
 __global__ void exact_prep_kernel(const double* __restrict__ C, int K, int Kpad, int d, int xf64,
                                   float* __restrict__ CT32, float* __restrict__ cconst, int metric) {
     const int c = blockIdx.x, lane = threadIdx.x;
@@ -645,16 +680,21 @@
     const TX* __restrict__ X, int d, const double* __restrict__ C, const float* __restrict__ CT32,
     const float* __restrict__ cconst, int K, int Kpad, const int32_t* __restrict__ rows,
     const unsigned long long* __restrict__ row_count, int64_t max_rows, int32_t* __restrict__ assign,
-    double* __restrict__ dist, const int32_t* __restrict__ seg_counts, int64_t seg_rows, int exact_dist) {
+    double* __restrict__ dist, const int32_t* __restrict__ seg_counts, int64_t seg_rows, int exact_dist,
+    const unsigned long long* __restrict__ pairs) {
     constexpr int RL = 64 / R;
     __shared__ TX xs[XP_WAVES][R][XB_DMAX];
     const int lane = threadIdx.x & 63, wave = threadIdx.x >> 6;
-    int64_t total, g0, gstride;
+    int64_t total, g0, gstride, ptotal = 0;
     if (seg_counts) {
         const int nseg = gridDim.x / XP_SPLIT;
         const int seg = blockIdx.x % nseg, part = blockIdx.x / nseg;
         rows += (int64_t)seg * seg_rows;
         total = seg_counts[SEG_SLOTS * seg + SEG_ROWS];
+        if (MET == 0 && pairs) {
+            pairs += (int64_t)seg * seg_rows;
+            ptotal = min((int64_t)seg_counts[SEG_SLOTS * seg + SEG_FIX], seg_rows);
+        }
         g0 = (int64_t)part * XP_WAVES + wave;
         gstride = (int64_t)XP_SPLIT * XP_WAVES;
     } else {
@@ -664,8 +704,16 @@
         gstride = (int64_t)gridDim.x * XP_WAVES;
     }
     const float* chunkc = cconst + Kpad;
-    const int64_t ngroups = (total + R - 1) / R;
-    for (int64_t g = g0; g < ngroups; g += gstride) {
+    const int64_t ngroups = (total + R - 1) / R, npgroups = (ptotal + R - 1) / R;
+    for (int64_t g = g0; g < ngroups + npgroups; g += gstride) {
+        if constexpr (MET == 0) {
+            if (g >= ngroups) {
+                const int64_t p0 = (g - ngroups) * R;
+                pruned_pair_group<R>(X, d, C, K, pairs + p0, (int)min((int64_t)R, ptotal - p0), xs[wave], lane,
+                                     exact_dist != 0, assign, dist);
+                continue;
+            }
+        }
         const int nr = (int)min((int64_t)R, total - g * R);
         int32_t myrow[R];
 #pragma unroll
@@ -836,13 +884,17 @@
     const TX* __restrict__ X, int d, const double* __restrict__ C, const float* __restrict__ CT32,
     const float* __restrict__ cconst, int K, int Kpad, const int32_t* __restrict__ rows,
     const unsigned long long* __restrict__ row_count, int64_t max_rows, int32_t* __restrict__ assign,
-    double* __restrict__ dist, const int32_t* __restrict__ seg_counts, int64_t seg_rows, int nseg, int exact_dist) {
+    double* __restrict__ dist, const int32_t* __restrict__ seg_counts, int64_t seg_rows, int nseg, int exact_dist,
+    const unsigned long long* __restrict__ pairs) {
     __shared__ TX xs[XP_WAVES][R][XB_DMAX];
     __shared__ int gpre[XPW_MAXSEG + 1];
     const int lane = threadIdx.x & 63, wave = threadIdx.x >> 6;
+    const bool has_pairs = MET == 0 && pairs && seg_counts;
     int64_t ngroups;
     if (seg_counts) {
-        for (int sg = threadIdx.x; sg < nseg; sg += 64 * XP_WAVES) gpre[sg + 1] = (seg_counts[SEG_SLOTS * sg + SEG_ROWS] + R - 1) / R;
+        for (int sg = threadIdx.x; sg < nseg; sg += 64 * XP_WAVES)
+            gpre[sg + 1] = (seg_counts[SEG_SLOTS * sg + SEG_ROWS] + R - 1) / R +
+                           (has_pairs ? (min(seg_counts[SEG_SLOTS * sg + SEG_FIX], (int)seg_rows) + R - 1) / R : 0);
         __syncthreads();
         if (threadIdx.x == 0) {
             gpre[0] = 0;
@@ -869,6 +921,16 @@
             grows = rows + (int64_t)lo * seg_rows;
             gbase = (g - gpre[lo]) * R;
             cnt = seg_counts[SEG_SLOTS * lo + SEG_ROWS];
+            if constexpr (MET == 0) {
+                const int64_t rgroups = (cnt + R - 1) / R;
+                if (has_pairs && g - gpre[lo] >= rgroups) {
+                    const int64_t p0 = (g - gpre[lo] - rgroups) * R;
+                    const int64_t pcnt = min(seg_counts[SEG_SLOTS * lo + SEG_FIX], (int)seg_rows);
+                    pruned_pair_group<R>(X, d, C, K, pairs + (int64_t)lo * seg_rows + p0, (int)min((int64_t)R, pcnt - p0),
+                                         xs[wave], lane, exact_dist != 0, assign, dist);
+                    continue;
+                }
+            }
         } else {
             grows = rows;
             gbase = g * R;
@@ -1007,8 +1069,8 @@
     return kstatus("exact_prep_kernel");
 }
 
-int launch_assign_pruned_list(hipStream_t s, const AssignJob& q, float* ws, const RowList& l, int exact_dist,
-                              bool prepped) {
+int launch_assign_pruned_list(hipStream_t s, const AssignJob& q, float* ws, const RowList& l,
+                              const unsigned long long* pairs, int exact_dist, bool prepped) {
     const Pts X = q.X;
     const int64_t max_rows = l.bound, seg_rows = l.seg_rows;
     const int d = q.d, K = q.K, nseg = l.nseg, metric = q.metric == 0 ? 0 : 1;
@@ -1022,6 +1084,10 @@
         set_error("launch_assign_pruned_list: unsupported shape");
         return -1;
     }
+    if (pairs && (!seg_counts || metric != 0)) {
+        set_error("launch_assign_pruned_list: a pair list needs the euclidean metric and a segmented row list");
+        return -1;
+    }
     const int Kpad = (K + 63) / 64 * 64;
     float* CT32 = ws;
     float* cconst = ws + (size_t)d * Kpad;
@@ -1036,11 +1102,12 @@
     const int64_t blocks = seg_counts ? (int64_t)nseg * XP_SPLIT : std::min<int64_t>((groups + XP_WAVES - 1) / XP_WAVES, 2048);
 #define XP_LAUNCH(TX, NCH, RR, MT, XP)                                                                              \
     hipLaunchKernelGGL((assign_pruned_kernel<TX, NCH, RR, MT>), dim3((unsigned)blocks), dim3(64 * XP_WAVES), 0, s, XP, \
-                       d, C, CT32, cconst, K, Kpad, rows, row_count, max_rows, assign, dist, seg_counts, seg_rows, exact_dist)
+                       d, C, CT32, cconst, K, Kpad, rows, row_count, max_rows, assign, dist, seg_counts, seg_rows, exact_dist, \
+                       pairs)
 #define XPW_LAUNCH(TX, MT, NC, RW, XP)                                                                           \
     hipLaunchKernelGGL((assign_pruned_wide_kernel<TX, MT, NC, RW>), dim3((unsigned)wblocks), dim3(64 * XP_WAVES), 0, s, \
                        XP, d, C, CT32, cconst, K, Kpad, rows, row_count, max_rows, assign, dist, seg_counts, seg_rows, nseg, \
-                       exact_dist)
+                       exact_dist, pairs)
     const int64_t wblocks = std::min<int64_t>((groups + XP_WAVES - 1) / XP_WAVES, 1024);
     if (flat) {
         if (metric == 1) {
diff --git a/crypto-recommendation_amd/csrc/common.h b/crypto-recommendation_amd/csrc/common.h
--- a/crypto-recommendation_amd/csrc/common.h
+++ b/crypto-recommendation_amd/csrc/common.h
@@ -82,7 +82,8 @@
     STAT_KM_SEQ = 9,
     STAT_PAM_SCREENED = 10,
     STAT_PAM_EXACT = 11,
-    STAT_COUNT = 12
+    STAT_ASSIGN_PAIR = 12,
+    STAT_COUNT = 13
 };
 
 constexpr int WAVE = 64;
diff --git a/crypto-recommendation_amd/csrc/fused.hip b/crypto-recommendation_amd/csrc/fused.hip
--- a/crypto-recommendation_amd/csrc/fused.hip
+++ b/crypto-recommendation_amd/csrc/fused.hip
@@ -38,6 +38,7 @@
     w.hfix = (unsigned long long*)at(ctx->ws_hfix, l.hfix_off);
     w.cfix = (unsigned long long*)at(ctx->ws_hfix, l.cfix_off);
     w.hfix2 = (unsigned long long*)at(ctx->ws_hfix, l.hfix2_off);
+    w.pair = (unsigned long long*)at(ctx->ws_hfix, l.pair_off);
     if (l.part) w.part = ctx->ws_part.as<float4>();
     w.cnt = ctx->ws_counter.as<unsigned long long>();
     if (l.xn2) w.xn2 = ctx->ws_xn2.as<double>();
@@ -212,6 +213,7 @@
     const FusedArgs common = fused_common_args(ctx, q, sh, w);
     RowList exact_rows;
     exact_rows.p = w.list1; exact_rows.count = w.cnt + CNT_AMBIG; exact_rows.bound = q.N;
+    RecList exact_pairs;
     RecList dist_fix[2];
     int ndist_fix = 0;
     SideFork side{ctx};
@@ -256,6 +258,9 @@
         rf.list_in = l1.p; rf.list_counts = l1.counts; rf.list_seg_rows = l1.seg_rows;
         rf.ambig = l2.p; rf.ambig_count = l2.count; rf.seg_counts = l2.counts;
         rf.hfix = cosine ? w.hfix2 : hi.hfix; rf.hfix_count = cosine ? w.cnt + CNT_CFIX : hi.hfix_count;
+        if (w.pair && xprep && !test_switch("LSHKM_PAIR_PASS", "0"))
+            exact_pairs = segmented(w.pair, w.cnt + CNT_PAIR, w.seg2, q, p);
+        rf.pair = exact_pairs.p; rf.pair_count = w.cnt + CNT_PAIR;
         if ((rc = fused_refine_passes(s, rf, p))) return rc;
         if (cosine && (rc = side.join())) return rc;
         if ((rc = kstatus("fused_hi_kernel"))) return rc;
@@ -264,15 +269,18 @@
         if (cosine) dist_fix[ndist_fix++] = segmented(w.hfix2, w.cnt + CNT_CFIX, w.seg2, q, p);
     }
     if (ctx->timing) LSHKM_HIP(hipEventRecord(ctx->tev[1], s));
-    if ((rc = exact_listed(ctx, q, exact_rows, !sh.fast, xprep, cosine ? w.xn2 : nullptr, cosine ? w.nbv : nullptr)))
+    if ((rc = exact_listed(ctx, q, exact_rows, exact_pairs, !sh.fast, xprep, cosine ? w.xn2 : nullptr,
+                           cosine ? w.nbv : nullptr)))
         return rc;
     if ((rc = side.join())) return rc;
     {
-        int di[3], n = 0;
-        const unsigned long long* sp[3];
+        int di[5], n = 0;
+        const unsigned long long* sp[5];
         di[n] = STAT_REFINED; sp[n++] = w.cnt + CNT_REFINED;
         if (sh.hash) { di[n] = STAT_HASH_FIX; sp[n++] = w.cnt + CNT_HFIX; }
         di[n] = STAT_ASSIGN_AMBIG; sp[n++] = w.cnt + CNT_AMBIG;
+        di[n] = STAT_ASSIGN_AMBIG; sp[n++] = w.cnt + CNT_PAIR;
+        di[n] = STAT_ASSIGN_PAIR; sp[n++] = w.cnt + CNT_PAIR;
         if ((rc = launch_add_counters(s, ctx->stats.as<unsigned long long>(), n, di, sp))) return rc;
     }
     if (cosine || pwfix) {
diff --git a/crypto-recommendation_amd/csrc/fused_args.h b/crypto-recommendation_amd/csrc/fused_args.h
--- a/crypto-recommendation_amd/csrc/fused_args.h
+++ b/crypto-recommendation_amd/csrc/fused_args.h
@@ -57,6 +57,8 @@
     int d, xvec;
     const double* Cd;
     int pw_lds;
+    unsigned long long* pair;
+    unsigned long long* pair_count;
 };
 
 }
diff --git a/crypto-recommendation_amd/csrc/fused_impl.h b/crypto-recommendation_amd/csrc/fused_impl.h
--- a/crypto-recommendation_amd/csrc/fused_impl.h
+++ b/crypto-recommendation_amd/csrc/fused_impl.h
@@ -11,6 +11,7 @@
 #include "exact.h"
 #include "hash_tile.h"
 #include "fused_args.h"
+#include "top3.h"
 
 namespace lshkm {
 
@@ -32,6 +33,7 @@
     int32_t *list2 = nullptr, *seg2 = nullptr;
     int32_t* seg3 = nullptr;
     unsigned long long *hfix = nullptr, *cfix = nullptr, *hfix2 = nullptr;
+    unsigned long long* pair = nullptr;
     float4* part = nullptr;
     unsigned long long* cnt = nullptr;
     double* xn2 = nullptr;
@@ -170,5 +172,13 @@
         m1 = vmax3(m1, ta, tb);
     }
 }
+__device__ inline void tile_epilogue3(const float (&sv)[16], float& m1, float& m2, float& m3) {
+#pragma unroll
+    for (int r = 0; r < 16; r += 2) {
+        const float ta = __uint_as_float((__float_as_uint(sv[r]) & ~0xFu) | (uint32_t)r);
+        const float tb = __uint_as_float((__float_as_uint(sv[r + 1]) & ~0xFu) | (uint32_t)(r + 1));
+        top3_update(m1, m2, m3, ta, tb);
+    }
+}
 
 }
diff --git a/crypto-recommendation_amd/csrc/fused_layout.h b/crypto-recommendation_amd/csrc/fused_layout.h
--- a/crypto-recommendation_amd/csrc/fused_layout.h
+++ b/crypto-recommendation_amd/csrc/fused_layout.h
@@ -27,6 +27,8 @@
     if (!hash && d >= 1 && d <= FUSED_DIMS && K <= FH_KMAX) return {FusedForm::hi, f64 ? 2 : 1};
     return {FusedForm::none, 0};
 }
+
+constexpr bool fused_pair_list(bool cosine, int rows) { return !cosine && rows == 0; }
 
 constexpr int FUSED_MAX_SEGS = 1024;
 constexpr int SEG_ROWS = 0, SEG_FIX = 1, SEG_SLOTS = 2;
@@ -62,7 +64,8 @@
 constexpr int CNT_HFIX = 1;
 constexpr int CNT_REFINED = 2;
 constexpr int CNT_CFIX = 3;
-constexpr size_t FUSED_COUNTER_BYTES = 64, FUSED_COUNTER_CLEAR = 32;
+constexpr int CNT_PAIR = 4;
+constexpr size_t FUSED_COUNTER_BYTES = 64, FUSED_COUNTER_CLEAR = 64;
 
 struct FusedShape {
     int64_t N = 0;
@@ -94,6 +97,7 @@
     size_t xn2 = 0;
     size_t cl_off = 0, cnh_off = 0, nbv_off = 0, rn32_off = 0;
     size_t hfix_off = NONE, cfix_off = NONE, hfix2_off = NONE;
+    size_t pair_off = NONE;
 };
 inline FusedLayout fused_layout(const FusedShape& q) {
     FusedLayout l;
@@ -114,6 +118,7 @@
     if (q.hash || q.cosine) l.hfix_off = 0;
     if (q.cosine || pwfix) l.cfix_off = regions++ * cap * 8;
     if (q.cosine) l.hfix2_off = regions++ * cap * 8;
+    if (fused_pair_list(q.cosine, q.rows)) l.pair_off = regions++ * cap * 8;
     l.fix = regions * cap * 8;
     if (q.cosine || pwfix) l.seg3 = SEG_COUNTER_BYTES;
     if (Kpad > (size_t)FP_KMAX) l.part = (size_t)(l.part_bytes = fused_part_bytes(q.N));
diff --git a/crypto-recommendation_amd/csrc/fused_refine.hip b/crypto-recommendation_amd/csrc/fused_refine.hip
--- a/crypto-recommendation_amd/csrc/fused_refine.hip
+++ b/crypto-recommendation_amd/csrc/fused_refine.hip
@@ -30,8 +30,9 @@
 __host__ __device__ constexpr int fp_lds_bytes(int Kpad) { return 16 + 2 * Kpad * FU_RS * 2 + Kpad * 4; }
 static_assert(fp_lds_bytes(FP_KMAX) <= 160 * 1024, "refinement LDS image exceeds 160 KiB");
 
-template <int MET, bool MP, int ROWS>
+template <int MET, bool MP, int ROWS, bool PAIR = false>
 __global__ __launch_bounds__(FP_THREADS, 1) void fused_persistent_kernel(FusedArgs a) {
+    static_assert(!PAIR || fused_pair_list(MET == 1, ROWS), "fused_layout.h states which forms have a pair list");
     extern __shared__ __attribute__((aligned(16))) char smem[];
     const int Kpad = a.Kpad;
     int* lcount = reinterpret_cast<int*>(smem);
@@ -58,9 +59,10 @@
         }
     }
     for (int e = threadIdx.x; e < Kpad; e += FP_THREADS) lcn[e] = a.cnh[e];
-    if (threadIdx.x < 2) lcount[threadIdx.x] = 0;
+    if (threadIdx.x < 3) lcount[threadIdx.x] = 0;
     int32_t* ambig_seg = a.ambig + (int64_t)blockIdx.x * a.seg_rows;
     unsigned long long* hfix_seg = a.hfix + (int64_t)blockIdx.x * a.seg_rows;
+    unsigned long long* pair_seg = PAIR ? a.pair + (int64_t)blockIdx.x * a.seg_rows : nullptr;
     __syncthreads();
 
     const int lane = threadIdx.x & 63, wave = threadIdx.x >> 6;
@@ -113,27 +115,33 @@
                       (ROWS == 2 ? 0x1p-24 * nx * (double)cmaxf : 0.0)) * (1.f + 0x1p-20f) + 1e-30f
             : (float)(nx * (double)ecf + (double)ebf + FU_A2 * x1 + 0x1p-41 * xn2 +
                       0x1p-18 * nx * (double)cmaxf + 0x1p-43 * nx) * (1.f + 0x1p-20f) + 1e-30f;
-        float m1 = -__builtin_inff(), m2 = -__builtin_inff();
-        int t1 = 0;
+        float m1 = -__builtin_inff(), m2 = -__builtin_inff(), m3 = -__builtin_inff();
+        int t1 = 0, t2 = 0;
         if (MP && !a.pass_first) {
             const float4 st = a.part[ptile * 64 + lane];
             m1 = st.x; m2 = st.y; t1 = __float_as_int(st.z);
+            if constexpr (PAIR) { m3 = st.w; t2 = top3_tile2_of(t1); t1 = top3_tile1(t1); }
         }
         const int tg0 = MP ? a.t0 : 0;
         __builtin_amdgcn_s_setprio(MFMA_PRIO);
 #pragma unroll 1
         for (int t = 0; t < ntile32; t++) {
-            const float m1_prev = m1;
+            const float m1_prev = m1, m2_prev = m2;
             float sv[16];
             floatx16 acc_hi, acc_lo;
             tile_mfma(my_h + t * 32 * FU_RS, my_l + t * 32 * FU_RS, bh, bl, acc_hi, acc_lo);
             tile_scores(acc_hi, acc_lo, lcn + t * 32 + 4 * h, sv);
-            tile_epilogue(sv, m1, m2);
+            if constexpr (PAIR) {
+                tile_epilogue3(sv, m1, m2, m3);
+                t2 = top3_tile2(m1_prev, m2_prev, m1, m2, t1, t2, t + tg0);
+            } else {
+                tile_epilogue(sv, m1, m2);
+            }
             t1 = m1 != m1_prev ? t + tg0 : t1;
         }
         __builtin_amdgcn_s_setprio(0);
         if (MP && !a.pass_last) {
-            a.part[ptile * 64 + lane] = make_float4(m1, m2, __int_as_float(t1), 0.f);
+            a.part[ptile * 64 + lane] = make_float4(m1, m2, __int_as_float(PAIR ? top3_pack_tiles(t1, t2) : t1), PAIR ? m3 : 0.f);
             continue;
         }
         const uint32_t l1 = __float_as_uint(m1) & 0xFu;
@@ -144,6 +152,16 @@
         const int I1 = (om1 > m1 || (om1 == m1 && oi1 < i1)) ? oi1 : i1;
         const float M1 = fmaxf(m1, om1);
         const bool cert = x_ok && c_ok && ((double)M2 < (double)M1 - 2.0 * (double)E);
+        bool pairc = false;
+        uint32_t pair_ids = 0;
+        if constexpr (PAIR) {
+            const uint32_t l2 = __float_as_uint(m2) & 0xFu;
+            const int i2 = t2 * 32 + 8 * (int)(l2 >> 2) + 4 * h + (int)(l2 & 3u);
+            const Top3Row tr = top3_merge(m1, m2, m3, i1, i2, om1, om2, __shfl_xor(m3, 32), oi1, __shfl_xor(i2, 32));
+            pairc = !cert && x_ok && c_ok && tr.M2 > -0x1p99f &&
+                    ((double)tr.M3 < (double)M1 - 2.0 * (double)E);
+            pair_ids = (uint32_t)tr.I1 | ((uint32_t)tr.I2 << 16);
+        }
 
         PT_MARK(2)
         if constexpr (MET == 1) {
@@ -219,31 +237,49 @@
             }
         }
         PT_MARK(3)
-        const bool amb = valid && !cert;
+        const bool amb = valid && !cert && !pairc;
         const unsigned long long amask = __ballot(amb && h == 1);
-        if (h == 1 && valid) {
-            if (!cert) {
+        if (h == 1 && amb) {
+            int base = 0;
+            const int leader = __builtin_ctzll(amask);
+            if (lane == leader) base = atomicAdd(lcount, __popcll(amask));
+            base = __shfl(base, leader);
+            const int rank = __popcll(amask & ((1ull << lane) - 1ull));
+            ambig_seg[base + rank] = (int32_t)row;
+        }
+        if constexpr (PAIR) {
+            const bool pr = valid && pairc && h == 1;
+            const unsigned long long pmask = __ballot(pr);
+            if (pr) {
                 int base = 0;
-                const int leader = __builtin_ctzll(amask);
-                if (lane == leader) base = atomicAdd(lcount, __popcll(amask));
+                const int leader = __builtin_ctzll(pmask);
+                if (lane == leader) base = atomicAdd(lcount + 2, __popcll(pmask));
                 base = __shfl(base, leader);
-                const int rank = __popcll(amask & ((1ull << lane) - 1ull));
-                ambig_seg[base + rank] = (int32_t)row;
+                const int rank = __popcll(pmask & ((1ull << lane) - 1ull));
+                pair_seg[base + rank] = (unsigned long long)row | ((unsigned long long)pair_ids << 32);
             }
         }
         PT_MARK(4)
     }
     PT_FLUSH
     __syncthreads();
-    if (threadIdx.x < 2 && (!MP || (threadIdx.x == 0 ? a.pass_last != 0 : (MET == 1 && a.pass_last)))) {
-        const int c = lcount[threadIdx.x];
+    static_assert(SEG_ROWS == 0 && SEG_FIX == 1, "thread i reports slot i");
+    if (threadIdx.x < 2 && (!MP || a.pass_last) && (threadIdx.x == 0 || !MP || MET == 1 || PAIR)) {
+        const int c = threadIdx.x == 0 ? lcount[0] : PAIR ? lcount[2] : lcount[1];
         a.seg_counts[SEG_SLOTS * blockIdx.x + threadIdx.x] = c;
-        if (c) atomicAdd(threadIdx.x == 0 ? a.ambig_count : a.hfix_count, (unsigned long long)c);
+        if (c) atomicAdd(threadIdx.x == 0 ? a.ambig_count : PAIR ? a.pair_count : a.hfix_count, (unsigned long long)c);
     }
 }
 
 template <int MET, bool MP, int ROWS>
 static void refine_launch(hipStream_t s, unsigned nblk, const FusedArgs& a) {
+    if constexpr (fused_pair_list(MET == 1, ROWS)) {
+        if (a.pair) {
+            hipLaunchKernelGGL((fused_persistent_kernel<MET, MP, ROWS, true>), dim3(nblk), dim3(FP_THREADS),
+                               (size_t)fp_lds_bytes(a.Kpad), s, a);
+            return;
+        }
+    }
     hipLaunchKernelGGL((fused_persistent_kernel<MET, MP, ROWS>), dim3(nblk), dim3(FP_THREADS),
                        (size_t)fp_lds_bytes(a.Kpad), s, a);
 }
@@ -259,6 +295,10 @@
         set_error("launch_fused_refine_pass: no kernel for this metric / row kind / slice");
         return -1;
     }
+    if (a.pair && (!fused_pair_list(metric == 1, rows) || (mp ? a.t0 : 0) + (a.Kpad >> 5) > TOP3_TILE_LIMIT)) {
+        set_error("launch_fused_refine_pass: a pair list needs the euclidean fp32 form and tiles that fit top3_pack_tiles");
+        return -1;
+    }
     if (metric == 1) mp ? refine_rows<1, true>(s, nblk, rows, a) : refine_rows<1, false>(s, nblk, rows, a);
     else mp ? refine_rows<0, true>(s, nblk, rows, a) : refine_rows<0, false>(s, nblk, rows, a);
     return 0;
diff --git a/crypto-recommendation_amd/csrc/index.h b/crypto-recommendation_amd/csrc/index.h
--- a/crypto-recommendation_amd/csrc/index.h
+++ b/crypto-recommendation_amd/csrc/index.h
@@ -43,8 +43,8 @@
               int32_t* out_phi, int32_t* out_bucket, int32_t* mm, bool* h16 = nullptr);
 bool exact_pruned(Pts X, int d, int K, int metric);
 int exact_listed_prep(lshkm_ctx_s* ctx, const AssignJob& q);
-int exact_listed(lshkm_ctx_s* ctx, const AssignJob& q, const RowList& l, bool exact_dist, bool prepped,
-                 const double* xn2, const double* nbv);
+int exact_listed(lshkm_ctx_s* ctx, const AssignJob& q, const RowList& l, const RecList& pairs, bool exact_dist,
+                 bool prepped, const double* xn2, const double* nbv);
 struct AssignRequest : AssignJob {
     const ::lshkm_lsh_s* lsh = nullptr;
     int32_t *tuples = nullptr, *phi = nullptr, *bucket = nullptr;
diff --git a/crypto-recommendation_amd/csrc/kernels.h b/crypto-recommendation_amd/csrc/kernels.h
--- a/crypto-recommendation_amd/csrc/kernels.h
+++ b/crypto-recommendation_amd/csrc/kernels.h
@@ -99,8 +99,8 @@
 int launch_assign_exact(hipStream_t s, const AssignJob& q, const RowList& l, const double* xn2 = nullptr,
                         const double* nbv = nullptr);
 int launch_assign_exact_list(hipStream_t s, const AssignJob& q, double* CT, const RowList& l);
-int launch_assign_pruned_list(hipStream_t s, const AssignJob& q, float* ws, const RowList& l, int exact_dist,
-                              bool prepped);
+int launch_assign_pruned_list(hipStream_t s, const AssignJob& q, float* ws, const RowList& l,
+                              const unsigned long long* pairs, int exact_dist, bool prepped);
 int launch_assign_pruned_prep(hipStream_t s, bool xf64, int d, const double* C, int K, float* ws, int metric);
 int launch_assign_override(hipStream_t s, const int32_t* src_rows, int K, int64_t N, int32_t* assign,
                            double* dist);
diff --git a/crypto-recommendation_amd/csrc/top3.h b/crypto-recommendation_amd/csrc/top3.h
--- /dev/null
+++ b/crypto-recommendation_amd/csrc/top3.h
@@ -0,0 +1,73 @@
+#pragma once
+
+#if defined(__HIPCC__)
+#define T3_HD __host__ __device__ inline
+#else
+#define T3_HD static inline
+#endif
+
+namespace lshkm {
+
+T3_HD float t3_min(float a, float b) {
+#if defined(__HIP_DEVICE_COMPILE__)
+    float r;
+    asm("v_min_f32 %0, %1, %2" : "=v"(r) : "v"(a), "v"(b));
+    return r;
+#else
+    return b < a ? b : a;
+#endif
+}
+T3_HD float t3_max(float a, float b) {
+#if defined(__HIP_DEVICE_COMPILE__)
+    float r;
+    asm("v_max_f32 %0, %1, %2" : "=v"(r) : "v"(a), "v"(b));
+    return r;
+#else
+    return b > a ? b : a;
+#endif
+}
+T3_HD float t3_max3(float a, float b, float c) {
+#if defined(__HIP_DEVICE_COMPILE__)
+    float r;
+    asm("v_max3_f32 %0, %1, %2, %3" : "=v"(r) : "v"(a), "v"(b), "v"(c));
+    return r;
+#else
+    return t3_max(t3_max(a, b), c);
+#endif
+}
+
+T3_HD void top3_update(float& m1, float& m2, float& m3, float ta, float tb) {
+    const float hi = t3_max(ta, tb), lo = t3_min(ta, tb);
+    m3 = t3_max3(m3, t3_min(m2, hi), t3_min(m1, lo));
+    m2 = t3_max3(m2, t3_min(m1, hi), lo);
+    m1 = t3_max(m1, hi);
+}
+
+T3_HD int top3_tile2(float p1, float p2, float m1, float m2, int t1, int t2, int t) {
+    if (m2 == p2) return t2;
+    return (m1 != p1 && m2 == p1) ? t1 : t;
+}
+
+T3_HD int top3_pack_tiles(int t1, int t2) { return (t1 & 0xFFFF) | (t2 << 16); }
+T3_HD int top3_tile1(int packed) { return packed & 0xFFFF; }
+T3_HD int top3_tile2_of(int packed) { return (int)((unsigned)packed >> 16); }
+constexpr int TOP3_TILE_LIMIT = 1 << 15;
+
+struct Top3Row {
+    float M1, M2, M3;
+    int I1, I2;
+};
+T3_HD Top3Row top3_merge(float a1, float a2, float a3, int ai1, int ai2, float b1, float b2, float b3, int bi1,
+                         int bi2) {
+    Top3Row r;
+    const bool bwins = b1 > a1 || (b1 == a1 && bi1 < ai1);
+    r.M1 = t3_max(a1, b1);
+    r.M2 = t3_max3(a2, b2, t3_min(a1, b1));
+    r.M3 = t3_max(t3_max3(a3, b3, t3_min(a1, b2)), t3_min(a2, b1));
+    r.I1 = bwins ? bi1 : ai1;
+    if (bwins) r.I2 = a1 >= b2 ? ai1 : bi2;
+    else r.I2 = b1 >= a2 ? bi1 : ai2;
+    return r;
+}
+
+}
diff --git a/crypto-recommendation_amd/lshkm.py b/crypto-recommendation_amd/lshkm.py
--- a/crypto-recommendation_amd/lshkm.py
+++ b/crypto-recommendation_amd/lshkm.py
@@ -13,6 +13,7 @@
 STAT_POW_FIX = 8
 STAT_KM_SEQ = 9
 STAT_PAM_SCREENED, STAT_PAM_EXACT = 10, 11
+STAT_ASSIGN_PAIR = 12
 _METRIC = {"euclidean": EUCLIDEAN, "cosine": COSINE, EUCLIDEAN: EUCLIDEAN, COSINE: COSINE}
 DIST_CERTIFIED, DIST_EXACT = 0, 1
 _DIST = {"certified": DIST_CERTIFIED, "default": DIST_CERTIFIED, "exact": DIST_EXACT,
```
